# maniacs-ops/ringpop-go

Measured on AMD Instinct MI355X. Metric: simulated member-rounds/sec at 64k members, higher is better.
Workload: dtype u32; 1 GPU; config3_cascade: 65536 members, 655 killed at r=10; rounds 5-592 timed (steady state, kill, suspect wave; faulty wave from r>=35 in window); members=65536, live_member_rounds=38153303, parallelism=1 GPU

## Files before the change

### ringpop-go_amd/csrc/swimsim_engine.hip

```cpp
#include "swimsim_kernels.hip"
#include "swimsim_xchg.hip"
#include "swimsim_census.hip"
#include "swimsim_route.hip"

#include <hipcub/hipcub.hpp>
#include <rccl/rccl.h>

#include <algorithm>
#include <cmath>
#include <condition_variable>
#include <cstdarg>
#include <cstdio>
#include <cstring>
#include <memory>
#include <mutex>
#include <string>
#include <thread>
#include <vector>

#include "../../include/swimsim.h"

using namespace swimdev;

namespace {

const char *kStatus[4] = {"alive", "suspect", "faulty", "leave"};
constexpr uint32_t kWatchCap = 64;

struct Timed {
    int fam;
    hipEvent_t a, b;
};

enum Fam { F_TIMERS, F_SELECT, F_ISSUE, F_SORT, F_RECV, F_RESP, F_PINGREQ, F_JOBS, F_CS_WIDE, F_CS_NARROW, F_CSPREP,
           F_EVENTS, F_XCHG, F_RECVFIN, F_CSD_SCAN, F_CS_FALLBACK, F_JOBS_MERGE, F_NFAM };
const char *kFamName[F_NFAM] = {"timers", "select", "issue", "sort", "recv_merge", "resp_merge", "pingreq",
                                "rfs_jobs", "checksum_wide", "checksum_narrow", "checksum_prep", "events", "exchange",
                                "recv_finish", "checksum_delta_scan", "checksum_fallback", "rfs_merge"};

struct Transport {
    uint32_t G = 1, rank = 0;
    virtual ~Transport() {}
    virtual int sizes(const uint64_t *send, uint64_t *recv, int k) = 0;
    virtual int data(const uint8_t *sbuf, const uint64_t *soff, const uint64_t *sbytes, uint8_t *rbuf,
                     const uint64_t *roff, const uint64_t *rbytes, hipStream_t st) = 0;
    virtual int bcast(void *buf, size_t bytes, uint32_t root) = 0;
    virtual const char *name() const = 0;
    virtual bool stream_ordered() const { return false; }
    virtual int sizes_dev(const uint64_t *dsend, uint64_t *drecv, int k, hipStream_t st) { return SWIMSIM_EINVAL; }
};

struct LocalHub {
    uint32_t G;
    std::mutex m;
    std::condition_variable cv;
    uint32_t arrived = 0, gen = 0;
    bool aborted = false;
    std::vector<const void *> ptr;
    std::vector<const uint64_t *> off, len;
    std::vector<int> dev;
    explicit LocalHub(uint32_t g) : G(g), ptr(g), off(g), len(g), dev(g, 0) {}
    bool barrier() {
        std::unique_lock<std::mutex> lk(m);
        if (aborted) return false;
        const uint32_t my = gen;
        if (++arrived == G) {
            arrived = 0;
            gen++;
            cv.notify_all();
        } else {
            cv.wait(lk, [&] { return gen != my || aborted; });
        }
        return !aborted;
    }
    void abort() {
        std::lock_guard<std::mutex> lk(m);
        aborted = true;
        cv.notify_all();
    }
};

struct LocalPort : Transport {
    std::shared_ptr<LocalHub> hub;
    int device = 0;
    const char *name() const override { return "local"; }
    int sizes(const uint64_t *send, uint64_t *recv, int k) override {
        hub->ptr[rank] = send;
        if (!hub->barrier()) return SWIMSIM_EHIP;
        for (uint32_t s = 0; s < G; s++)
            for (int i = 0; i < k; i++) recv[s * k + i] = ((const uint64_t *)hub->ptr[s])[rank * k + i];
        return hub->barrier() ? 0 : SWIMSIM_EHIP;
    }
    int data(const uint8_t *sbuf, const uint64_t *soff, const uint64_t *sbytes, uint8_t *rbuf, const uint64_t *roff,
             const uint64_t *rbytes, hipStream_t st) override {
        hub->ptr[rank] = sbuf;
        hub->off[rank] = soff;
        hub->len[rank] = sbytes;
        hub->dev[rank] = device;
        if (!hub->barrier()) return SWIMSIM_EHIP;
        hipError_t e = hipSuccess;
        for (uint32_t s = 0; s < G && e == hipSuccess; s++) {
            if (!rbytes[s]) continue;
            const uint8_t *src = (const uint8_t *)hub->ptr[s] + hub->off[s][rank];
            e = hub->dev[s] == device ? hipMemcpyAsync(rbuf + roff[s], src, rbytes[s], hipMemcpyDeviceToDevice, st)
                                      : hipMemcpyPeerAsync(rbuf + roff[s], device, src, hub->dev[s], rbytes[s], st);
        }
        if (e == hipSuccess) e = hipStreamSynchronize(st);
        if (e != hipSuccess) { hub->abort(); return SWIMSIM_EHIP; }
        return hub->barrier() ? 0 : SWIMSIM_EHIP;
    }
    int bcast(void *buf, size_t bytes, uint32_t root) override {
        hub->ptr[rank] = buf;
        if (!hub->barrier()) return SWIMSIM_EHIP;
        if (rank != root) memcpy(buf, hub->ptr[root], bytes);
        return hub->barrier() ? 0 : SWIMSIM_EHIP;
    }
};

struct RcclPort : Transport {
    ncclComm_t comm = nullptr;
    hipStream_t st = nullptr;
    hipEvent_t order = nullptr;
    uint64_t *dsz = nullptr;
    size_t dsz_cap = 0;
    const char *name() const override { return "rccl"; }
    bool stream_ordered() const override { return true; }
    ~RcclPort() override {
        if (comm) ncclCommDestroy(comm);
        if (dsz) hipFree(dsz);
        if (order) hipEventDestroy(order);
    }
    int stage(size_t bytes) {
        if (bytes <= dsz_cap) return 0;
        if (dsz) hipFree(dsz);
        dsz_cap = std::max<size_t>(bytes, 4096);
        return hipMalloc(&dsz, dsz_cap) == hipSuccess ? 0 : SWIMSIM_ENOMEM;
    }
    int sizes(const uint64_t *send, uint64_t *recv, int k) override {
        const size_t n = (size_t)G * k;
        if (int rc = stage(2 * n * 8)) return rc;
        uint64_t *ds = dsz, *dr = dsz + n;
        if (hipMemcpyAsync(ds, send, n * 8, hipMemcpyHostToDevice, st) != hipSuccess) return SWIMSIM_EHIP;
        if (int rc = sizes_dev(ds, dr, k, st)) return rc;
        if (hipMemcpyAsync(recv, dr, n * 8, hipMemcpyDeviceToHost, st) != hipSuccess) return SWIMSIM_EHIP;
        return hipStreamSynchronize(st) == hipSuccess ? 0 : SWIMSIM_EHIP;
    }
    int sizes_dev(const uint64_t *dsend, uint64_t *drecv, int k, hipStream_t s) override {
        if (s != st) return SWIMSIM_EINVAL;
        ncclResult_t rc = ncclGroupStart();
        for (uint32_t p = 0; p < G && rc == ncclSuccess; p++) {
            rc = ncclSend(dsend + (size_t)p * k, k, ncclUint64, (int)p, comm, st);
            if (rc == ncclSuccess) rc = ncclRecv(drecv + (size_t)p * k, k, ncclUint64, (int)p, comm, st);
        }
        const ncclResult_t rc_end = ncclGroupEnd();
        return rc == ncclSuccess && rc_end == ncclSuccess ? 0 : SWIMSIM_EHIP;
    }
    int data(const uint8_t *sbuf, const uint64_t *soff, const uint64_t *sbytes, uint8_t *rbuf, const uint64_t *roff,
             const uint64_t *rbytes, hipStream_t s) override {
        if (s != st) {
            if (!order && hipEventCreateWithFlags(&order, hipEventDisableTiming) != hipSuccess) return SWIMSIM_EHIP;
            if (hipEventRecord(order, st) != hipSuccess || hipStreamWaitEvent(s, order, 0) != hipSuccess) return SWIMSIM_EHIP;
        }
        ncclResult_t rc = ncclGroupStart();
        for (uint32_t p = 0; p < G && rc == ncclSuccess; p++) {
            if (sbytes[p]) rc = ncclSend(sbuf + soff[p], sbytes[p], ncclUint8, (int)p, comm, s);
            if (rbytes[p] && rc == ncclSuccess) rc = ncclRecv(rbuf + roff[p], rbytes[p], ncclUint8, (int)p, comm, s);
        }
        const ncclResult_t rc_end = ncclGroupEnd();
        if (rc != ncclSuccess || rc_end != ncclSuccess) return SWIMSIM_EHIP;
        if (s != st && (hipEventRecord(order, s) != hipSuccess || hipStreamWaitEvent(st, order, 0) != hipSuccess))
            return SWIMSIM_EHIP;
        return 0;
    }
    int bcast(void *buf, size_t bytes, uint32_t root) override {
        if (int rc = stage(bytes)) return rc;
        if (hipMemcpyAsync(dsz, buf, bytes, hipMemcpyHostToDevice, st) != hipSuccess) return SWIMSIM_EHIP;
        if (ncclBroadcast(dsz, dsz, bytes, ncclUint8, (int)root, comm, st) != ncclSuccess) return SWIMSIM_EHIP;
        if (hipMemcpyAsync(buf, dsz, bytes, hipMemcpyDeviceToHost, st) != hipSuccess) return SWIMSIM_EHIP;
        return hipStreamSynchronize(st) == hipSuccess ? 0 : SWIMSIM_EHIP;
    }
};

struct HostPort : Transport {
    swimsim_host_transport t{};
    uint8_t *hs = nullptr, *hr = nullptr;
    size_t hs_cap = 0, hr_cap = 0;
    const char *name() const override { return "host"; }
    ~HostPort() override {
        if (hs) hipHostFree(hs);
        if (hr) hipHostFree(hr);
    }
    static int grow(uint8_t **p, size_t *cap, size_t bytes) {
        if (bytes <= *cap) return 0;
        if (*p) hipHostFree(*p);
        *cap = std::max<size_t>(bytes + bytes / 2, 1 << 16);
        return hipHostMalloc((void **)p, *cap, 0) == hipSuccess ? 0 : SWIMSIM_ENOMEM;
    }
    int sizes(const uint64_t *send, uint64_t *recv, int k) override {
        return t.alltoall_u64(t.ctx, send, recv, k) ? SWIMSIM_EHIP : 0;
    }
    int data(const uint8_t *sbuf, const uint64_t *soff, const uint64_t *sbytes, uint8_t *rbuf, const uint64_t *roff,
             const uint64_t *rbytes, hipStream_t st) override {
        size_t stot = 0, rtot = 0;
        for (uint32_t p = 0; p < G; p++) {
            stot = std::max<size_t>(stot, soff[p] + sbytes[p]);
            rtot = std::max<size_t>(rtot, roff[p] + rbytes[p]);
        }
        if (grow(&hs, &hs_cap, stot) || grow(&hr, &hr_cap, rtot)) return SWIMSIM_ENOMEM;
        if (stot && hipMemcpyAsync(hs, sbuf, stot, hipMemcpyDeviceToHost, st) != hipSuccess) return SWIMSIM_EHIP;
        if (hipStreamSynchronize(st) != hipSuccess) return SWIMSIM_EHIP;
        if (t.alltoallv(t.ctx, hs, soff, sbytes, hr, roff, rbytes)) return SWIMSIM_EHIP;
        if (rtot && hipMemcpyAsync(rbuf, hr, rtot, hipMemcpyHostToDevice, st) != hipSuccess) return SWIMSIM_EHIP;
        return hipStreamSynchronize(st) == hipSuccess ? 0 : SWIMSIM_EHIP;
    }
    int bcast(void *buf, size_t bytes, uint32_t root) override { return t.bcast(t.ctx, buf, bytes, root) ? SWIMSIM_EHIP : 0; }
};

struct CsrSet {
    bool ready = false, failed = false;
    uint32_t rows = 0;
    uint32_t *B = nullptr, *Lb = nullptr, *OB = nullptr, *SBw = nullptr, *fb = nullptr, *fbcnt = nullptr, *nrec = nullptr;
    uint4 *ent = nullptr, *P = nullptr;
    CsdRow *rinfo = nullptr;
    CsrPlan *plan = nullptr;
    CsrRec *rec = nullptr;
    uint4 *ucol = nullptr;
    uint32_t *fbsplit = nullptr;
    unsigned long long *acc = nullptr;
    void *cub_tmp = nullptr;
    size_t cub_bytes = 0;
    uint32_t *ucl = nullptr, *uhk = nullptr, *ucold = nullptr, *ucnt = nullptr;
};

}

struct swimsim {
    uint32_t N = 0, NP = 0, NL = 0, lo = 0, W = 19, K = 3, maxjobs = 5, pfactor = 15;
    int64_t t0 = 0;
    uint32_t period = 200;
    uint32_t to_susp = 25, to_faulty = 0, to_tomb = 0;
    uint64_t seed = 1;
    uint32_t ecap = 0, max_tl = 0;
    bool fast_cs = false;
    int device = 0;
    hipStream_t s = nullptr;
    hipStream_t side = nullptr;
    hipEvent_t ev_snap = nullptr, ev_side[2] = {nullptr, nullptr};
    hipEvent_t ev_rt = nullptr;
    hipStream_t side2 = nullptr;
    hipEvent_t ev_csr2 = nullptr;
    bool csr2_used = false;
    bool sync_spin = true;
    bool cs_async = true, side_pending = false;
    bool side_pend[2] = {false, false};
    uint32_t side_halves = 1, side_gen = 0;
    uint32_t cs_narrow_rows = CS_NARROW_ROWS;
    uint32_t snap_cap = 0;
    uint32_t *side_ids = nullptr, *side_cnt = nullptr;

    DS d{};
    std::vector<uint8_t> live;
    std::vector<int32_t> part;
    std::vector<int32_t> coff;
    int32_t coff_min = 0, coff_max = 0;
    std::vector<std::string> addrs;
    uint32_t round = 0;
    uint64_t host_ctr[SWIMSIM_NCOUNTERS] = {0};
    uint32_t G = 1, rank = 0;
    std::vector<uint32_t> shard_lo;
    std::unique_ptr<Transport> xp;
    uint4 *xitems = nullptr;
    uint32_t *xcnt = nullptr, xcap = 0;
    unsigned long long *xsz = nullptr, *xseg = nullptr, *xtcur = nullptr, *xdcur = nullptr;
    ulonglong2 *xsrcs = nullptr;
    uint8_t *sbuf = nullptr, *rbuf = nullptr;
    size_t sbuf_cap = 0, rbuf_cap = 0;
    uint2 *needlist = nullptr;
    uint32_t *needcnt = nullptr, needcap = 0;
    uint32_t *hsics = nullptr, *npairs = nullptr;
    unsigned long long *keys = nullptr, *keys_sorted = nullptr;
    uint32_t keycap = 0;
    uint64_t x_bytes = 0, x_calls = 0;
    uint64_t x_syncs = 0;
    uint64_t lazy_fallbacks = 0;
    uint64_t alloc_bytes = 0;
    int32_t *tgt = nullptr;
    uint8_t *failed = nullptr;
    MsgDesc *sdesc = nullptr, *rdesc = nullptr, *sdesc2 = nullptr, *rdesc2 = nullptr, *snapdesc = nullptr, *hdesc = nullptr;
    uint32_t *sI = nullptr, *sC = nullptr, *sI2 = nullptr, *sC2 = nullptr;
    uint32_t *sS = nullptr, *sS2 = nullptr;
    uint32_t *rcs = nullptr, *csreqcnt = nullptr;
    uint4 *csreq = nullptr;
    uint32_t *fpv = nullptr, *fpv_s = nullptr, *fph = nullptr, *fph_s = nullptr, *fplist = nullptr, *fpcnt = nullptr,
             *dup_of = nullptr;
    uint8_t *hflag = nullptr;
    uint32_t *H = nullptr, *nh = nullptr;
    uint32_t *keys_in = nullptr, *vals_out = nullptr;
    uint4 *pinfo = nullptr;
    uint32_t inbox_n = 0;
    uint32_t *ukeys = nullptr, *counts = nullptr, *offs = nullptr, *nruns = nullptr, *info = nullptr;
    void *cub_tmp = nullptr;
    size_t cub_bytes = 0;
    uint32_t *list = nullptr, *cnt = nullptr;
    uint4 *defer = nullptr;
    uint32_t *defer_cnt = nullptr;
    uint8_t *defer_eq = nullptr;
    unsigned long long *rep_tab = nullptr;
    unsigned long long *fp_tab = nullptr;
    uint32_t rep_mask = 0, rep_gen = 0;
    uint32_t *exh_list = nullptr, *exh_cnt = nullptr, *scratch = nullptr;
    uint8_t *need = nullptr, *fsflag = nullptr;
    uint4 *evbuf = nullptr;
    uint32_t *ev_applied = nullptr;
    uint32_t evcap = 0;
    uint4 *jl = nullptr;
    unsigned long long *digest_buf = nullptr;
    uint32_t *hinfo = nullptr;
    std::vector<void *> allocs;
    bool timing = false;
    uint32_t timing_mask = 0;
    std::vector<Timed> pending;
    std::vector<hipEvent_t> evpool;
    double fam_ms[F_NFAM] = {0};
    uint64_t fam_n[F_NFAM] = {0};
    uint64_t fam_bytes_base[CTR_STRIDE] = {0};
    std::vector<hipEvent_t> round_ev;
    std::vector<float> round_ms;
    std::vector<uint32_t> wslot_h;
    std::vector<uint8_t> wused;
    std::vector<uint32_t> wcs;
    std::vector<uint32_t> wcs_ev;
    std::vector<uint4 *> wev_h;
    std::vector<unsigned long long *> wevt_h;
    uint4 *wout = nullptr;
    uint32_t *winfo = nullptr;
    uint32_t *cn_slab = nullptr, *cn_part = nullptr, *cn_nlp = nullptr, *cn_ticket = nullptr, *cn_cols = nullptr,
             *cn_res = nullptr;
    size_t cn_cap = 0;
    hipEvent_t cn_ev[2] = {nullptr, nullptr};
    uint32_t *tr_cols = nullptr, *tr_buf = nullptr, *tr_part = nullptr, *tr_nlp = nullptr, *tr_state = nullptr;
    uint32_t tr_n = 0, tr_cap = 0;
    size_t tr_bytes[5] = {0, 0, 0, 0, 0};
    struct RouteTable {
        uint32_t R;
        uint32_t *hm;
        unsigned long long *pts;
    };
    std::vector<RouteTable> rt_tabs;
    uint8_t *rt_bytes = nullptr;
    uint64_t *rt_off = nullptr;
    uint32_t *rt_kh = nullptr, *rt_p0 = nullptr, *rt_rows = nullptr, *rt_cnt = nullptr;
    int32_t *rt_base = nullptr, *rt_own = nullptr;
    uint32_t *rt_srv = nullptr;
    int32_t *rt_nbase = nullptr;
    size_t rt_srv_cap = 0, rt_nbase_cap = 0;
    unsigned long long *rt_exc = nullptr, *rt_exc2 = nullptr, *rt_uniq = nullptr, *rt_cur = nullptr;
    void *rt_cub = nullptr;
    size_t rt_bytes_cap = 0, rt_keys_cap = 0, rt_rows_cap = 0, rt_own_cap = 0, rt_exc_cap = 0, rt_cub_bytes = 0;
    std::vector<uint64_t> rt_rel;
    hipEvent_t rt_ev[2] = {nullptr, nullptr};
    int csr_mode = 1;
    CsrSet csr, csr2;
    size_t csr_sbw_words = 0;
    uint32_t csr_ecap = 4096, csr_rcap = 1024, csr_KP = 0;
    uint64_t csr_launches = 0;
    uint32_t csr_side_min = 4097;
    int fault_inject = 0;
    int defer_test = 0;
    int cs_defer = 1;
    uint32_t rounds_left = 0;
    uint32_t round_deferred = 0;
    bool cs_carried = false;
    bool cs_defer_log = false;
    uint64_t cs_skipped_rounds = 0, cs_carried_rows = 0, cs_forced = 0, cs_units_base[3] = {0, 0, 0};
    bool colx_stale = false;
    std::string err;

    int fail(int code, const char *fmt, ...) {
        char buf[512];
        va_list ap;
        va_start(ap, fmt);
        vsnprintf(buf, sizeof buf, fmt, ap);
        va_end(ap);
        err = buf;
        return code;
    }
};

#define HIPCHK(h, x)                                                                             \
    do {                                                                                         \
        hipError_t e_ = (x);                                                                     \
        if (e_ != hipSuccess) return (h)->fail(SWIMSIM_EHIP, "%s: %s", #x, hipGetErrorString(e_)); \
    } while (0)

namespace {

template <typename T>
int dalloc(swimsim *h, T **p, size_t count, const char *what) {
    void *q = nullptr;
    size_t bytes = std::max<size_t>(count * sizeof(T), 16);
    hipError_t e = hipMalloc(&q, bytes);
    if (e != hipSuccess) return h->fail(SWIMSIM_ENOMEM, "hipMalloc(%s, %zu bytes): %s", what, bytes, hipGetErrorString(e));
    h->allocs.push_back(q);
    h->alloc_bytes += bytes;
    *p = (T *)q;
    return 0;
}

template <typename T>
void dfree(swimsim *h, T **p, size_t bytes) {
    if (!*p) return;
    auto it = std::find(h->allocs.begin(), h->allocs.end(), (void *)*p);
    if (it != h->allocs.end()) h->allocs.erase(it);
    hipFree(*p);
    h->alloc_bytes -= bytes;
    *p = nullptr;
}

hipEvent_t take_event(swimsim *h) {
    if (!h->evpool.empty()) {
        hipEvent_t e = h->evpool.back();
        h->evpool.pop_back();
        return e;
    }
    hipEvent_t e;
    hipEventCreate(&e);
    return e;
}

struct Scope {
    swimsim *h;
    int fam;
    hipStream_t st;
    hipEvent_t a{}, b{};
    bool on;
    Scope(swimsim *h_, int f, hipStream_t st_ = nullptr)
        : h(h_), fam(f), st(st_ ? st_ : h_->s), on(h_->timing && ((h_->timing_mask >> f) & 1u)) {
        if (on) {
            a = take_event(h);
            hipEventRecord(a, st);
        }
    }
    ~Scope() {
        if (on) {
            b = take_event(h);
            hipEventRecord(b, st);
            h->pending.push_back(Timed{fam, a, b});
        }
    }
};

void drain_timing(swimsim *h) {
    if (h->pending.empty()) return;
    hipStreamSynchronize(h->s);
    for (auto &t : h->pending) {
        float ms = 0;
        hipEventElapsedTime(&ms, t.a, t.b);
        h->fam_ms[t.fam] += ms;
        h->fam_n[t.fam]++;
        h->evpool.push_back(t.a);
        h->evpool.push_back(t.b);
    }
    h->pending.clear();
}

constexpr uint32_t SWIM_WAVE_BLOCK = 256;
constexpr uint32_t kWavesPerBlock = SWIM_WAVE_BLOCK / 64;
inline uint32_t blocks_for_waves(uint32_t waves) { return waves ? (waves + kWavesPerBlock - 1) / kWavesPerBlock : 1; }
inline uint32_t blocks_for_threads(uint32_t n) { return n ? (n + 255) / 256 : 1; }
inline uint32_t rep_slots(uint32_t nl) { uint32_t s = 1024; while (s < 2 * nl) s <<= 1; return s; }

constexpr uint32_t kMaxEcap = 1u << 24;

int build_tail_table(swimsim *h, uint32_t ecap) {
    if (ecap > kMaxEcap)
        return h->fail(SWIMSIM_ERANGE, "incarnation step %u beyond the checksum tables (at most 2^24 steps of the period)",
                       ecap - 1);
    std::vector<uint32_t> t((size_t)ecap * 4 * 8, 0u);
    uint32_t max_tl = 0, min_tl = 0xFFFFFFFFu;
    for (uint32_t e = 0; e < ecap; e++) {
        char digits[32];
        snprintf(digits, sizeof digits, "%lld", (long long)(h->t0 + (int64_t)e * h->period));
        for (uint32_t s = 0; s < 4; s++) {
            char buf[64];
            int n = snprintf(buf, sizeof buf, "%s%s;", kStatus[s], digits);
            if (n > 24) return h->fail(SWIMSIM_EINVAL, "incarnation %s too long for the checksum tail table", digits);
            uint8_t bytes[24] = {0};
            memcpy(bytes, buf, (size_t)n);
            uint32_t *dst = &t[((size_t)e * 4 + s) * 8];
            for (int w = 0; w < 6; w++)
                dst[w] = (uint32_t)bytes[4 * w] | ((uint32_t)bytes[4 * w + 1] << 8) | ((uint32_t)bytes[4 * w + 2] << 16) |
                         ((uint32_t)bytes[4 * w + 3] << 24);
            dst[6] = (uint32_t)n;
            max_tl = std::max(max_tl, (uint32_t)n);
            min_tl = std::min(min_tl, (uint32_t)n);
        }
    }
    std::vector<uint32_t> rt((size_t)ecap * 4 * 8, 0u);
    const uint32_t q = h->W / 4, r = h->W % 4;
    for (size_t i = 0; i < (size_t)ecap * 4; i++) {
        uint8_t bytes[32] = {0};
        const uint32_t n = t[i * 8 + 6];
        memcpy(bytes + r, &t[i * 8], n);
        for (int w = 0; w < 7; w++)
            rt[i * 8 + w] = (uint32_t)bytes[4 * w] | ((uint32_t)bytes[4 * w + 1] << 8) | ((uint32_t)bytes[4 * w + 2] << 16) |
                            ((uint32_t)bytes[4 * w + 3] << 24);
        const uint32_t L = h->W + n;
        const uint8_t *tb = (const uint8_t *)&t[i * 8];
        rt[i * 8 + 7] = (uint32_t)tb[n - 4] | ((uint32_t)tb[n - 3] << 8) | ((uint32_t)tb[n - 2] << 16) |
                        ((uint32_t)tb[n - 1] << 24);
        if (r + n > 27) return h->fail(SWIMSIM_EINVAL, "record tail too long for the checksum tail table");
        rt[i * 8 + 6] |= L << 24;
    }
    (void)q;
    std::vector<uint32_t> rt8((size_t)ecap * 8 * 8, 0u);
    for (size_t e = 0; e < ecap; e++)
        for (int s = 0; s < 4; s++) memcpy(&rt8[(e * 8 + s) * 8], &rt[(e * 4 + s) * 8], 32);
    uint32_t *dev = nullptr, *rdev = nullptr, *r8dev = nullptr;
    if (int rc = dalloc(h, &dev, t.size(), "tail table")) return rc;
    if (int rc = dalloc(h, &rdev, rt.size(), "record tail table")) return rc;
    if (int rc = dalloc(h, &r8dev, rt8.size(), "record tail table by member word")) return rc;
    HIPCHK(h, hipMemcpy(dev, t.data(), t.size() * 4, hipMemcpyHostToDevice));
    HIPCHK(h, hipMemcpy(rdev, rt.data(), rt.size() * 4, hipMemcpyHostToDevice));
    HIPCHK(h, hipMemcpy(r8dev, rt8.data(), rt8.size() * 4, hipMemcpyHostToDevice));
    h->d.tailw = dev;
    h->d.rtail = rdev;
    h->d.rtail8 = r8dev;
    {
        uint32_t d0 = t[6] - 6, nthr = 0;
        for (int k = 0; k < 8; k++) h->d.dig_thr[k] = 0xFFFFFFFFu;
        uint32_t prev = d0;
        for (uint32_t e = 1; e < ecap; e++) {
            const uint32_t de = t[((size_t)e * 4) * 8 + 6] - 6;
            if (de != prev) {
                if (de != prev + 1 || nthr == 8) return h->fail(SWIMSIM_EINVAL, "incarnation digit count changes too often");
                h->d.dig_thr[nthr++] = e;
                prev = de;
            }
        }
        h->d.dig_d0 = d0;
    }
    h->ecap = ecap;
    h->d.ecap = ecap;
    h->max_tl = max_tl;
    h->d.max_tail = max_tl;
    h->d.min_tail = min_tl;
    h->fast_cs = (h->W == 19 && h->W + max_tl <= 40);
    return 0;
}

hipError_t stream_sync(swimsim *h) {
    if (!h->sync_spin || !h->ev_rt) return hipStreamSynchronize(h->s);
    const hipError_t prior = hipPeekAtLastError();
    hipError_t e = hipEventRecord(h->ev_rt, h->s);
    if (e != hipSuccess) return e;
    while ((e = hipEventQuery(h->ev_rt)) == hipErrorNotReady) {
    }
    (void)hipGetLastError();
    return prior != hipSuccess ? prior : e;
}

int check_err(swimsim *h) {
    uint32_t e = 0;
    HIPCHK(h, hipMemcpyAsync(&e, h->d.err, 4, hipMemcpyDeviceToHost, h->s));
    HIPCHK(h, stream_sync(h));
    if (!e) return 0;
    hipMemsetAsync(h->d.err, 0, 4, h->s);
    if (e & E_POOL) return h->fail(SWIMSIM_ECAPACITY, "message pool overflow (raise message_pool_bytes)");
    if (e & E_DENSE) return h->fail(SWIMSIM_ECAPACITY, "dense snapshot pool overflow");
    if (e & E_ECAP) return h->fail(SWIMSIM_ECAPACITY, "incarnation beyond the checksum table");
    if (e & E_SHORT) return h->fail(SWIMSIM_EINVAL, "checksum string of <= 24 bytes is not supported");
    if (e & E_ITER) return h->fail(SWIMSIM_EINVAL, "iterator found no pingable member despite a positive count");
    return h->fail(SWIMSIM_EINVAL, "dissemination count mismatch (internal error %u)", e);
}

int read_counters(swimsim *h, uint64_t *out ) {
    std::vector<uint64_t> c((size_t)CTR_SHARDS * CTR_STRIDE);
    HIPCHK(h, hipMemcpyAsync(c.data(), h->d.ctr, c.size() * 8, hipMemcpyDeviceToHost, h->s));
    HIPCHK(h, stream_sync(h));
    for (int i = 0; i < CTR_STRIDE; i++) {
        uint64_t t = 0;
        for (int k = 0; k < CTR_SHARDS; k++) t += c[(size_t)k * CTR_STRIDE + i];
        out[i] = t;
    }
    return 0;
}

int sort_inbox(swimsim *h, uint32_t n, uint32_t *host_info) {
    Scope sc(h, F_SORT);
    h->inbox_n = n;
    int endbit = 1;
    while ((1u << endbit) <= h->N) endbit++;
    size_t bytes = h->cub_bytes;
    HIPCHK(h, hipcub::DeviceRadixSort::SortKeys(h->cub_tmp, bytes, h->keys, h->keys_sorted, (int)n, 0, 32 + endbit, h->s));
    hipLaunchKernelGGL(k_split_keys, dim3(blocks_for_threads(n)), dim3(256), 0, h->s, h->keys_sorted, n, h->keys_in,
                       h->vals_out);
    bytes = h->cub_bytes;
    HIPCHK(h, hipcub::DeviceRunLengthEncode::Encode(h->cub_tmp, bytes, h->keys_in, h->ukeys, h->counts, h->nruns,
                                                    (int)n, h->s));
    bytes = h->cub_bytes;
    HIPCHK(h, hipcub::DeviceScan::ExclusiveSum(h->cub_tmp, bytes, h->counts, h->offs, (int)n, h->s));
    HIPCHK(h, hipMemsetAsync(h->info, 0, 8, h->s));
    hipLaunchKernelGGL(k_runs_info, dim3(blocks_for_threads(n)), dim3(256), 0, h->s, h->ukeys, h->counts, h->nruns, h->N,
                       h->info);
    HIPCHK(h, hipMemcpyAsync(host_info, h->info, 16, hipMemcpyDeviceToHost, h->s));
    HIPCHK(h, stream_sync(h));
    return 0;
}

inline uint32_t owner_host(const swimsim *h, uint32_t o) {
    uint32_t r = 0;
    while (r + 1 < h->G && o >= h->shard_lo[r + 1]) r++;
    return r;
}

XArgs xargs(swimsim *h) {
    XArgs x{};
    x.sdesc = h->sdesc; x.sdesc2 = h->sdesc2; x.rdesc = h->rdesc; x.rdesc2 = h->rdesc2; x.snapdesc = h->snapdesc;
    x.hdesc = h->hdesc;
    x.sI = h->sI; x.sC = h->sC; x.sI2 = h->sI2; x.sC2 = h->sC2;
    x.hsics = h->hsics;
    x.need = h->need;
    x.keys = h->keys; x.npairs = h->npairs; x.keycap = h->keycap;
    x.needlist = h->needlist; x.needcnt = h->needcnt; x.needcap = h->needcap;
    x.sS = h->sS; x.sS2 = h->sS2; x.rcs = h->rcs;
    x.csreq = h->csreq; x.csreqcnt = h->csreqcnt; x.csreqcap = h->keycap;
    return x;
}

int xchg(swimsim *h) {
    Scope sc(h, F_XCHG);
    const uint32_t G = h->G;
    const XArgs x = xargs(h);
    HIPCHK(h, hipMemsetAsync(h->xsz, 0, 2 * G * 8, h->s));
    hipLaunchKernelGGL(k_x_size, dim3(blocks_for_threads(h->xcap)), dim3(256), 0, h->s, h->d, x, h->xitems, h->xcnt,
                       h->xcap, h->xsz);
    const bool dev_sizes = h->xp->stream_ordered();
    std::vector<uint64_t> sz(2 * G), sendsz(2 * G), recvsz(2 * G), devsend(2 * G);
    uint32_t nitems = 0;
    hipLaunchKernelGGL(k_x_sendsz, dim3(1), dim3(64), 0, h->s, h->xsz, G, h->xsz + 2 * G);
    if (dev_sizes) {
        if (int rc = h->xp->sizes_dev((const uint64_t *)(h->xsz + 2 * G), (uint64_t *)(h->xsz + 4 * G), 2, h->s))
            return h->fail(rc, "shard size exchange failed (%s)", h->xp->name());
        HIPCHK(h, hipMemcpyAsync(recvsz.data(), h->xsz + 4 * G, 2 * G * 8, hipMemcpyDeviceToHost, h->s));
    } else {
        HIPCHK(h, hipMemcpyAsync(devsend.data(), h->xsz + 2 * G, 2 * G * 8, hipMemcpyDeviceToHost, h->s));
    }
    HIPCHK(h, hipMemcpyAsync(sz.data(), h->xsz, 2 * G * 8, hipMemcpyDeviceToHost, h->s));
    HIPCHK(h, hipMemcpyAsync(&nitems, h->xcnt, 4, hipMemcpyDeviceToHost, h->s));
    HIPCHK(h, stream_sync(h));
    h->x_syncs++;
    if (nitems > h->xcap) return h->fail(SWIMSIM_ECAPACITY, "exchange item list overflow (%u items)", nitems);
    std::vector<uint64_t> soff(G), sbytes(G), tbl(G), cur(3 * G);
    uint64_t total = 0;
    for (uint32_t p = 0; p < G; p++) {
        tbl[p] = (sz[2 * p + 1] * 4 + 15) & ~15ull;
        sbytes[p] = sz[2 * p + 1] ? tbl[p] + sz[2 * p] : 0;
        soff[p] = total;
        total += (sbytes[p] + 15) & ~15ull;
        cur[p] = soff[p];
        cur[G + p] = 0;
        cur[2 * G + p] = tbl[p];
        sendsz[2 * p] = sbytes[p];
        sendsz[2 * p + 1] = sz[2 * p + 1];
    }
    if (!dev_sizes && devsend != sendsz)
        return h->fail(SWIMSIM_EHIP, "exchange: device send sizes (k_x_sendsz) differ from the host's");
    if (total > h->sbuf_cap) {
        if (h->sbuf) hipFree(h->sbuf);
        h->sbuf_cap = std::max<uint64_t>(total + total / 2, 1 << 20);
        HIPCHK(h, hipMalloc(&h->sbuf, h->sbuf_cap));
    }
    HIPCHK(h, hipMemcpyAsync(h->xseg, cur.data(), 3 * G * 8, hipMemcpyHostToDevice, h->s));
    if (nitems)
        hipLaunchKernelGGL(k_x_pack, dim3(blocks_for_waves(nitems)), dim3(SWIM_WAVE_BLOCK), 0, h->s, h->d, x, h->xitems, h->xcnt,
                           h->xcap, h->sbuf, h->xseg, h->xtcur, h->xdcur);
    if (!dev_sizes) {
        HIPCHK(h, stream_sync(h));
        if (int rc = h->xp->sizes(sendsz.data(), recvsz.data(), 2)) return h->fail(rc, "shard size exchange failed (%s)", h->xp->name());
        h->x_syncs += 2;
    }
    std::vector<uint64_t> roff(G), rbytes(G);
    std::vector<ulonglong2> srcs(G);
    uint64_t rtotal = 0, nparc = 0;
    for (uint32_t p = 0; p < G; p++) {
        rbytes[p] = recvsz[2 * p];
        roff[p] = rtotal;
        srcs[p] = make_ulonglong2(rtotal, nparc);
        rtotal += (rbytes[p] + 15) & ~15ull;
        nparc += recvsz[2 * p + 1];
    }
    if (rtotal > h->rbuf_cap) {
        if (h->rbuf) hipFree(h->rbuf);
        h->rbuf_cap = std::max<uint64_t>(rtotal + rtotal / 2, 1 << 20);
        HIPCHK(h, hipMalloc(&h->rbuf, h->rbuf_cap));
    }
    if (int rc = h->xp->data(h->sbuf, soff.data(), sbytes.data(), h->rbuf, roff.data(), rbytes.data(), h->s))
        return h->fail(rc, "shard data exchange failed (%s)", h->xp->name());
    if (nparc) {
        HIPCHK(h, hipMemcpyAsync(h->xsrcs, srcs.data(), G * sizeof(ulonglong2), hipMemcpyHostToDevice, h->s));
        hipLaunchKernelGGL(k_x_unpack, dim3(blocks_for_waves((uint32_t)nparc)), dim3(SWIM_WAVE_BLOCK), 0, h->s, h->d, x, h->rbuf,
                           h->xsrcs, G, (uint32_t)nparc);
    }
    HIPCHK(h, hipMemsetAsync(h->xcnt, 0, 4, h->s));
    h->x_bytes += total;
    h->x_calls++;
    return 0;
}

int shard_sum(swimsim *h, uint64_t v, uint64_t *out) {
    if (h->G == 1) { *out = v; return 0; }
    std::vector<uint64_t> send(h->G, v), recv(h->G);
    if (int rc = h->xp->sizes(send.data(), recv.data(), 1)) return h->fail(rc, "shard reduction failed");
    uint64_t t = 0;
    for (uint64_t x : recv) t += x;
    *out = t;
    return 0;
}

bool csr_wanted(swimsim *h, uint32_t n, CsKind kind) {
    if (h->csr_mode == 0 || h->csr.failed || n < CSD_MIN_ROWS || h->N < 1024) return false;
    return kind == CS_WIDE || h->csr_mode == 2;
}

bool csr_side_wanted(swimsim *h, uint32_t n) {
    return h->csr_mode != 0 && !h->csr2.failed && h->csr2.rows && n >= h->csr_side_min && n <= h->csr2.rows &&
           h->N >= 1024;
}

int csr_alloc(swimsim *h, CsrSet &c, uint32_t rows) {
    if (c.ready) return 0;
    if (c.failed) return 1;
    const bool side = &c == &h->csr2;
    h->csr_rcap = h->N <= 131072 ? 1024u : 512u;
    h->csr_sbw_words = ((size_t)h->N * (h->W + 32) + 256) / 4;
    h->csr_KP = (uint32_t)(h->csr_sbw_words * 4 / 20 + 2);
    c.rows = rows;
    const size_t nalloc0 = h->allocs.size();
    const uint64_t bytes0 = h->alloc_bytes;
    auto undo = [&](int rc) {
        for (size_t i = nalloc0; i < h->allocs.size(); i++) hipFree(h->allocs[i]);
        h->allocs.resize(nalloc0);
        h->alloc_bytes = bytes0;
        (void)hipGetLastError();
        c.failed = true;
        c.rows = 0;
        h->err.clear();
        return rc;
    };
    int rc = 0;
    if ((rc = dalloc(h, &c.B, (size_t)h->NP, "csr reference row")) ||
        (rc = dalloc(h, &c.Lb, (size_t)h->N + 1, "csr reference lengths")) ||
        (rc = dalloc(h, &c.OB, (size_t)h->N + 1, "csr reference offsets")) ||
        (rc = dalloc(h, &c.SBw, h->csr_sbw_words, "csr reference string")) ||
        (rc = dalloc(h, &c.P, (size_t)20 * h->csr_KP * 2, "csr premix table")) ||
        (rc = dalloc(h, &c.fb, (size_t)rows, "csr fallback list")) ||
        (rc = dalloc(h, &c.fbcnt, 8, "csr fallback count and reasons")) ||
        (rc = dalloc(h, &c.rinfo, (size_t)rows, "csr row info")) ||
        (rc = dalloc(h, &c.ent, ((size_t)rows * h->csr_ecap + CSR_EREG) * 2, "csr exception entries")) ||
        (rc = dalloc(h, &c.plan, (size_t)rows / CSR_ROWS + 1, "csr plans")) ||
        (rc = dalloc(h, &c.rec, (size_t)rows * h->csr_rcap, "csr records")) ||
        (rc = dalloc(h, &c.nrec, (size_t)rows, "csr record counts")) ||
        (rc = dalloc(h, &c.ucol, (size_t)h->N, "csr divergent column table")) ||
        (rc = (h->fault_inject & 1) ? h->fail(SWIMSIM_ENOMEM, "injected allocation failure") : 0) ||
        (rc = dalloc(h, &c.fbsplit, 4, "csr fallback split")) ||
        (rc = dalloc(h, &c.acc, 8, "csr path statistics")))
        return undo(rc);
    if (side && ((rc = dalloc(h, &c.ucl, (size_t)h->N, "csr side divergent columns")) ||
                 (rc = dalloc(h, &c.uhk, (size_t)h->N, "csr side divergent column slots")) ||
                 (rc = dalloc(h, &c.ucold, (size_t)h->N, "csr side cold columns")) ||
                 (rc = dalloc(h, &c.ucnt, 2, "csr side column counts"))))
        return undo(rc);
    size_t need = 0;
    hipcub::DeviceScan::ExclusiveSum(nullptr, need, c.Lb, c.OB, (int)h->N + 1, h->s);
    void *p = nullptr;
    if ((side || need > h->cub_bytes) && (rc = dalloc(h, (uint8_t **)&p, need, "cub temp (csr)"))) return undo(rc);
    if (hipMemsetAsync(c.acc, 0, 8 * sizeof(unsigned long long), h->s) != hipSuccess) return undo(SWIMSIM_EHIP);
    if (side) {
        c.cub_tmp = p;
        c.cub_bytes = need;
    } else if (p) {
        h->cub_tmp = p;
        h->cub_bytes = need;
    }
    c.ready = true;
    return 0;
}
int csr_alloc(swimsim *h) { return csr_alloc(h, h->csr, h->NL); }

__global__ void k_csr_fbsplit(uint32_t *fbcnt, uint32_t *split, unsigned long long *acc) {
    const uint32_t t = threadIdx.x;
    const uint32_t nf = fbcnt[0];
    if (t == 0) {
        split[0] = min(nf, 4096u);
        split[1] = nf > 4096u ? min(nf - 4096u, 8192u) : 0u;
        split[2] = nf > 12288u ? nf - 12288u : 0u;
    }
    if (t < 8 && nf) acc[t] += fbcnt[t];
}

int csr_hash(swimsim *h, CsrSet &c, const uint32_t *list, const uint32_t *cnt, uint32_t n, hipStream_t st, int chains = 4) {
    const bool side = &c == &h->csr2;
    if (n > (side ? c.rows : h->NL)) return 1;
    if (side ? !c.ready : csr_alloc(h, c, h->NL)) return 1;
    if (h->fault_inject & 2) {
        h->fault_inject &= ~2;
        return h->fail(SWIMSIM_EHIP, "csr_hash: injected HIP error");
    }
    DS d = h->d;
    if (side) { d.ucl = c.ucl; d.uhk = c.uhk; d.ucold = c.ucold; d.ucnt = c.ucnt; }
    void *cub = side ? c.cub_tmp : h->cub_tmp;
    size_t cub_bytes = side ? c.cub_bytes : h->cub_bytes;
    CsdArgs ca{};
    ca.B = c.B;
    ca.OB = c.OB;
    ca.SBw = c.SBw;
    ca.sbw_words = (uint32_t)h->csr_sbw_words;
    ca.ent = c.ent;
    ca.rinfo = c.rinfo;
    ca.ecap = h->csr_ecap;
    ca.ulist = d.ucl;
    ca.ucnt = d.ucnt;
    ca.ucol = c.ucol;
    ca.uhk = side ? nullptr : d.uhk;
    CsrArgs a{};
    a.P = c.P;
    a.KP = h->csr_KP;
    a.ent = c.ent;
    a.rinfo = c.rinfo;
    a.ecap = h->csr_ecap;
    a.plan = c.plan;
    a.rec = c.rec;
    a.nrec = c.nrec;
    a.rcap = h->csr_rcap;
    a.fb_list = c.fb;
    a.fb_cnt = c.fbcnt;
    a.exw = (h->fault_inject & 4) ? 8u : 0xFFFFFFFFu;
    a.stprio = (h->fault_inject & 16) ? 1u : 0u;
    a.jitter = (h->fault_inject & 64) ? (((uint32_t)h->fault_inject >> 8) & 15u) | ((uint32_t)h->fault_inject >> 12 << 8) : 0u;
    {
        Scope sc(h, F_CSD_SCAN, st);
        hipLaunchKernelGGL(k_csd_ref, dim3((h->N + 256) / 256), dim3(256), 0, st, d, list, n, c.B, c.Lb);
        size_t bytes = cub_bytes;
        HIPCHK(h, hipcub::DeviceScan::ExclusiveSum(cub, bytes, c.Lb, c.OB, (int)h->N + 1, st));
        HIPCHK(h, hipMemsetAsync(c.SBw, 0, h->csr_sbw_words * 4, st));
        hipLaunchKernelGGL(k_ucols, dim3(1), dim3(1024), 0, st, d);
        hipLaunchKernelGGL(k_csr_ucol, dim3((h->N + 255) / 256), dim3(256), 0, st, d.ucl, d.ucnt, c.B, c.OB, c.ucol);
        launch_csr(d, list, n, cnt, ca, a, st, 0);
        launch_csr(d, list, n, cnt, ca, a, st, 1);
        launch_csr(d, list, n, cnt, ca, a, st, 2);
        launch_csr(d, list, n, cnt, ca, a, st, 3);
        HIPCHK(h, hipMemsetAsync(c.fbcnt, 0, 32, st));
        hipLaunchKernelGGL(k_ctr_add, dim3(1), dim3(1), 0, st, d, (int)C_X_CSD_SCANNED, (unsigned long long)n);
    }
    {
        Scope sc(h, F_CS_WIDE, st);
        launch_csr(d, list, n, cnt, ca, a, st, chains);
    }
    h->csr_launches++;
    Scope sc(h, F_CS_FALLBACK, st);
    hipLaunchKernelGGL(k_csr_fbsplit, dim3(1), dim3(64), 0, st, c.fbcnt, c.fbsplit, c.acc);
    launch_checksum_kind(d, c.fb, c.fbsplit, std::min(n, 4096u), CS_NARROW, st);
    if (n > 4096u) launch_checksum_kind(d, c.fb + 4096, c.fbsplit + 1, std::min(n - 4096u, 8192u), CS_NARROW, st);
    if (n > 12288u) launch_checksum_kind(d, c.fb + 12288, c.fbsplit + 2, n - 12288u, CS_WIDE, st);
    return 0;
}
int csr_hash(swimsim *h, const uint32_t *list, const uint32_t *cnt, uint32_t n, int chains = 4) {
    return csr_hash(h, h->csr, list, cnt, n, h->s, chains);
}

int hash_rows(swimsim *h, const uint32_t *list, const uint32_t *cnt, uint32_t maxn, uint32_t nrows,
              hipStream_t st = nullptr, bool ordered = false) {
    if (std::min(maxn, nrows) == 0) return 0;
    if (!st && !ordered && nrows != ~0u && nrows >= 64 && nrows <= h->NL && (list == h->list || list == h->fplist)) {
        Scope sc(h, F_CSPREP);
        uint32_t *out = list == h->list ? h->fplist : h->list;
        const uint32_t maxid = h->NL + h->d.dense_cap;
        size_t bytes = h->cub_bytes;
        if (hipcub::DeviceRadixSort::SortKeys(h->cub_tmp, bytes, list, out, (int)nrows, 0, 32 - __builtin_clz(maxid),
                                              h->s) == hipSuccess)
            list = out;
    }
    const uint32_t n = std::min(maxn, nrows);
    const CsKind kind = cs_kind(n, h->cs_narrow_rows);
    if (!st && nrows != ~0u && csr_wanted(h, n, kind)) {
        const int rc = csr_hash(h, list, cnt, n);
        if (rc <= 0) return rc;
    }
    if (st && nrows != ~0u && csr_side_wanted(h, n)) {
        if (h->csr2_used) HIPCHK(h, hipStreamWaitEvent(st, h->ev_csr2, 0));
        const int rc = csr_hash(h, h->csr2, list, cnt, n, st);
        HIPCHK(h, hipEventRecord(h->ev_csr2, st));
        h->csr2_used = true;
        if (rc <= 0) return rc;
    }
    Scope sc(h, kind == CS_WIDE ? F_CS_WIDE : F_CS_NARROW, st);
    launch_checksum_kind(h->d, list, cnt, n, kind, st ? st : h->s);
    return 0;
}

void hot_flush(swimsim *h, uint32_t ol0, uint32_t n) {
    if (!h->d.hidx || n == 0) return;
    hipLaunchKernelGGL(k_hot_flush, dim3(blocks_for_waves(n)), dim3(SWIM_WAVE_BLOCK), 0, h->s, h->d, ol0, n);
}

void hot_reset(swimsim *h, bool flush) {
    if (!h->d.hidx) return;
    if (flush) hot_flush(h, 0, h->NL);
    hipMemsetAsync(h->d.hidx, 0xFF, (size_t)h->N * 4, h->s);
    hipMemsetAsync(h->d.hotnew, 0, (size_t)h->d.NBIT * 4, h->s);
    hipMemsetAsync(h->d.hot_cnt, 0, 8, h->s);
    hipLaunchKernelGGL(k_nhe_reset, dim3(blocks_for_threads(h->NL)), dim3(256), 0, h->s, h->d);
}

void hot_update(swimsim *h) {
    if (!h->d.hidx) return;
    hipLaunchKernelGGL(k_hot_extend, dim3(1), dim3(1024), 0, h->s, h->d);
    hipLaunchKernelGGL(k_hot_fill, dim3(blocks_for_waves(h->NL)), dim3(SWIM_WAVE_BLOCK), 0, h->s, h->d);
}

int retire_half(swimsim *h, uint32_t g) {
    if (!h->side_pend[g]) return 0;
    HIPCHK(h, hipStreamWaitEvent(h->s, h->ev_side[g], 0));
    const uint32_t lo = h->d.dense_cap + g * h->snap_cap;
    hipLaunchKernelGGL(k_side_retire, dim3(blocks_for_threads(h->NL)), dim3(256), 0, h->s, h->d, lo, lo + h->snap_cap);
    h->side_pend[g] = false;
    h->side_pending = h->side_pend[0] || h->side_pend[1];
    return 0;
}

int sync_side(swimsim *h) {
    if (!h->side_pending) return 0;
    for (uint32_t g = 0; g < 2; g++)
        if (int rc = retire_half(h, (h->side_gen + g) % 2)) return rc;
    return 0;
}

constexpr uint32_t CS_DEFER_CHANGED_NUM = 3, CS_DEFER_CHANGED_DEN = 4, CS_DEFER_MAX_DEFERRED_DIV = 64;

int checksum_dirty(swimsim *h, int mode, bool async = false) {
    const uint32_t g = h->side_gen;
    if (async && h->cs_async && h->side_halves == 2) {
        if (int rc = retire_half(h, g)) return rc;
    } else if (int rc = sync_side(h)) {
        return rc;
    }
    HIPCHK(h, hipMemsetAsync(h->cnt, 0, 8, h->s));
    {
        Scope sc(h, F_CSPREP);
        hipLaunchKernelGGL(k_list, dim3(blocks_for_threads(h->NL)), dim3(256), 0, h->s, h->d, mode, h->tgt, h->failed,
                           h->list, h->cnt);
    }
    if (mode != 0) return hash_rows(h, h->list, h->cnt, h->NL, ~0u);
    uint32_t *hn = h->hinfo + 8;
    HIPCHK(h, hipMemcpyAsync(hn, h->cnt, 8, hipMemcpyDeviceToHost, h->s));
    HIPCHK(h, stream_sync(h));
    const uint32_t n = *hn;
    if (async && h->cs_defer && h->rounds_left && n) {
        const uint32_t changed = hn[1];
        const bool wide = n > (h->cs_async ? h->snap_cap : 0u);
        const bool moving = (uint64_t)changed * CS_DEFER_CHANGED_DEN >= (uint64_t)n * CS_DEFER_CHANGED_NUM;
        const bool calm = h->round_deferred <= h->NL / CS_DEFER_MAX_DEFERRED_DIV;
        const bool skip = h->cs_defer == 2 || (wide && moving && calm);
        if (h->cs_defer_log)
            fprintf(stderr, "cs_defer round %u: dirty %u changed %u deferred %u: %s\n", h->round, n, changed,
                    h->round_deferred, skip ? "carried" : wide && moving ? "hashed (valve)" : "hashed");
        if (skip) {
            hipLaunchKernelGGL(k_carry, dim3(blocks_for_threads(h->NL)), dim3(256), 0, h->s, h->d);
            h->cs_carried = true;
            h->cs_skipped_rounds++;
            h->cs_carried_rows += n;
            return 0;
        }
        if (wide && moving) h->cs_forced++;
    }
    h->cs_carried = false;
    auto go_side = [&](const uint32_t *rows, uint32_t n2, const uint32_t *vals, const uint32_t *dups) -> int {
        uint32_t *ids = h->side_ids + (size_t)g * h->snap_cap, *icnt = h->side_cnt + g;
        {
            Scope sc(h, F_CSPREP);
            hipLaunchKernelGGL(k_snap_rows, dim3(blocks_for_waves(std::max(n2, 1u))), dim3(SWIM_WAVE_BLOCK), 0, h->s, h->d, rows, n2,
                               ids, icnt, h->d.dense_cap + g * h->snap_cap);
            hipLaunchKernelGGL(k_snap_dups, dim3(blocks_for_threads(n)), dim3(256), 0, h->s, h->d, vals, n, dups);
            hipLaunchKernelGGL(k_ctr_add, dim3(1), dim3(1), 0, h->s, h->d, (int)C_X_CS_DUP, (unsigned long long)(n - n2));
        }
        HIPCHK(h, hipEventRecord(h->ev_snap, h->s));
        hipStream_t ss = g == 0 || !h->side2 ? h->side : h->side2;
        HIPCHK(h, hipStreamWaitEvent(ss, h->ev_snap, 0));
        if (int rc = hash_rows(h, ids, icnt, n2, n2, ss)) return rc;
        HIPCHK(h, hipEventRecord(h->ev_side[g], ss));
        h->side_pend[g] = true;
        h->side_pending = true;
        h->side_gen = (g + 1) % h->side_halves;
        return 0;
    };
    const bool side_ok = async && h->cs_async;
    if (n < 2) {
        if (n == 1 && side_ok && h->snap_cap >= 1) return go_side(h->list, 1, h->list, nullptr);
        return hash_rows(h, h->list, h->cnt, n, n);
    }
    {
        Scope sc(h, F_CSPREP);
        const unsigned long long keymask = (h->fault_inject & 8) ? 7ull : ~0ull;
        const uint32_t fmask = 2u * rep_slots(h->NL) - 1u;
        HIPCHK(h, hipMemsetAsync(h->fp_tab, 0xFF, (size_t)(fmask + 1) * 2 * 8, h->s));
        for (int pass = 0; pass < 2; pass++)
            hipLaunchKernelGGL(k_fp_table, dim3(blocks_for_threads(n)), dim3(256), 0, h->s, h->d, h->list, n, h->fp_tab,
                               fmask, keymask, pass);
        hipLaunchKernelGGL(k_ucols, dim3(1), dim3(1024), 0, h->s, h->d);
        hipLaunchKernelGGL(k_fp_verify_tab, dim3(blocks_for_waves(n)), dim3(SWIM_WAVE_BLOCK), 0, h->s, h->d, h->list, n,
                           h->fp_tab, fmask, keymask, h->hflag, h->dup_of);
        hipLaunchKernelGGL(k_list_flagged_ordered, dim3(1), dim3(1024), 0, h->s, h->NL, h->hflag, h->fplist, h->fpcnt);
        HIPCHK(h, hipMemcpyAsync(hn + 1, h->fpcnt, 4, hipMemcpyDeviceToHost, h->s));
    }
    HIPCHK(h, stream_sync(h));
    if (side_ok && hn[1] <= h->snap_cap) return go_side(h->fplist, hn[1], h->list, h->dup_of);
    if (int rc = hash_rows(h, h->fplist, h->fpcnt, n, hn[1], nullptr, true)) return rc;
    Scope sc(h, F_CSPREP);
    hipLaunchKernelGGL(k_fp_copy, dim3(blocks_for_threads(n)), dim3(256), 0, h->s, h->d, h->list, n, h->dup_of);
    return 0;
}

int bound_lazy_snapshots(swimsim *h, int mode) {
    if (h->NL <= h->d.dense_cap / 2) return 0;
    HIPCHK(h, hipMemsetAsync(h->cnt, 0, 4, h->s));
    hipLaunchKernelGGL(k_list, dim3(blocks_for_threads(h->NL)), dim3(256), 0, h->s, h->d, mode, h->tgt, h->failed,
                       h->list, h->cnt);
    uint32_t *hc = h->hinfo + 12;
    HIPCHK(h, hipMemcpyAsync(hc, h->cnt, 4, hipMemcpyDeviceToHost, h->s));
    HIPCHK(h, stream_sync(h));
    if (*hc <= h->d.dense_cap / 2) return 0;
    if (int rc = sync_side(h)) return rc;
    if (int rc = hash_rows(h, h->list, h->cnt, h->NL, *hc)) return rc;
    h->lazy_fallbacks++;
    return 0;
}

int resolve_deferred(swimsim *h, int phase, MsgDesc *rdesc, uint32_t maxn) {
    const bool remote = h->G > 1 && phase != 2;
    uint32_t *sS = phase == 0 ? h->sS : phase == 1 ? h->sS2 : nullptr;
    const uint32_t *sI = phase == 1 ? h->sI2 : h->sI;
    if (remote || phase == 2)
        if (int rc = sync_side(h)) return rc;
    uint32_t maxlist = 2 * maxn;
    {
        Scope sc(h, F_CSPREP);
        HIPCHK(h, hipMemsetAsync(h->cnt, 0, 8, h->s));
        hipLaunchKernelGGL(k_ucols, dim3(1), dim3(1024), 0, h->s, h->d);
        if (h->rep_tab) {
            h->rep_gen = h->rep_gen % 255u + 1u;
            hipLaunchKernelGGL(k_cs_reps, dim3(blocks_for_threads(h->NL)), dim3(256), 0, h->s, h->d, h->defer_cnt, h->rep_tab,
                               h->rep_mask, h->rep_gen);
        }
        hipLaunchKernelGGL(k_defer_eq, dim3(blocks_for_waves(maxn)), dim3(SWIM_WAVE_BLOCK), 0, h->s, h->d, h->defer, h->defer_cnt,
                           phase, h->defer_eq, h->rep_tab, h->rep_mask, h->rep_gen, sS);
        if (sS)
            hipLaunchKernelGGL(k_lazy_mat, dim3(blocks_for_waves(maxn)), dim3(SWIM_WAVE_BLOCK), 0, h->s, h->d, h->defer,
                               h->defer_eq, (const uint4 *)nullptr, h->defer_cnt, 0xFFFFFFFFu, phase, sS, sI);
        hipLaunchKernelGGL(k_defer_ids, dim3(blocks_for_threads(maxn)), dim3(256), 0, h->s, h->d, h->defer,
                           h->defer_cnt, h->defer_eq, h->list, h->cnt, phase, sS);
    }
    if (remote) {
        HIPCHK(h, hipMemsetAsync(h->csreqcnt, 0, 4, h->s));
        hipLaunchKernelGGL(k_x_csreq, dim3(blocks_for_threads(maxn)), dim3(256), 0, h->s, h->d, h->defer, h->defer_cnt,
                           phase, h->xitems, h->xcnt, h->xcap);
        if (int rc = xchg(h)) return rc;
        hipLaunchKernelGGL(k_lazy_mat, dim3(blocks_for_waves(h->keycap)), dim3(SWIM_WAVE_BLOCK), 0, h->s, h->d,
                           (const uint4 *)nullptr, (const uint8_t *)nullptr, h->csreq, h->csreqcnt, h->keycap, phase, sS, sI);
        hipLaunchKernelGGL(k_csreq_ids, dim3(blocks_for_threads(h->keycap)), dim3(256), 0, h->s, h->d, h->csreq,
                           h->csreqcnt, h->list, h->cnt, sS);
        maxlist += h->keycap;
    }
    {
        uint32_t *hc = h->hinfo + 10;
        HIPCHK(h, hipMemcpyAsync(hc, h->cnt, 4, hipMemcpyDeviceToHost, h->s));
        HIPCHK(h, hipMemcpyAsync(hc + 1, h->cnt + 1, 4, hipMemcpyDeviceToHost, h->s));
        HIPCHK(h, hipMemcpyAsync(h->hinfo + 14, h->defer_cnt, 4, hipMemcpyDeviceToHost, h->s));
        HIPCHK(h, stream_sync(h));
        if (phase != 2) h->round_deferred += h->hinfo[14];
        if (int rc = hash_rows(h, h->list, h->cnt, maxlist, *hc)) return rc;
        if (hc[1])
            if (int rc = sync_side(h)) return rc;
    }
    if (remote) {
        hipLaunchKernelGGL(k_x_csresp, dim3(blocks_for_threads(h->keycap)), dim3(256), 0, h->s, h->d, h->csreq,
                           h->csreqcnt, h->xitems, h->xcnt, h->xcap, sS);
        if (int rc = xchg(h)) return rc;
    }
    Scope sc(h, phase == 1 ? F_PINGREQ : F_RECVFIN);
    hipLaunchKernelGGL(k_recv_finish, dim3(blocks_for_threads(maxn)), dim3(256), 0, h->s, h->d, h->defer,
                       h->defer_cnt, rdesc, phase, h->fsflag, h->rcs, h->defer_eq, sS);
    return 0;
}

int run_waves(swimsim *h, int phase, uint32_t nruns_valid, uint32_t maxcount) {
    RecvArgs a{};
    a.ukeys = h->ukeys; a.counts = h->counts; a.offs = h->offs; a.vals = h->vals_out;
    a.nruns_max = nruns_valid;
    a.phase = phase;
    a.sdesc = phase == 0 ? h->sdesc : h->sdesc2;
    a.sI = phase == 0 ? h->sI : h->sI2;
    a.sC = phase == 0 ? h->sC : h->sC2;
    a.sS = phase == 0 ? h->sS : h->sS2;
    a.rdesc = phase == 0 ? h->rdesc : h->rdesc2;
    a.defer = h->defer;
    a.defer_cnt = h->defer_cnt;
    a.fsflag = h->fsflag;
    a.r = h->round;
    a.pinfo = h->pinfo;
    hipMemsetAsync(h->defer_cnt, 0, 4, h->s);
    {
        Scope sc(h, F_SORT);
        hipLaunchKernelGGL(k_pair_info, dim3(blocks_for_threads(std::max(h->inbox_n, h->NL))), dim3(256), 0, h->s, h->d,
                           h->vals_out, h->inbox_n, phase, a.sdesc, a.sI, a.sC, a.sS, h->pinfo);
    }
    {
        Scope sc(h, F_RECV);
        hipLaunchKernelGGL(k_recv, dim3(blocks_for_waves(nruns_valid)), dim3(SWIM_WAVE_BLOCK), 0, h->s, h->d, a);
    }
    const uint32_t maxdefer = std::min<uint64_t>((uint64_t)nruns_valid * maxcount, h->d.dense_cap);
    if (int rc = resolve_deferred(h, phase, a.rdesc, maxdefer)) return rc;
    if (phase == 0) {
        Scope sc(h, F_RECVFIN);
        hipLaunchKernelGGL(k_build_jobs, dim3(blocks_for_threads(nruns_valid)), dim3(256), 0, h->s, h->d, h->ukeys,
                           h->counts, h->offs, h->vals_out, nruns_valid, h->fsflag);
    }
    return 0;
}

void clock_offset_range(swimsim *h) {
    h->coff_min = h->coff_max = 0;
    for (int32_t k : h->coff) {
        h->coff_min = std::min(h->coff_min, k);
        h->coff_max = std::max(h->coff_max, k);
    }
}

inline uint32_t census_cols_chunks(const swimsim *h) {
    return std::max(1u, (h->NL + CENSUS_COLS_CHUNK_ROWS - 1) / CENSUS_COLS_CHUNK_ROWS);
}
inline uint32_t census_chunks(const swimsim *h) { return std::max(1u, (h->NL + CENSUS_CHUNK_ROWS - 1) / CENSUS_CHUNK_ROWS); }

int flush_events(swimsim *h, std::vector<uint4> &evs) {
    if (evs.empty()) return 0;
    Scope sc(h, F_EVENTS);
    if (evs.size() > h->evcap) return h->fail(SWIMSIM_EINVAL, "too many events in one round (%zu)", evs.size());
    HIPCHK(h, hipMemcpyAsync(h->evbuf, evs.data(), evs.size() * sizeof(uint4), hipMemcpyHostToDevice, h->s));
    hipLaunchKernelGGL(k_events, dim3(1), dim3(64), 0, h->s, h->d, h->evbuf, (uint32_t)evs.size(), h->round, h->ev_applied);
    evs.clear();
    return 0;
}

int upload_topology(swimsim *h) {
    HIPCHK(h, hipMemcpyAsync(h->d.live, h->live.data(), h->N, hipMemcpyHostToDevice, h->s));
    HIPCHK(h, hipMemcpyAsync(h->d.part, h->part.data(), h->N * 4, hipMemcpyHostToDevice, h->s));
    return 0;
}

bool host_reach(swimsim *h, uint32_t a, uint32_t b) { return h->live[a] && h->live[b] && h->part[a] == h->part[b]; }

int ensure_clean_checksum(swimsim *h, uint32_t ol) {
    hipLaunchKernelGGL(k_list_one, dim3(1), dim3(64), 0, h->s, h->list, h->cnt, ol, h->d);
    return hash_rows(h, h->list, h->cnt, 1, 1);
}

inline bool own(const swimsim *h, uint32_t o) { return o >= h->lo && o < h->lo + h->NL; }

int push_item(swimsim *h, uint4 it) {
    hipLaunchKernelGGL(k_x_item, dim3(1), dim3(64), 0, h->s, h->d, it, h->xitems, h->xcnt, h->xcap);
    return 0;
}

int ping_with(swimsim *h, uint32_t o, uint32_t t, int slot) {
    const uint32_t root = owner_host(h, o), ot = owner_host(h, t);
    if (h->rank == root) {
        if (int rc = ensure_clean_checksum(h, o - h->lo)) return rc;
        hipLaunchKernelGGL(k_sender_info, dim3(1), dim3(64), 0, h->s, h->d, o - h->lo, h->hsics);
    }
    const MsgDesc *md = h->hdesc + slot;
    const uint32_t *sics = h->hsics;
    if (h->G > 1) {
        if (h->rank == root) {
            HIPCHK(h, hipMemcpyAsync(h->hdesc + 7, h->hdesc + slot, sizeof(MsgDesc), hipMemcpyDeviceToDevice, h->s));
            push_item(h, make_uint4(ot, P_PING, t, o));
        }
        if (int rc = xchg(h)) return rc;
        md = h->hdesc + 5;
        sics = h->hsics + 2;
    }
    if (h->rank == ot) {
        hipMemsetAsync(h->defer_cnt, 0, 4, h->s);
        hipLaunchKernelGGL(k_ping_with, dim3(1), dim3(64), 0, h->s, h->d, t - h->lo, o, md, sics, h->hdesc + 8,
                           h->defer, h->defer_cnt, h->round);
        if (int rc = resolve_deferred(h, 2, h->hdesc + 9, 1)) return rc;
    }
    return 0;
}

int do_heal(swimsim *h, uint32_t o, std::vector<int32_t> *ret) {
    if (int rc = sync_side(h)) return rc;
    const uint32_t root = owner_host(h, o);
    const bool me = h->rank == root;
    const uint32_t ol = o - h->lo;
    std::vector<int32_t> targets;
    if (me) {
        std::vector<uint32_t> row(h->NP);
        HIPCHK(h, hipMemcpyAsync(row.data(), h->d.mw + (size_t)ol * h->NP, h->NP * 4, hipMemcpyDeviceToHost, h->s));
        HIPCHK(h, stream_sync(h));
        for (uint32_t m = 0; m < h->N; m++)
            if ((row[m] & 7u) >= ST_FAULTY) targets.push_back((int32_t)m);
        for (uint32_t i = 0; i < targets.size(); i++) {
            const U4 v = philox10(h->round, o, 3u, i >> 2, h->seed);
            const uint32_t j = mulhi_n(pick(v, i), i + 1);
            std::swap(targets[i], targets[j]);
        }
    }
    auto del = [](std::vector<int32_t> &t, int32_t v) {
        for (size_t i = 0; i < t.size(); i++) {
            if (t[i] != v) continue;
            t[i] = t.back();
            t.pop_back();
            i--;
        }
    };
    int failures = 0;
    for (;;) {
        int32_t cmd = (me && !targets.empty() && failures < 10) ? targets[0] : -1;
        if (h->G > 1)
            if (int rc = h->xp->bcast(&cmd, sizeof cmd, root)) return h->fail(rc, "heal broadcast failed");
        if (cmd < 0) break;
        const uint32_t target = (uint32_t)cmd;
        if (me) {
            del(targets, cmd);
            h->host_ctr[SWIMSIM_C_HEAL_ATTEMPTS]++;
        }
        if (!host_reach(h, o, target)) {
            if (me) {
                failures++;
                h->host_ctr[SWIMSIM_C_HEAL_FAILURES]++;
            }
            continue;
        }
        const uint32_t ot = owner_host(h, target);
        HIPCHK(h, hipMemsetAsync(h->d.dense_cur, 0, 4, h->s));
        if (h->G == 1) {
            hipLaunchKernelGGL(k_snapshot_row, dim3(1), dim3(64), 0, h->s, h->d, target - h->lo, h->hdesc + 1);
        } else {
            if (h->rank == ot) {
                hipLaunchKernelGGL(k_snapshot_row, dim3(1), dim3(64), 0, h->s, h->d, target - h->lo, h->hdesc + 6);
                push_item(h, make_uint4(root, P_HEALROW, target, 0));
            }
            if (int rc = xchg(h)) return rc;
        }
        uint32_t lens[2] = {0, 0};
        MsgDesc hd[4];
        if (me) {
            hipLaunchKernelGGL(k_snapshot_row, dim3(1), dim3(64), 0, h->s, h->d, ol, h->hdesc + 0);
            hipLaunchKernelGGL(k_heal_diff, dim3(1), dim3(64), 0, h->s, h->d, h->hdesc + 0, h->hdesc + 1, h->hdesc + 2,
                               h->hdesc + 3);
            HIPCHK(h, hipMemcpyAsync(hd, h->hdesc, sizeof hd, hipMemcpyDeviceToHost, h->s));
            HIPCHK(h, stream_sync(h));
            if (hd[0].kind != 1 || hd[1].kind != 1) return h->fail(SWIMSIM_ECAPACITY, "dense snapshot pool overflow in heal");
            lens[0] = hd[2].len;
            lens[1] = hd[3].len;
        }
        if (h->G > 1)
            if (int rc = h->xp->bcast(lens, sizeof lens, root)) return h->fail(rc, "heal broadcast failed");
        if (lens[0] || lens[1]) {
            if (me && lens[0]) hipLaunchKernelGGL(k_apply_msg, dim3(1), dim3(64), 0, h->s, h->d, ol, h->hdesc + 2, h->round);
            if (lens[1])
                if (int rc = ping_with(h, o, target, 3)) return rc;
        } else {
            if (me) {
                hipLaunchKernelGGL(k_apply_msg, dim3(1), dim3(64), 0, h->s, h->d, ol, h->hdesc + 1, h->round);
                hipLaunchKernelGGL(k_snapshot_row, dim3(1), dim3(64), 0, h->s, h->d, ol, h->hdesc + 4);
            }
            if (int rc = ping_with(h, o, target, 4)) return rc;
        }
        if (me) {
            std::vector<uint32_t> mb(h->NP);
            HIPCHK(h, hipMemcpyAsync(mb.data(), h->d.dense + (size_t)hd[1].off_lo * h->NP, h->NP * 4,
                                     hipMemcpyDeviceToHost, h->s));
            HIPCHK(h, stream_sync(h));
            for (uint32_t m = 0; m < h->N; m++) {
                const uint32_t st = mb[m] & 7u;
                if (st != ST_UNKNOWN && is_pingable(st == ST_TOMB ? ST_FAULTY : st)) del(targets, (int32_t)m);
            }
            if (ret) ret->push_back(cmd);
        }
    }
    return 0;
}

int step_one(swimsim *h, const swimsim_event *ev, size_t nev, uint32_t rounds_left) {
    const uint32_t r = h->round;
    const bool sharded = h->G > 1;
    h->rounds_left = rounds_left;
    h->round_deferred = 0;
    {
        hipEvent_t e = take_event(h);
        HIPCHK(h, hipEventRecord(e, h->s));
        h->round_ev.push_back(e);
    }
    HIPCHK(h, hipMemsetAsync(h->d.pool_cur, 0, POOL_SHARDS * POOL_CUR_STRIDE * 8, h->s));
    std::vector<uint4> batch;
    bool topo_dirty = false;
    for (size_t i = 0; i < nev; i++) {
        const swimsim_event &e = ev[i];
        if (e.round != r) continue;
        const uint32_t a = (uint32_t)e.a;
        if (a >= h->N) return h->fail(SWIMSIM_EINVAL, "event member %d out of range", e.a);
        switch (e.kind) {
        case SWIMSIM_EV_KILL: h->live[a] = 0; topo_dirty = true; break;
        case SWIMSIM_EV_REVIVE:
            h->live[a] = 1; topo_dirty = true;
            if (own(h, a)) batch.push_back(make_uint4(2, a, a, 0));
            break;
        case SWIMSIM_EV_REINCARNATE: if (h->live[a] && own(h, a)) batch.push_back(make_uint4(2, a, a, 0)); break;
        case SWIMSIM_EV_LEAVE: if (h->live[a] && own(h, a)) batch.push_back(make_uint4(3, a, a, 0)); break;
        case SWIMSIM_EV_PARTITION: h->part[a] = e.b; topo_dirty = true; break;
        case SWIMSIM_EV_REAP: if (h->live[a] && own(h, a)) batch.push_back(make_uint4(4, a, a, 0)); break;
        case SWIMSIM_EV_CLOCK:
            h->coff[a] = e.b;
            clock_offset_range(h);
            batch.push_back(make_uint4(5, a, a, (uint32_t)e.b));
            break;
        case SWIMSIM_EV_HEAL:
            if (!h->live[a]) break;
            if (int rc = flush_events(h, batch)) return rc;
            if (int rc = upload_topology(h)) return rc;
            topo_dirty = false;
            if (int rc = do_heal(h, a, nullptr)) return rc;
            break;
        default: return h->fail(SWIMSIM_EINVAL, "unknown event kind %u", e.kind);
        }
    }
    if (int rc = flush_events(h, batch)) return rc;
    if (topo_dirty)
        if (int rc = upload_topology(h)) return rc;
    {
        Scope sc(h, F_TIMERS);
        hipLaunchKernelGGL(k_timers, dim3(blocks_for_waves(h->NL)), dim3(SWIM_WAVE_BLOCK), 0, h->s, h->d, r);
    }
    {
        Scope sc(h, F_SELECT);
        hipMemsetAsync(h->exh_cnt, 0, 4, h->s);
        hipLaunchKernelGGL(k_select, dim3(blocks_for_threads(h->NL)), dim3(256), 0, h->s, h->d, h->tgt, h->exh_list,
                           h->exh_cnt);
        hipLaunchKernelGGL(k_select_exhaust, dim3(64), dim3(64), 0, h->s, h->d, h->exh_list, h->exh_cnt, h->scratch);
    }
    uint32_t *hi = h->hinfo;
    uint32_t ninbox = h->NL;
    if (int rc = bound_lazy_snapshots(h, 1)) return rc;
    HIPCHK(h, hipMemsetAsync(h->d.dense_cur, 0, 4, h->s));
    hot_update(h);
    {
        {
            Scope sc(h, F_ISSUE);
            hipLaunchKernelGGL(k_issue, dim3(blocks_for_waves(h->NL)), dim3(SWIM_WAVE_BLOCK), 0, h->s, h->d, 0, h->tgt, h->failed,
                               h->sdesc, h->sI, h->sC, h->sS);
        }
        Scope sc(h, F_SORT);
        HIPCHK(h, hipMemsetAsync(h->info + 2, 0, 4, h->s));
        hipLaunchKernelGGL(k_pairs_direct, dim3(blocks_for_threads(h->NL)), dim3(256), 0, h->s, h->d, h->tgt, h->keys,
                           h->failed, h->info, h->xitems, h->xcnt, h->xcap);
    }
    if (sharded) {
        HIPCHK(h, hipMemcpyAsync(h->npairs, &h->NL, 4, hipMemcpyHostToDevice, h->s));
        if (int rc = xchg(h)) return rc;
        HIPCHK(h, hipMemcpyAsync(&hi[5], h->npairs, 4, hipMemcpyDeviceToHost, h->s));
    }
    if (sharded) {
        HIPCHK(h, stream_sync(h));
        ninbox = std::min(hi[5], h->keycap);
    }
    if (int rc = sort_inbox(h, ninbox, hi)) return rc;
    const uint32_t nfailed = hi[2];
    if (int rc = run_waves(h, 0, hi[0], hi[1])) return rc;
    if (sharded) {
        hipLaunchKernelGGL(k_x_resp, dim3(blocks_for_threads(ninbox)), dim3(256), 0, h->s, h->d, h->keys, ninbox, 0,
                           h->xitems, h->xcnt, h->xcap);
        if (int rc = xchg(h)) return rc;
    }
    {
        Scope sc(h, F_RESP);
        hipLaunchKernelGGL(k_resp, dim3(blocks_for_waves(h->NL)), dim3(SWIM_WAVE_BLOCK), 0, h->s, h->d, h->tgt, h->failed, h->sdesc,
                           h->rdesc, r);
    }
    uint64_t anyfailed = nfailed;
    if (int rc = shard_sum(h, nfailed, &anyfailed)) return rc;
    if (anyfailed) {
        {
            Scope sc(h, F_PINGREQ);
            hipLaunchKernelGGL(k_helpers, dim3(blocks_for_threads(h->NL)), dim3(256), 0, h->s, h->d, h->tgt, h->failed,
                               h->H, h->nh, r);
        }
        if (int rc = bound_lazy_snapshots(h, 2)) return rc;
        HIPCHK(h, hipMemsetAsync(h->d.dense_cur, 0, 4, h->s));
        {
            {
                Scope sc(h, F_ISSUE);
                hipLaunchKernelGGL(k_issue, dim3(blocks_for_waves(h->NL)), dim3(SWIM_WAVE_BLOCK), 0, h->s, h->d, 1, h->tgt, h->failed,
                                   h->sdesc2, h->sI2, h->sC2, h->sS2);
            }
            Scope sc(h, F_PINGREQ);
            hipLaunchKernelGGL(k_pairs_helpers, dim3(blocks_for_threads(h->NL * h->K)), dim3(256), 0, h->s, h->d,
                               h->failed, h->H, h->nh, h->keys, h->xitems, h->xcnt, h->xcap);
        }
        uint32_t ninbox2 = h->NL * h->K;
        if (sharded) {
            HIPCHK(h, hipMemcpyAsync(h->npairs, &ninbox2, 4, hipMemcpyHostToDevice, h->s));
            if (int rc = xchg(h)) return rc;
            HIPCHK(h, hipMemcpyAsync(&hi[5], h->npairs, 4, hipMemcpyDeviceToHost, h->s));
            HIPCHK(h, stream_sync(h));
            ninbox2 = std::min(hi[5], h->keycap);
        }
        if (int rc = sort_inbox(h, ninbox2, hi)) return rc;
        if (int rc = run_waves(h, 1, hi[0], hi[1])) return rc;
        if (sharded) {
            hipLaunchKernelGGL(k_x_resp, dim3(blocks_for_threads(ninbox2)), dim3(256), 0, h->s, h->d, h->keys, ninbox2, 1,
                               h->xitems, h->xcnt, h->xcap);
            if (int rc = xchg(h)) return rc;
        }
        {
            Scope sc(h, F_PINGREQ);
            hipLaunchKernelGGL(k_resolve, dim3(blocks_for_waves(h->NL)), dim3(SWIM_WAVE_BLOCK), 0, h->s, h->d, h->tgt, h->failed,
                               h->H, h->nh, h->sdesc2, h->rdesc2, r);
        }
    }
    {
        Scope sc(h, F_JOBS);
        HIPCHK(h, hipMemsetAsync(h->d.dense_cur, 0, 4, h->s));
        hipLaunchKernelGGL(k_jobs_mark, dim3(blocks_for_threads(h->NL)), dim3(256), 0, h->s, h->d, h->need);
    }
    if (sharded) {
        HIPCHK(h, hipMemsetAsync(h->needcnt, 0, 4, h->s));
        hipLaunchKernelGGL(k_x_need, dim3(blocks_for_threads(h->N)), dim3(256), 0, h->s, h->d, h->need, h->xitems,
                           h->xcnt, h->xcap);
        if (int rc = xchg(h)) return rc;
    }
    {
        Scope sc(h, F_JOBS);
        hipLaunchKernelGGL(k_jobs_snap, dim3(blocks_for_waves(h->NL)), dim3(SWIM_WAVE_BLOCK), 0, h->s, h->d, h->need, h->snapdesc);
    }
    if (sharded) {
        hipLaunchKernelGGL(k_x_snap, dim3(blocks_for_threads(h->needcap)), dim3(256), 0, h->s, h->d, h->needlist,
                           h->needcnt, h->xitems, h->xcnt, h->xcap);
        if (int rc = xchg(h)) return rc;
    }
    {
        Scope sc(h, F_JOBS_MERGE);
        hipLaunchKernelGGL(k_jobs_merge, dim3(blocks_for_waves(h->NL)), dim3(SWIM_WAVE_BLOCK), 0, h->s, h->d, h->snapdesc, r);
    }
    {
        Scope sc(h, F_JOBS);
        hipLaunchKernelGGL(k_jobs_reset, dim3(blocks_for_threads(std::max(h->NL, h->N))), dim3(256), 0, h->s, h->d,
                           h->need);
    }
    if (int rc = checksum_dirty(h, 0, true)) return rc;
    if (h->tr_n)
        hipLaunchKernelGGL(k_census_cols, dim3(census_cols_chunks(h)), dim3(64), 0, h->s, h->d, h->tr_cols, h->tr_n, 0u,
                           h->tr_part, h->tr_nlp, h->tr_state + 2, h->tr_buf, 6u, h->tr_state, h->tr_cap,
                           2u + 6u * h->tr_n, r);
    h->round++;
    h->host_ctr[SWIMSIM_C_ROUNDS]++;
    HIPCHK(h, hipGetLastError());
    return 0;
}

int ensure_ecap(swimsim *h, uint32_t upto) {
    if (upto < h->ecap) return 0;
    if (upto >= kMaxEcap)
        return h->fail(SWIMSIM_ERANGE, "incarnation step %u beyond the checksum tables (at most 2^24 steps of the period)", upto);
    uint32_t c = h->ecap;
    while (c <= upto) c = c >= kMaxEcap / 2 ? kMaxEcap : c * 2;
    HIPCHK(h, stream_sync(h));
    return build_tail_table(h, c);
}

int to_e(swimsim *h, int64_t inc_ms, uint32_t *e) {
    const int64_t dlt = inc_ms - h->t0;
    if (dlt < 0 || dlt % h->period) return h->fail(SWIMSIM_ERANGE, "incarnation %lld is not t0 + e*period", (long long)inc_ms);
    const int64_t q = dlt / h->period;
    if (q >= (int64_t)kMaxEcap) return h->fail(SWIMSIM_ERANGE, "incarnation %lld too far from t0 (at most 2^24 periods)", (long long)inc_ms);
    *e = (uint32_t)q;
    return 0;
}

inline int64_t from_e(const swimsim *h, uint32_t e) { return h->t0 + (int64_t)e * h->period; }

constexpr int64_t kMaxClockOffset = 32767;

int check_clock_offset(swimsim *h, uint32_t o, int64_t k, uint32_t round) {
    if (k > kMaxClockOffset || k < -kMaxClockOffset)
        return h->fail(SWIMSIM_ERANGE, "clock offset of observer %u: %lld periods (at most %lld either way)", o, (long long)k,
                       (long long)kMaxClockOffset);
    if ((int64_t)round + k < 0)
        return h->fail(SWIMSIM_ERANGE, "clock offset of observer %u: %lld periods at round %u puts its clock before t0", o,
                       (long long)k, round);
    return 0;
}

int clock_offset_periods(swimsim *h, uint32_t o, int64_t offset_ms, int64_t *k) {
    if (offset_ms % (int64_t)h->period)
        return h->fail(SWIMSIM_ERANGE, "clock offset of observer %u: %lld ms is not a multiple of the period (%u ms)", o,
                       (long long)offset_ms, h->period);
    *k = offset_ms / (int64_t)h->period;
    return 0;
}

std::vector<uint32_t> canonical_split(uint32_t N, uint32_t G) {
    std::vector<uint32_t> lo(G + 1);
    for (uint32_t r = 0; r <= G; r++) lo[r] = (uint32_t)((uint64_t)N * r / G);
    return lo;
}

int set_shards(swimsim *h, uint32_t G, uint32_t rank, const std::vector<uint32_t> &lo) {
    if (lo[rank] != h->lo || lo[rank + 1] != h->lo + h->NL)
        return h->fail(SWIMSIM_EINVAL, "observer range [%u, %u) is not shard %u of %u ([%u, %u))", h->lo, h->lo + h->NL,
                       rank, G, lo[rank], lo[rank + 1]);
    int rc = 0;
    uint32_t *sl = nullptr;
    h->xcap = (uint32_t)((size_t)h->N * h->K + h->N + 64);
    h->needcap = h->NL * (G - 1) + 64;
    if ((rc = dalloc(h, &sl, G + 1, "shard table")) || (rc = dalloc(h, &h->xitems, h->xcap, "exchange items")) ||
        (rc = dalloc(h, &h->xcnt, 1, "exchange count")) || (rc = dalloc(h, &h->xsz, 6 * G, "exchange sizes")) ||
        (rc = dalloc(h, &h->xseg, 3 * G, "exchange cursors")) || (rc = dalloc(h, &h->xsrcs, G, "exchange sources")) ||
        (rc = dalloc(h, &h->needlist, h->needcap, "need list")) || (rc = dalloc(h, &h->needcnt, 1, "need count")))
        return rc;
    h->xtcur = h->xseg + G;
    h->xdcur = h->xseg + 2 * G;
    HIPCHK(h, hipMemcpy(sl, lo.data(), (G + 1) * 4, hipMemcpyHostToDevice));
    HIPCHK(h, hipMemset(h->xcnt, 0, 4));
    HIPCHK(h, hipMemset(h->needcnt, 0, 4));
    h->G = G;
    h->rank = rank;
    h->shard_lo = lo;
    h->d.G = G;
    h->d.rank = rank;
    h->d.shard_lo = sl;
    return 0;
}

}

extern "C" {

int swimsim_abi_version(void) { return SWIMSIM_ABI_VERSION; }

static thread_local std::string create_err;

const char *swimsim_last_error(swimsim_t *h) {
    if (h) return h->err.c_str();
    return create_err.empty() ? "null handle" : create_err.c_str();
}

int swimsim_create(const swimsim_config *cfg, swimsim_t **out) {
    if (!cfg || !out) return SWIMSIM_EINVAL;
    *out = nullptr;
    swimsim *h = new swimsim();
    create_err.clear();
    auto bail = [&](int rc) {
        create_err = h->err;
        swimsim_destroy(h);
        return rc;
    };
    h->N = cfg->num_members;
    if (h->N < 1 || h->N >= (1u << 24)) return bail(SWIMSIM_EINVAL);
    h->NP = (h->N + 63) & ~63u;
    h->lo = cfg->observer_begin;
    const uint32_t hi_o = cfg->observer_end ? cfg->observer_end : h->N;
    if (h->lo >= hi_o || hi_o > h->N) return bail(SWIMSIM_EINVAL);
    h->NL = hi_o - h->lo;
    h->t0 = cfg->t0_ms ? cfg->t0_ms : 1500000000000ll;
    h->period = cfg->protocol_period_ms ? cfg->protocol_period_ms : 200;
    const uint32_t ts = cfg->suspect_timeout_ms ? cfg->suspect_timeout_ms : 5000;
    const uint32_t tf = cfg->faulty_timeout_ms ? cfg->faulty_timeout_ms : 24u * 3600u * 1000u;
    const uint32_t tt = cfg->tombstone_timeout_ms ? cfg->tombstone_timeout_ms : 60000;
    if (ts % h->period || tf % h->period || tt % h->period) {
        h->err = "state timeouts must be multiples of the protocol period";
        return bail(SWIMSIM_EINVAL);
    }
    h->to_susp = ts / h->period;
    h->to_faulty = tf / h->period;
    h->to_tomb = tt / h->period;
    h->K = cfg->ping_request_size ? cfg->ping_request_size : 3;
    if (h->K > 8) {
        h->err = "ping_request_size " + std::to_string(h->K) + " is above the limit of 8";
        return bail(SWIMSIM_EINVAL);
    }
    h->maxjobs = cfg->max_reverse_full_sync_jobs ? cfg->max_reverse_full_sync_jobs : 5;
    h->pfactor = cfg->p_factor ? cfg->p_factor : 15;
    {
        const uint64_t maxp = (uint64_t)h->pfactor * (uint64_t)digits10((int32_t)std::max<uint32_t>(h->N - 1, 1u));
        if (maxp > 255) {
            h->err = "p_factor " + std::to_string(h->pfactor) + " gives maxP " + std::to_string(maxp) + " at " +
                     std::to_string(h->N) + " members: the 8-bit piggyback counter holds maxP up to 255";
            return bail(SWIMSIM_EINVAL);
        }
    }
    h->seed = cfg->seed;
    h->device = (int)cfg->device;
    h->addrs.resize(h->N);
    if (cfg->addresses) {
        for (uint32_t m = 0; m < h->N; m++) {
            const char *a = cfg->addresses + (size_t)m * cfg->addr_stride;
            h->addrs[m] = std::string(a, strnlen(a, cfg->addr_stride));
        }
        h->W = (uint32_t)h->addrs[0].size();
        for (uint32_t m = 0; m < h->N; m++) {
            if (h->addrs[m].size() != h->W || (m && !(h->addrs[m - 1] < h->addrs[m]))) {
                h->err = "addresses must be fixed-width and strictly ascending";
                return bail(SWIMSIM_EINVAL);
            }
        }
    } else {
        char buf[32];
        for (uint32_t m = 0; m < h->N; m++) {
            snprintf(buf, sizeof buf, "10.%03u.%03u.%03u:7000", (m >> 16) & 255, (m >> 8) & 255, m & 255);
            h->addrs[m] = buf;
        }
        h->W = 19;
    }
    if (h->W < 13 || h->W > 20) {
        h->err = "address width must be 13..20 bytes";
        return bail(SWIMSIM_EINVAL);
    }
#ifdef SWIMSIM_DEV_W19
    if (h->W != 19) {
        h->err = "this library was built with DEV=1 (checksum kernels for 19-byte addresses only)";
        return bail(SWIMSIM_EINVAL);
    }
#endif
    if (hipSetDevice(h->device) != hipSuccess) {
        h->err = "hipSetDevice failed (no usable MI355X device)";
        return bail(SWIMSIM_EHIP);
    }
    if (hipStreamCreateWithFlags(&h->s, hipStreamNonBlocking) != hipSuccess ||
        hipStreamCreateWithFlags(&h->side, hipStreamNonBlocking) != hipSuccess ||
        hipStreamCreateWithFlags(&h->side2, hipStreamNonBlocking) != hipSuccess ||
        hipEventCreateWithFlags(&h->ev_csr2, hipEventDisableTiming) != hipSuccess ||
        hipEventCreateWithFlags(&h->ev_snap, hipEventDisableTiming) != hipSuccess ||
        hipEventCreateWithFlags(&h->ev_side[0], hipEventDisableTiming) != hipSuccess ||
        hipEventCreateWithFlags(&h->ev_side[1], hipEventDisableTiming) != hipSuccess ||
        hipEventCreateWithFlags(&h->ev_rt, hipEventDisableTiming) != hipSuccess) {
        h->err = "hipStreamCreate / hipEventCreate failed";
        return bail(SWIMSIM_EHIP);
    }
    const swimsim_tuning *tun = cfg->tuning;
    if (tun && tun->cs_async >= 0) h->cs_async = tun->cs_async != 0;
    if (tun && tun->cs_narrow_rows >= 0) h->cs_narrow_rows = (uint32_t)tun->cs_narrow_rows;
    if (tun && tun->cs_ref >= 0) h->csr_mode = tun->cs_ref;
    if (tun && tun->fault_inject > 0) h->fault_inject = tun->fault_inject;
    if (tun && tun->defer_test > 0) h->defer_test = tun->defer_test;
    if (tun && tun->cs_defer >= 0) h->cs_defer = tun->cs_defer;
    if (const char *v = getenv("SWIMSIM_CS_DEFER")) h->cs_defer = atoi(v);
    if (const char *v = getenv("SWIMSIM_CS_DEFER_LOG")) h->cs_defer_log = atoi(v) != 0;
    if (h->cs_defer < 0 || h->cs_defer > 2) {
        h->err = "swimsim_tuning.cs_defer is -1, 0, 1 or 2";
        return bail(SWIMSIM_EINVAL);
    }
    if (h->fault_inject & 32) h->csr_ecap = 24;
    if (h->fault_inject & 256) h->csr_side_min = 1024;
    if (const char *v = getenv("SWIMSIM_SYNC_SPIN")) h->sync_spin = atoi(v) != 0;
    if (const char *v = getenv("SWIMSIM_SIDE2"))
        if (atoi(v) == 0 && h->side2) { hipStreamDestroy(h->side2); h->side2 = nullptr; }
    DS &d = h->d;
    d.N = h->N; d.NP = h->NP; d.NL = h->NL; d.lo = h->lo;
    d.NB = h->NP / 64;
    d.NBW = (d.NB + 63) / 64;
    d.NBIT = ((h->NP / 32) + 3) & ~3u;
    d.W = h->W; d.pfactor = h->pfactor; d.K = h->K; d.maxjobs = h->maxjobs;
    d.to_susp = h->to_susp; d.to_faulty = h->to_faulty; d.to_tomb = h->to_tomb;
    d.seed = h->seed;
    const size_t rows = (size_t)h->NL * h->NP;
    int rc = 0;
    if ((rc = dalloc(h, &d.mw, rows, "member words")) || (rc = dalloc(h, &d.dent, rows, "dissemination entries")) ||
        (rc = dalloc(h, &d.tst, rows, "timer states")) ||
        (rc = dalloc(h, &d.tmr, rows, "timers")) ||
        (rc = dalloc(h, &d.ping, h->NL, "ping")) || (rc = dalloc(h, &d.maxp, h->NL, "maxp")) ||
        (rc = dalloc(h, &d.dcnt, h->NL, "dcnt")) || (rc = dalloc(h, &d.dirty, h->NL, "dirty")) ||
        (rc = dalloc(h, &d.cs, h->NL, "cs")) || (rc = dalloc(h, &d.it_idx, h->NL, "it_idx")) ||
        (rc = dalloc(h, &d.it_ep, h->NL, "it_ep")) || (rc = dalloc(h, &d.tmin, h->NL, "tmin")) ||
        (rc = dalloc(h, &d.njobs, h->NL, "njobs")) || (rc = dalloc(h, &d.jobs, (size_t)h->NL * h->maxjobs, "jobs")) ||
        (rc = dalloc(h, &d.dbit, (size_t)h->NL * d.NBIT, "dbit")) || (rc = dalloc(h, &d.tblk, (size_t)h->NL * d.NB, "tblk")) ||
        (rc = dalloc(h, &d.live, h->N, "live")) || (rc = dalloc(h, &d.part, h->N, "part")) ||
        (rc = dalloc(h, &d.coff, h->N, "clock offsets")) ||
        (rc = dalloc(h, &d.ctr, (size_t)CTR_SHARDS * CTR_STRIDE, "counters")) || (rc = dalloc(h, &d.err, 4, "err")) ||
        (rc = dalloc(h, &d.clen, h->NL, "clen")) || (rc = dalloc(h, &d.clast, h->NL, "clast")) ||
        (rc = dalloc(h, &d.cpslot, h->NL, "cpslot")) || (rc = dalloc(h, &d.nhe, h->NL, "cold entry counts")) ||
        (rc = dalloc(h, &d.colx, d.NBIT, "divergent columns")) || (rc = dalloc(h, &d.ucl, h->N, "divergent column list")) ||
        (rc = dalloc(h, &d.uhk, h->N, "divergent column hot slots")) || (rc = dalloc(h, &d.ucold, h->N, "cold divergent columns")) ||
        (rc = dalloc(h, &d.ucnt, 2, "divergent column counts")))
        return bail(rc);
    hipMemset(d.nhe, 0, (size_t)h->NL * 4);
    hipMemset(d.coff, 0, (size_t)h->N * 4);
    h->coff.assign(h->N, 0);
    hipMemset(d.colx, 0xFF, (size_t)d.NBIT * 4);
    hipMemset(d.cpslot, 0xFF, (size_t)h->NL * 4);
    {
        uint32_t hp = std::min<uint32_t>(2048u, h->NP);
        if (tun && tun->hot_slots >= 0) hp = std::min<uint32_t>((uint32_t)tun->hot_slots, h->NP);
        hp = std::min<uint32_t>((hp + 63) & ~63u, RT_MAXSLOTS);
        d.hidx = nullptr; d.hlist = nullptr; d.hmw = nullptr; d.hde = nullptr; d.hotnew = nullptr; d.hot_cnt = nullptr;
        d.HP = 0;
        if (hp) {
            if ((rc = dalloc(h, &d.hidx, h->N, "hot index")) || (rc = dalloc(h, &d.hlist, hp, "hot list")) ||
                (rc = dalloc(h, &d.hmw, (size_t)h->NL * hp, "hot member words")) ||
                (rc = dalloc(h, &d.hde, (size_t)h->NL * hp, "hot dissemination cells")) ||
                (rc = dalloc(h, &d.hotnew, d.NBIT, "hot candidates")) || (rc = dalloc(h, &d.hot_cnt, 2, "hot count")))
                return bail(rc);
            d.HP = hp;
            hot_reset(h, false);
        }
    }
    {
        std::vector<uint32_t> aw((size_t)h->N * 6, 0u);
        for (uint32_t m = 0; m < h->N; m++) {
            uint8_t b[24] = {0};
            memcpy(b, h->addrs[m].data(), h->W);
            for (int w = 0; w < 6; w++)
                aw[(size_t)m * 6 + w] = (uint32_t)b[4 * w] | ((uint32_t)b[4 * w + 1] << 8) | ((uint32_t)b[4 * w + 2] << 16) |
                                        ((uint32_t)b[4 * w + 3] << 24);
        }
        uint32_t *dev = nullptr;
        if ((rc = dalloc(h, &dev, aw.size(), "address words"))) return bail(rc);
        if (hipMemcpy(dev, aw.data(), aw.size() * 4, hipMemcpyHostToDevice) != hipSuccess) return bail(SWIMSIM_EHIP);
        d.addrw = dev;
    }
    if ((rc = build_tail_table(h, cfg->max_rounds ? cfg->max_rounds : 65536))) return bail(rc);
    size_t free_rows = 0, total_rows = 0;
    hipMemGetInfo(&free_rows, &total_rows);
    const uint64_t pool_bound = std::max<uint64_t>(8ull << 30, (uint64_t)(free_rows / 100) * 45) / 16;
    const uint64_t want_records = cfg->message_pool_bytes
                                      ? cfg->message_pool_bytes / 16
                                      : std::min<uint64_t>(std::max<uint64_t>(4ull * h->NL * h->N, 1ull << 20), pool_bound);
    if (want_records < (uint64_t)POOL_SHARDS * h->N) {
        h->err = "message_pool_bytes below 64 sub-pools x N records x 16 bytes";
        return bail(SWIMSIM_EINVAL);
    }
    d.pool_cap = want_records;
    if ((rc = dalloc(h, &d.pool, want_records, "message pool")) || (rc = dalloc(h, &d.pool_cur, POOL_SHARDS * POOL_CUR_STRIDE, "pool cursors")))
        return bail(rc);
    {
        size_t freeb = 0, totalb = 0;
        hipMemGetInfo(&freeb, &totalb);
        const uint64_t by_mem = (uint64_t)(freeb / 3) / (4ull * h->NP);
        d.dense_cap = (uint32_t)std::max<uint64_t>(64, std::min<uint64_t>(2ull * h->NL + 64, by_mem));
        if (tun && tun->dense_slots >= 0)
            d.dense_cap = std::max<uint32_t>(64, std::min<uint32_t>(d.dense_cap, (uint32_t)tun->dense_slots));
        const uint64_t snap_mem = (uint64_t)(freeb / 8) / (4ull * h->NP);
        uint64_t async_rows = CS_ASYNC_ROWS;
        if (tun && tun->cs_async_rows >= 0) async_rows = (uint64_t)tun->cs_async_rows;
        h->snap_cap = h->cs_async ? (uint32_t)std::min<uint64_t>(std::min<uint64_t>(async_rows, h->NL), snap_mem) : 0u;
        h->side_halves = h->snap_cap && snap_mem >= 2ull * h->snap_cap && !(h->fault_inject & 1024) ? 2u : 1u;
    }
    const size_t nslots = (size_t)d.dense_cap + (size_t)h->side_halves * h->snap_cap;
    if ((rc = dalloc(h, &d.dense, nslots * h->NP, "dense snapshots")) ||
        (rc = dalloc(h, &d.dense_meta, nslots, "dense meta")) || (rc = dalloc(h, &d.dense_cur, 1, "dense cursor")) ||
        (rc = dalloc(h, &d.dense_len, nslots, "dense len")) || (rc = dalloc(h, &d.dense_last, nslots, "dense last")) ||
        (rc = dalloc(h, &d.dense_cs, nslots, "dense cs")) ||
        (rc = dalloc(h, &h->side_ids, (size_t)h->side_halves * std::max<uint32_t>(h->snap_cap, 1), "side ids")) ||
        (rc = dalloc(h, &h->side_cnt, 2, "side count")))
        return bail(rc);
    const size_t NLK = (size_t)h->NL * h->K, NK = (size_t)h->N * h->K;
    h->keycap = (uint32_t)(NK + 64);
    const size_t KC = h->keycap;
    if ((rc = dalloc(h, &h->tgt, h->NL, "tgt")) || (rc = dalloc(h, &h->failed, h->NL, "failed")) ||
        (rc = dalloc(h, &h->sdesc, h->N, "sdesc")) || (rc = dalloc(h, &h->rdesc, h->N, "rdesc")) ||
        (rc = dalloc(h, &h->sdesc2, h->N, "sdesc2")) || (rc = dalloc(h, &h->rdesc2, NK, "rdesc2")) ||
        (rc = dalloc(h, &h->snapdesc, h->N, "snapdesc")) || (rc = dalloc(h, &h->hdesc, 10, "hdesc")) ||
        (rc = dalloc(h, &h->sI, h->N, "sI")) || (rc = dalloc(h, &h->sC, h->N, "sC")) ||
        (rc = dalloc(h, &h->sI2, h->N, "sI2")) || (rc = dalloc(h, &h->sC2, h->N, "sC2")) ||
        (rc = dalloc(h, &h->sS, h->N, "sS")) || (rc = dalloc(h, &h->sS2, h->N, "sS2")) ||
        (rc = dalloc(h, &h->rcs, h->N, "rcs")) || (rc = dalloc(h, &h->csreq, KC, "csreq")) ||
        (rc = dalloc(h, &h->csreqcnt, 1, "csreqcnt")) ||
        (rc = dalloc(h, &h->fpv, h->NL, "fpv")) || (rc = dalloc(h, &h->fpv_s, h->NL, "fpv_s")) ||
        (rc = dalloc(h, &h->fph, h->NL, "fph")) || (rc = dalloc(h, &h->fph_s, h->NL, "fph_s")) ||
        (rc = dalloc(h, &h->fplist, h->NL, "fplist")) || (rc = dalloc(h, &h->fpcnt, 1, "fpcnt")) ||
        (rc = dalloc(h, &h->dup_of, h->NL, "dup_of")) || (rc = dalloc(h, &h->hflag, h->NL, "hflag")) || (rc = dalloc(h, &h->d.fp, h->NL, "fp")) ||
        (rc = dalloc(h, &h->H, NLK, "H")) || (rc = dalloc(h, &h->nh, h->NL, "nh")) ||
        (rc = dalloc(h, &h->keys, KC, "keys")) || (rc = dalloc(h, &h->keys_sorted, KC, "keys_sorted")) ||
        (rc = dalloc(h, &h->keys_in, KC, "receivers")) || (rc = dalloc(h, &h->vals_out, KC, "vals_out")) ||
        (rc = dalloc(h, &h->pinfo, (size_t)KC * 2, "inbox pair snapshots")) ||
        (rc = dalloc(h, &h->ukeys, KC, "ukeys")) || (rc = dalloc(h, &h->counts, KC, "counts")) ||
        (rc = dalloc(h, &h->offs, KC, "offs")) || (rc = dalloc(h, &h->nruns, 1, "nruns")) ||
        (rc = dalloc(h, &h->info, 8, "info")) || (rc = dalloc(h, &h->list, 3 * KC + 2 * (size_t)h->NL + 64, "list")) ||
        (rc = dalloc(h, &h->cnt, 2, "cnt")) || (rc = dalloc(h, &h->defer, KC + 2 * (size_t)h->NL + 64, "defer")) ||
        (rc = dalloc(h, &h->defer_eq, KC + 2 * (size_t)h->NL + 64, "defer eq")) ||
        (rc = dalloc(h, &h->rep_tab, (size_t)rep_slots(h->NL), "checksum representatives")) ||
        (rc = dalloc(h, &h->fp_tab, (size_t)rep_slots(h->NL) * 4, "dedup groups")) ||
        (rc = dalloc(h, &h->d.ulog, (size_t)h->NL * ULOG_STRIDE, "receive-phase undo log")) ||
        (rc = dalloc(h, &h->d.ulog_cnt, (size_t)h->NL, "receive-phase undo log counts")) ||
        (rc = dalloc(h, &h->d.ilen, (size_t)h->NL, "issue-time checksum lengths")) ||
        (rc = dalloc(h, &h->d.ilast, (size_t)h->NL, "issue-time last members")) ||
        (rc = dalloc(h, &h->defer_cnt, 1, "defer_cnt")) || (rc = dalloc(h, &h->exh_list, h->NL, "exh_list")) ||
        (rc = dalloc(h, &h->exh_cnt, 1, "exh_cnt")) || (rc = dalloc(h, &h->scratch, (size_t)64 * (h->NP / 32), "scratch")) ||
        (rc = dalloc(h, &h->need, h->N, "need")) || (rc = dalloc(h, &h->digest_buf, 4, "digest")) ||
        (rc = dalloc(h, &h->fsflag, KC, "fsflag")) || (rc = dalloc(h, &h->hsics, 4, "hsics")) ||
        (rc = dalloc(h, &h->npairs, 1, "npairs")))
        return bail(rc);
    h->rep_mask = (h->defer_test & 16) ? 0u : rep_slots(h->NL) - 1u;
    h->d.ulog_stride = ULOG_STRIDE;
    h->d.ulog_cap = (h->defer_test & 8) ? 2u : ULOG_CAP;
    h->d.defer_test = (uint32_t)h->defer_test;
    hipMemset(h->rep_tab, 0, (size_t)rep_slots(h->NL) * 8);
    h->evcap = 4 * h->N + 64;
    if ((rc = dalloc(h, &h->evbuf, h->evcap, "events")) || (rc = dalloc(h, &h->ev_applied, h->evcap, "ev_applied")))
        return bail(rc);
    {
        size_t b1 = 0, b2 = 0, b3 = 0, b4 = 0, b5 = 0;
        hipcub::DeviceRadixSort::SortKeys(nullptr, b1, h->keys, h->keys_sorted, (int)KC, 0, 64);
        hipcub::DeviceRunLengthEncode::Encode(nullptr, b2, h->keys_in, h->ukeys, h->counts, h->nruns, (int)KC);
        hipcub::DeviceScan::ExclusiveSum(nullptr, b3, h->counts, h->offs, (int)KC);
        hipcub::DeviceRadixSort::SortPairs(nullptr, b4, h->keys, h->keys_sorted, h->fpv, h->fpv_s, (int)h->NL, 0, 64);
        hipcub::DeviceScan::InclusiveScan(nullptr, b5, h->fph, h->fph_s, hipcub::Max(), (int)h->NL);
        size_t b6 = 0;
        hipcub::DeviceRadixSort::SortKeys(nullptr, b6, h->fplist, h->list, (int)h->NL, 0, 32);
        h->cub_bytes = std::max(std::max(std::max(b1, b6), std::max(b2, b3)), std::max(b4, b5));
        if ((rc = dalloc(h, (uint8_t **)&h->cub_tmp, h->cub_bytes, "cub temp"))) return bail(rc);
    }
    {
        uint32_t *sl = nullptr;
        if ((rc = dalloc(h, &sl, 2, "shard table"))) return bail(rc);
        const uint32_t t2[2] = {0, h->N};
        if (hipMemcpy(sl, t2, 8, hipMemcpyHostToDevice) != hipSuccess) return bail(SWIMSIM_EHIP);
        h->shard_lo = {0, h->N};
        d.G = 1; d.rank = 0; d.shard_lo = sl;
    }
    if (hipHostMalloc((void **)&h->hinfo, 128, 0) != hipSuccess) return bail(SWIMSIM_ENOMEM);
    hipMemset(d.ctr, 0, (size_t)CTR_SHARDS * CTR_STRIDE * 8);
    hipMemset(d.err, 0, 4);
    hipMemset(h->need, 0, h->N);
    hipMemset(h->fsflag, 0, KC);
    hipMemset(h->sS, 0xFF, h->N * 4);
    hipMemset(h->hflag, 0, h->NL);
    hipMemset(h->sS2, 0xFF, h->N * 4);
    hipMemset(d.njobs, 0, h->NL * 4);
    h->live.assign(h->N, 1);
    h->part.assign(h->N, 0);
    if (upload_topology(h) || hipStreamSynchronize(h->s) != hipSuccess) return bail(SWIMSIM_EHIP);
    if (h->csr_mode != 0 && h->N >= 1024 && h->NL > h->cs_narrow_rows && h->NL >= CSD_MIN_ROWS) (void)csr_alloc(h);
    if (h->csr_mode != 0 && h->N >= 1024 && h->cs_async && h->snap_cap >= h->csr_side_min && !(h->fault_inject & 128)) {
        const uint32_t rcap = h->N <= 131072 ? 1024u : 512u;
        const uint64_t kp = ((uint64_t)h->N * (h->W + 32) + 256) / 20 + 2;
        const uint64_t need = (uint64_t)h->snap_cap * ((uint64_t)h->csr_ecap * 32 + rcap * sizeof(CsrRec) + 64) +
                              kp * 20 * 32 + (uint64_t)h->N * 64 + (64ull << 20);
        size_t fr = 0, tot = 0;
        if (hipMemGetInfo(&fr, &tot) == hipSuccess && fr > need && fr - need >= tot / 100 * 12)
            (void)csr_alloc(h, h->csr2, h->snap_cap);
    }
    if (hipGetLastError() != hipSuccess) return bail(SWIMSIM_EHIP);
    *out = h;
    return SWIMSIM_OK;
}

int swimsim_destroy(swimsim_t *h) {
    if (!h) return SWIMSIM_OK;
    if (h->side) hipStreamSynchronize(h->side);
    if (h->side2) hipStreamSynchronize(h->side2);
    if (h->s) hipStreamSynchronize(h->s);
    for (auto &t : h->pending) { hipEventDestroy(t.a); hipEventDestroy(t.b); }
    for (auto e : h->round_ev) hipEventDestroy(e);
    for (auto e : h->evpool) hipEventDestroy(e);
    for (void *p : h->allocs) hipFree(p);
    if (h->sbuf) hipFree(h->sbuf);
    if (h->rbuf) hipFree(h->rbuf);
    h->xp.reset();
    if (h->hinfo) hipHostFree(h->hinfo);
    if (h->ev_snap) hipEventDestroy(h->ev_snap);
    if (h->ev_rt) hipEventDestroy(h->ev_rt);
    for (hipEvent_t e : h->ev_side)
        if (e) hipEventDestroy(e);
    if (h->side) hipStreamDestroy(h->side);
    if (h->side2) hipStreamDestroy(h->side2);
    if (h->ev_csr2) hipEventDestroy(h->ev_csr2);
    for (hipEvent_t e : h->cn_ev)
        if (e) hipEventDestroy(e);
    for (hipEvent_t e : h->rt_ev)
        if (e) hipEventDestroy(e);
    if (h->s) hipStreamDestroy(h->s);
    delete h;
    return SWIMSIM_OK;
}

static int init_rows(swimsim_t *h, int mode) {
    hot_reset(h, false);
    hipLaunchKernelGGL(k_init_rows, dim3(blocks_for_waves(h->NL)), dim3(SWIM_WAVE_BLOCK), 0, h->s, h->d, mode, 0u);
    HIPCHK(h, hipMemsetAsync(h->d.colx, mode == 0 ? 0 : 0xFF, (size_t)h->d.NBIT * 4, h->s));
    h->colx_stale = mode != 0;
    if (int rc = checksum_dirty(h, 0)) return rc;
    return check_err(h);
}

int swimsim_init_converged(swimsim_t *h) { return h ? init_rows(h, 0) : SWIMSIM_EINVAL; }
int swimsim_init_self_only(swimsim_t *h) { return h ? init_rows(h, 1) : SWIMSIM_EINVAL; }


int swimsim_set_member(swimsim_t *h, uint32_t o, uint32_t m, int32_t status, int64_t inc_ms) {
    if (!h || !own(h, o) || m >= h->N) return SWIMSIM_EINVAL;
    if (!(status >= 0 && status <= 4) && status != SWIMSIM_UNKNOWN) return SWIMSIM_EINVAL;
    uint32_t e = 0;
    if (status != SWIMSIM_UNKNOWN) {
        if (int rc = to_e(h, inc_ms, &e)) return rc;
        if (int rc = ensure_ecap(h, e)) return rc;
    }
    const uint32_t w = (e << 3) | (uint32_t)status;
    HIPCHK(h, hipMemsetAsync(h->d.colx, 0xFF, (size_t)h->d.NBIT * 4, h->s));
    h->colx_stale = true;
    hot_reset(h, true);
    HIPCHK(h, hipMemcpyAsync(h->d.mw + (size_t)(o - h->lo) * h->NP + m, &w, 4, hipMemcpyHostToDevice, h->s));
    hipLaunchKernelGGL(k_recount, dim3(1), dim3(64), 0, h->s, h->d, o - h->lo);
    HIPCHK(h, stream_sync(h));
    return SWIMSIM_OK;
}

int swimsim_set_row(swimsim_t *h, uint32_t o, const uint8_t *status, const int64_t *inc_ms) {
    if (!h || !own(h, o) || !status || !inc_ms) return SWIMSIM_EINVAL;
    std::vector<uint32_t> row(h->NP, (uint32_t)SWIMSIM_UNKNOWN);
    uint32_t emax = 0;
    for (uint32_t m = 0; m < h->N; m++) {
        const int32_t s = status[m];
        if (s == SWIMSIM_UNKNOWN) continue;
        if (s > 4) return h->fail(SWIMSIM_EINVAL, "member %u: status %d", m, s);
        uint32_t e;
        if (int rc = to_e(h, inc_ms[m], &e)) return rc;
        row[m] = (e << 3) | (uint32_t)s;
        emax = std::max(emax, e);
    }
    if (int rc = ensure_ecap(h, emax)) return rc;
    HIPCHK(h, hipMemsetAsync(h->d.colx, 0xFF, (size_t)h->d.NBIT * 4, h->s));
    h->colx_stale = true;
    hot_reset(h, true);
    HIPCHK(h, hipMemcpyAsync(h->d.mw + (size_t)(o - h->lo) * h->NP, row.data(), (size_t)h->N * 4,
                             hipMemcpyHostToDevice, h->s));
    hipLaunchKernelGGL(k_recount, dim3(1), dim3(64), 0, h->s, h->d, o - h->lo);
    HIPCHK(h, stream_sync(h));
    return SWIMSIM_OK;
}

int swimsim_make_change(swimsim_t *h, uint32_t o, uint32_t m, int64_t inc_ms, int32_t status) {
    if (!h || !own(h, o) || m >= h->N || status < 0 || status > 4) return SWIMSIM_EINVAL;
    uint32_t e;
    if (int rc = to_e(h, inc_ms, &e)) return rc;
    if (int rc = ensure_ecap(h, e)) return rc;
    std::vector<uint4> b{make_uint4(1, o, m, e | ((uint32_t)status << 29))};
    if (int rc = flush_events(h, b)) return rc;
    uint32_t applied = 0;
    HIPCHK(h, hipMemcpyAsync(&applied, h->ev_applied, 4, hipMemcpyDeviceToHost, h->s));
    HIPCHK(h, stream_sync(h));
    return (int)applied;
}

int swimsim_clear_changes(swimsim_t *h, uint32_t o) {
    if (!h || !own(h, o)) return SWIMSIM_EINVAL;
    hipLaunchKernelGGL(k_clear_changes, dim3(1), dim3(256), 0, h->s, h->d, o - h->lo);
    HIPCHK(h, stream_sync(h));
    return SWIMSIM_OK;
}

int swimsim_add_join_list(swimsim_t *h, uint32_t o, const int32_t *member, const int32_t *status, const int64_t *inc_ms,
                          const int32_t *source, const int64_t *source_inc_ms, size_t n, uint32_t *applied) {
    if (!h || !own(h, o) || (n && (!member || !status || !inc_ms))) return SWIMSIM_EINVAL;
    if (n > h->N) return h->fail(SWIMSIM_EINVAL, "join list of %zu changes for %u members", n, h->N);
    std::vector<uint4> rec(n);
    std::vector<uint8_t> seen(h->N, 0);
    uint32_t emax = 0;
    for (size_t i = 0; i < n; i++) {
        const int32_t m = member[i], st = status[i];
        if (m < 0 || (uint32_t)m >= h->N) return h->fail(SWIMSIM_EINVAL, "join list change %zu: member %d", i, m);
        if (st < 0 || st > 4) return h->fail(SWIMSIM_EINVAL, "join list change %zu: status %d", i, st);
        if (seen[m]++) return h->fail(SWIMSIM_EINVAL, "join list names member %d twice (MembershipAsChanges lists each once)", m);
        uint32_t e = 0, se = 0, src = SRC_NONE;
        if (int rc = to_e(h, inc_ms[i], &e)) return rc;
        if (source && source[i] >= 0) {
            if ((uint32_t)source[i] >= h->N) return h->fail(SWIMSIM_EINVAL, "join list change %zu: source %d", i, source[i]);
            src = (uint32_t)source[i];
            if (source_inc_ms)
                if (int rc = to_e(h, source_inc_ms[i], &se)) return rc;
        }
        emax = std::max(emax, e);
        rec[i] = make_uint4((uint32_t)m | ((uint32_t)st << 24), e, src, se);
    }
    if (int rc = ensure_ecap(h, std::max(emax, h->round + (uint32_t)h->coff_max) + 1)) return rc;
    if (!h->jl)
        if (int rc = dalloc(h, &h->jl, h->N, "join list")) return rc;
    uint32_t napp = 0;
    if (n) {
        HIPCHK(h, hipMemcpyAsync(h->jl, rec.data(), n * sizeof(uint4), hipMemcpyHostToDevice, h->s));
        hipLaunchKernelGGL(k_add_join_list, dim3(1), dim3(64), 0, h->s, h->d, o - h->lo, h->jl, (uint32_t)n, h->round,
                           h->ev_applied);
        HIPCHK(h, hipMemcpyAsync(&napp, h->ev_applied, 4, hipMemcpyDeviceToHost, h->s));
    }
    HIPCHK(h, stream_sync(h));
    if (applied) *applied = napp;
    return check_err(h);
}

int swimsim_set_live(swimsim_t *h, uint32_t m, int32_t live) {
    if (!h || m >= h->N) return SWIMSIM_EINVAL;
    h->live[m] = live ? 1 : 0;
    return upload_topology(h);
}

int swimsim_set_partition(swimsim_t *h, uint32_t m, int32_t label) {
    if (!h || m >= h->N) return SWIMSIM_EINVAL;
    h->part[m] = label;
    return upload_topology(h);
}

int swimsim_set_round(swimsim_t *h, uint32_t r) {
    if (!h) return SWIMSIM_EINVAL;
    if ((int64_t)r + h->coff_min < 0)
        return h->fail(SWIMSIM_ERANGE, "round %u puts a clock before t0 (an offset of %d periods is in force)", r, h->coff_min);
    h->round = r;
    return ensure_ecap(h, r + (uint32_t)h->coff_max + 1);
}

int swimsim_set_clock_offset(swimsim_t *h, uint32_t o, int64_t offset_ms) {
    if (!h || o >= h->N) return SWIMSIM_EINVAL;
    int64_t k = 0;
    if (int rc = clock_offset_periods(h, o, offset_ms, &k)) return rc;
    if (int rc = check_clock_offset(h, o, k, h->round)) return rc;
    if (int rc = ensure_ecap(h, h->round + (uint32_t)std::max<int64_t>(k, h->coff_max) + 1)) return rc;
    h->coff[o] = (int32_t)k;
    clock_offset_range(h);
    HIPCHK(h, hipMemcpyAsync(h->d.coff + o, &h->coff[o], 4, hipMemcpyHostToDevice, h->s));
    HIPCHK(h, stream_sync(h));
    return SWIMSIM_OK;
}

int swimsim_set_clock_offsets(swimsim_t *h, const int64_t *offset_ms) {
    if (!h || !offset_ms) return SWIMSIM_EINVAL;
    std::vector<int32_t> ks(h->N);
    int64_t kmax = 0;
    for (uint32_t o = 0; o < h->N; o++) {
        int64_t k = 0;
        if (int rc = clock_offset_periods(h, o, offset_ms[o], &k)) return rc;
        if (int rc = check_clock_offset(h, o, k, h->round)) return rc;
        ks[o] = (int32_t)k;
        kmax = std::max(kmax, k);
    }
    if (int rc = ensure_ecap(h, h->round + (uint32_t)kmax + 1)) return rc;
    h->coff.swap(ks);
    clock_offset_range(h);
    HIPCHK(h, hipMemcpyAsync(h->d.coff, h->coff.data(), (size_t)h->N * 4, hipMemcpyHostToDevice, h->s));
    HIPCHK(h, stream_sync(h));
    return SWIMSIM_OK;
}

int swimsim_clock_offsets(swimsim_t *h, int64_t *out) {
    if (!h || !out) return SWIMSIM_EINVAL;
    for (uint32_t o = 0; o < h->N; o++) out[o] = (int64_t)h->coff[o] * (int64_t)h->period;
    return SWIMSIM_OK;
}

static int agree_ecap(swimsim *h) {
    if (h->G == 1 || dynamic_cast<LocalPort *>(h->xp.get())) return 0;
    std::vector<uint64_t> send(h->G, h->ecap), recv(h->G);
    if (int rc = h->xp->sizes(send.data(), recv.data(), 1)) return h->fail(rc, "shard table exchange failed (%s)", h->xp->name());
    const uint64_t want = *std::max_element(recv.begin(), recv.end());
    if (want > kMaxEcap) return h->fail(SWIMSIM_ERANGE, "a shard reports a checksum table of %llu steps", (unsigned long long)want);
    return ensure_ecap(h, (uint32_t)want - 1);
}

int swimsim_step(swimsim_t *h, uint32_t nrounds, const swimsim_event *events, size_t nevents) {
    if (!h) return SWIMSIM_EINVAL;
    if (h->G == 1 && h->NL != h->N) return h->fail(SWIMSIM_EINVAL, "a partial observer range needs a shard transport");
    int32_t ev_kmax = 0;
    for (size_t i = 0; i < nevents; i++) {
        const swimsim_event &e = events[i];
        if (e.kind != SWIMSIM_EV_CLOCK || e.round < h->round || e.round - h->round >= nrounds) continue;
        if (e.a < 0 || (uint32_t)e.a >= h->N) return h->fail(SWIMSIM_EINVAL, "event member %d out of range", e.a);
        if (int rc = check_clock_offset(h, (uint32_t)e.a, e.b, e.round)) return rc;
        ev_kmax = std::max(ev_kmax, e.b);
    }
    if (nrounds)
        if (int rc = agree_ecap(h)) return rc;
    if (h->colx_stale && nrounds) {
        if (h->side_pending) return h->fail(SWIMSIM_EINVAL, "internal: divergent-column rebuild with side checksums pending");
        hipLaunchKernelGGL(k_colx_rebuild, dim3(blocks_for_threads(h->NP)), dim3(256), 0, h->s, h->d);
        h->colx_stale = false;
    }
    for (uint32_t i = 0; i < nrounds; i++) {
        if (int rc = ensure_ecap(h, h->round + (uint32_t)std::max(h->coff_max, ev_kmax) + 1)) return rc;
        if (int rc = step_one(h, events, nevents, nrounds - 1 - i)) return rc;
    }
    h->rounds_left = 0;
    if (h->cs_carried)
        if (int rc = checksum_dirty(h, 0)) return rc;
    if (int rc = sync_side(h)) return rc;
    if (!h->round_ev.empty()) {
        hipEvent_t e = take_event(h);
        HIPCHK(h, hipEventRecord(e, h->s));
        h->round_ev.push_back(e);
    }
    if (int rc = check_err(h)) return rc;
    for (size_t i = 0; i + 1 < h->round_ev.size(); i++) {
        float ms = 0;
        hipEventElapsedTime(&ms, h->round_ev[i], h->round_ev[i + 1]);
        if (h->round_ms.size() < (1u << 20)) h->round_ms.push_back(ms);
    }
    for (hipEvent_t e : h->round_ev) h->evpool.push_back(e);
    h->round_ev.clear();
    drain_timing(h);
    return SWIMSIM_OK;
}

int swimsim_heal(swimsim_t *h, uint32_t o, int32_t *targets, size_t cap, size_t *ntargets) {
    if (!h || !own(h, o)) return SWIMSIM_EINVAL;
    if (h->G > 1) return h->fail(SWIMSIM_EINVAL, "sharded clusters heal through SWIMSIM_EV_HEAL events (collective)");
    std::vector<int32_t> ret;
    HIPCHK(h, hipMemsetAsync(h->d.pool_cur, 0, POOL_SHARDS * POOL_CUR_STRIDE * 8, h->s));
    if (int rc = do_heal(h, o, &ret)) return rc;
    if (int rc = check_err(h)) return rc;
    if (targets)
        for (size_t i = 0; i < ret.size() && i < cap; i++) targets[i] = ret[i];
    if (ntargets) *ntargets = ret.size();
    return SWIMSIM_OK;
}

uint32_t swimsim_round(swimsim_t *h) { return h ? h->round : 0; }
// ... 906 lines not shown
```

### ringpop-go_amd/csrc/swimsim_kernels.hip

```cpp
#include "swimsim_kernels.h"

namespace swimdev {

#define SWIM_DPP(old, src, ctrl, rm) ((uint32_t)__builtin_amdgcn_update_dpp((int)(old), (int)(src), (ctrl), (rm), 0xf, false))
template <typename Op>
__device__ __forceinline__ uint32_t dpp_scan(uint32_t x, uint32_t id, Op op) {
    x = op(x, SWIM_DPP(id, x, 0x111, 0xf));
    x = op(x, SWIM_DPP(id, x, 0x112, 0xf));
    x = op(x, SWIM_DPP(id, x, 0x114, 0xf));
    x = op(x, SWIM_DPP(id, x, 0x118, 0xf));
    x = op(x, SWIM_DPP(id, x, 0x142, 0xa));
    x = op(x, SWIM_DPP(id, x, 0x143, 0xc));
    return x;
}
__device__ __forceinline__ uint32_t dpp_scan_add(uint32_t x) { return dpp_scan(x, 0u, [](uint32_t a, uint32_t b) { return a + b; }); }
__device__ __forceinline__ uint32_t dpp_scan_umin(uint32_t x) {
    return dpp_scan(x, 0xFFFFFFFFu, [](uint32_t a, uint32_t b) { return min(a, b); });
}
__device__ __forceinline__ int32_t dpp_scan_imax(int32_t x) {
    return (int32_t)dpp_scan((uint32_t)x, 0x80000000u, [](uint32_t a, uint32_t b) { return (uint32_t)max((int32_t)a, (int32_t)b); });
}
__device__ __forceinline__ int32_t dpp_scan_imin(int32_t x) {
    return (int32_t)dpp_scan((uint32_t)x, 0x7FFFFFFFu, [](uint32_t a, uint32_t b) { return (uint32_t)min((int32_t)a, (int32_t)b); });
}
// ... 747 lines not shown
                     ((v[u].w & 7u) != ST_UNKNOWN);
        }
    }
    known = wsum(known);
    if (lane_id() == 0) {
        d.dense_meta[slot] = make_uint4(o, d.mw[(size_t)ol * d.NP + o] >> 3, (uint32_t)known, 0);
        d.dense_len[slot] = d.clen[ol];
        d.dense_last[slot] = d.clast[ol];
    }
    out.kind = 1; out.off_lo = slot; out.len = (uint32_t)known;
    return true;
}

__global__ void k_init_rows(DS d, int mode, uint32_t e0) {
    const uint32_t ol = wave_gid();
    if (ol >= d.NL) return;
    const uint32_t o = d.lo + ol;
    unsigned long long fp = 0;
    for (uint32_t m = lane_id(); m < d.NP; m += 64) {
        const size_t idx = (size_t)ol * d.NP + m;
        uint32_t w = ST_UNKNOWN;
        if (m < d.N && (mode == 0 || m == o)) w = (e0 << 3) | ST_ALIVE;
        if (m < d.N) fp += fpmix(m, w);
        d.mw[idx] = w;
        d.dent[idx] = make_uint2(DE_NONE, 0);
        d.tst[idx] = 0;
        d.tmr[idx] = make_uint2(NO_DEADLINE, 0);
    }
    for (uint32_t b = lane_id(); b < d.NB; b += 64) d.tblk[(size_t)ol * d.NB + b] = NO_DEADLINE;
    for (uint32_t b = lane_id(); b < d.NBIT; b += 64) d.dbit[(size_t)ol * d.NBIT + b] = 0;
#pragma unroll
    for (int off = 32; off > 0; off >>= 1) fp += __shfl_xor(fp, off, 64);
    if (lane_id() == 0) {
        d.fp[ol] = fp;
        const int32_t p = mode == 0 ? (int32_t)d.N - 1 : 0;
        const uint32_t rl = (uint32_t)reclen(d, ST_ALIVE, e0);
        d.clen[ol] = mode == 0 ? rl * d.N : rl;
        d.clast[ol] = mode == 0 ? (int32_t)d.N - 1 : (int32_t)o;
        d.ping[ol] = p;
        d.maxp[ol] = mode == 0 ? (int32_t)d.pfactor * digits10(p) : (int32_t)d.pfactor;
        d.dcnt[ol] = 0;
        d.nhe[ol] = 0;
        d.dirty[ol] = 1;
        d.cs[ol] = 0;
        d.it_idx[ol] = -1;
        d.it_ep[ol] = 0;
        d.tmin[ol] = NO_DEADLINE;
        d.njobs[ol] = 0;
    }
}

__global__ void k_recount(DS d, uint32_t ol) {
    const uint32_t o = d.lo + ol;
    int p = 0, c = 0, len = 0, last = -1;
    unsigned long long fp = 0;
    for (uint32_t m = lane_id(); m < d.N; m += 64) {
        const size_t idx = (size_t)ol * d.NP + m;
        const uint32_t w = d.mw[idx];
        fp += fpmix(m, w);
        if (m != o && is_pingable(w & 7u)) p++;
        if (de_p(d.dent[idx].x) != DP_NONE) c++;
        len += reclen(d, w & 7u, w >> 3);
        if ((w & 7u) < 4u) last = (int)m;
    }
    p = wsum(p);
    c = wsum(c);
    len = wsum(len);
    last = wmax(last);
#pragma unroll
    for (int off = 32; off > 0; off >>= 1) fp += __shfl_xor(fp, off, 64);
    if (lane_id() == 0) {
        d.ping[ol] = p; d.dcnt[ol] = c; d.dirty[ol] = 1; d.clen[ol] = (uint32_t)len; d.clast[ol] = last; d.fp[ol] = fp;
        d.nhe[ol] = c;
    }
}

__global__ void k_clear_changes(DS d, uint32_t ol) {
    for (uint32_t m = threadIdx.x; m < d.NP; m += blockDim.x) d.dent[(size_t)ol * d.NP + m].x = DE_NONE;
    if (d.hidx)
        for (uint32_t k = threadIdx.x; k < d.HP; k += blockDim.x) d.hde[(size_t)ol * d.HP + k].x = DE_NONE;
    for (uint32_t b = threadIdx.x; b < d.NBIT; b += blockDim.x) d.dbit[(size_t)ol * d.NBIT + b] = 0;
    if (threadIdx.x == 0) {
        d.dcnt[ol] = 0;
        d.nhe[ol] = 0;
    }
}

__global__ void k_nhe_reset(DS d) {
    const uint32_t ol = blockIdx.x * blockDim.x + threadIdx.x;
    if (ol < d.NL) d.nhe[ol] = d.dcnt[ol];
}

__global__ void __launch_bounds__(1024) k_hot_extend(DS d) {
    __shared__ uint32_t n;
    if (threadIdx.x == 0) {
        n = d.hot_cnt[0];
        d.hot_cnt[1] = n;
    }
    __syncthreads();
    for (uint32_t w = threadIdx.x; w < d.NBIT; w += blockDim.x) {
        uint32_t bits = d.hotnew[w];
        if (!bits) continue;
        d.hotnew[w] = 0;
        while (bits) {
            const uint32_t m = w * 32 + (uint32_t)(__ffs(bits) - 1);
            bits &= bits - 1;
            if (m >= d.N || d.hidx[m] != SRC_NONE) continue;
            const uint32_t k = atomicAdd(&n, 1u);
            if (k < d.HP) {
                d.hidx[m] = k;
                d.hlist[k] = m;
            }
        }
    }
    __syncthreads();
    if (threadIdx.x == 0) d.hot_cnt[0] = min(n, d.HP);
}

__global__ void k_hot_fill(DS d) {
    const uint32_t ol = wave_gid();
    if (ol >= d.NL) return;
    const uint32_t k0 = d.hot_cnt[1], k1 = d.hot_cnt[0];
    const size_t rb = (size_t)ol * d.NP, hb = (size_t)ol * d.HP;
    int nowhot = 0;
    for (uint32_t k = k0 + lane_id(); k < k1; k += 64 * MB) {
        uint32_t m[MB], w[MB];
        uint2 cell[MB];
#pragma unroll
        for (int u = 0; u < MB; u++) m[u] = k + 64u * u < k1 ? d.hlist[k + 64u * u] : 0u;
#pragma unroll
        for (int u = 0; u < MB; u++) {
            cell[u] = d.dent[rb + m[u]];
            w[u] = d.mw[rb + m[u]];
        }
#pragma unroll
        for (int u = 0; u < MB; u++) {
            if (k + 64u * u >= k1) continue;
            d.hmw[hb + k + 64u * u] = w[u];
            d.hde[hb + k + 64u * u] = cell[u];
            nowhot += de_p(cell[u].x) != DP_NONE;
        }
    }
    if (k1 > k0) {
        nowhot = wsum(nowhot);
        if (lane_id() == 0 && nowhot) d.nhe[ol] -= nowhot;
    }
}

__global__ void k_hot_flush(DS d, uint32_t ol0, uint32_t nrows) {
    const uint32_t i = wave_gid();
    if (i >= nrows) return;
    const uint32_t ol = ol0 + i, k1 = d.hot_cnt[0];
    const size_t rb = (size_t)ol * d.NP, hb = (size_t)ol * d.HP;
    for (uint32_t k = lane_id(); k < k1; k += 64) d.dent[rb + d.hlist[k]] = d.hde[hb + k];
}

__global__ void k_add_join_list(DS d, uint32_t ol, const uint4 *__restrict__ rec, uint32_t n, uint32_t r,
                                uint32_t *applied_out) {
    const uint32_t o = d.lo + ol;
    const uint32_t now = wave_clock(d, o, r);
    const uint32_t *rowp = d.mw + (size_t)ol * d.NP;
    MAcc acc;
    acc_begin(d, ol, acc);
    for (uint32_t base = 0; base < n; base += 64 * MB) {
        uint4 c[MB];
        uint32_t cur[MB];
#pragma unroll
        for (int u = 0; u < MB; u++) {
            const uint32_t i = base + u * 64 + lane_id();
            c[u] = i < n ? rec[i] : make_uint4(0xFFFFFFFFu, 0, 0, 0);
        }
#pragma unroll
        for (int u = 0; u < MB; u++) cur[u] = c[u].x != 0xFFFFFFFFu ? rowp[c[u].x & 0xFFFFFFu] : 0u;
#pragma unroll
        for (int u = 0; u < MB; u++) {
            if (c[u].x == 0xFFFFFFFFu) continue;
            const uint32_t m = c[u].x & 0xFFFFFFu;
            const int before = acc.napp;
            merge_change_w(d, ol, o, m, cur[u], c[u].x >> 24, c[u].y, c[u].z, c[u].w, now, now, acc);
            if (acc.napp != before && m != o) {
                const size_t idx = (size_t)ol * d.NP + m;
                d.dent[idx].x = DE_NONE;
                const uint32_t hk = hot_slot(d, m);
                if (hk != SRC_NONE) d.hde[(size_t)ol * d.HP + hk].x = DE_NONE;
                else acc.dnh--;
                atomicAnd(&d.dbit[(size_t)ol * d.NBIT + (m >> 5)], ~(1u << (m & 31)));
                acc.ddc--;
            }
        }
    }
    const int napp = wsum(acc.napp);
    __threadfence_block();
    wave_finalize(d, ol, acc, 2);
    if (lane_id() == 0) *applied_out = (uint32_t)napp;
}

__device__ int thread_make_change(const DS &d, uint32_t ol, uint32_t o, uint32_t m, uint32_t e, uint32_t st, uint32_t now) {
    MAcc acc;
    acc_begin(d, ol, acc);
    const uint32_t self_e = d.mw[(size_t)ol * d.NP + o] >> 3;
    merge_change(d, ol, o, m, st, e, o, self_e, now, now, acc);
    fold_row(d, ol, acc.dping, acc.ddc, acc.napp, acc.nref, 0, acc.dlen, acc.maxlast, acc.inval, acc.dfp, true, acc.dnh);
    return acc.napp;
}

__global__ void k_events(DS d, const uint4 *ev, uint32_t nev, uint32_t r, uint32_t *applied_out) {
    if (threadIdx.x != 0 || blockIdx.x != 0) return;
    for (uint32_t i = 0; i < nev; i++) {
        const uint4 e = ev[i];
        const uint32_t kind = e.x, o = e.y;
        if (kind == 5) {
            d.coff[o] = (int32_t)e.w;
            if (applied_out) applied_out[i] = 0;
            continue;
        }
        if (o < d.lo || o >= d.lo + d.NL) continue;
        const uint32_t ol = o - d.lo;
        const uint32_t now = clock_of(d, o, r);
        int applied = 0;
        switch (kind) {
        case 1:
            applied = thread_make_change(d, ol, o, e.z, e.w & 0x1FFFFFFFu, e.w >> 29, now);
            break;
        case 2:
            applied = thread_make_change(d, ol, o, o, now, ST_ALIVE, now);
            break;
        case 3:
            applied = thread_make_change(d, ol, o, o, d.mw[(size_t)ol * d.NP + o] >> 3, ST_LEAVE, now);
            break;
        case 4:
            for (uint32_t m = 0; m < d.N; m++) {
                const uint32_t w = d.mw[(size_t)ol * d.NP + m];
                if ((w & 7u) == ST_FAULTY) applied += thread_make_change(d, ol, o, m, w >> 3, ST_TOMB, now);
            }
            break;
        }
        if (applied_out) applied_out[i] = (uint32_t)applied;
    }
}

__global__ void k_timers(DS d, uint32_t round) {
    const uint32_t ol = wave_gid();
    if (ol >= d.NL) return;
    const uint32_t o = d.lo + ol;
    const uint32_t r = wave_clock(d, o, round);
    if (!d.live[o] || d.tmin[ol] > r) return;
    const uint32_t self_e = d.mw[(size_t)ol * d.NP + o] >> 3;
    MAcc acc;
    const unsigned long long tbase = d.useq ? d.useq[ol] : 0ull;
    uint32_t newmin = NO_DEADLINE;
    int fired = 0;
    for (uint32_t b0 = 0; b0 < d.NB; b0 += 64) {
        const uint32_t bl = b0 + lane_id();
        const uint32_t bm = bl < d.NB ? d.tblk[(size_t)ol * d.NB + bl] : NO_DEADLINE;
        unsigned long long due = __ballot(bm <= r);
        if (bm > r) newmin = min(newmin, bm);
        while (due) {
            const uint32_t bb = __ffsll((long long)due) - 1;
            due &= due - 1;
            const uint32_t b = b0 + bb;
            const uint32_t m = (b << 6) + lane_id();
            const size_t idx = (size_t)ol * d.NP + m;
            const uint8_t ts = d.tst[idx];
            const uint32_t state = ts & 7u;
            uint2 a = d.tmr[idx];
            if (state && !(ts & 0x80) && a.x <= r) {
                d.tst[idx] = ts | 0x80;
                fired++;
                acc.tag = tbase + ((0xFFFFull - min(r - a.x, 0xFFFFu)) << 24) + m;
                if (state == ST_SUSPECT) merge_change(d, ol, o, m, ST_FAULTY, a.y, o, self_e, r, a.x, acc);
                else if (state == ST_FAULTY) merge_change(d, ol, o, m, ST_TOMB, a.y, o, self_e, r, a.x, acc);
                else {
                    const uint32_t w = d.mw[idx];
                    if ((w & 7u) != ST_UNKNOWN && m != o) {
                        if (is_pingable(w & 7u)) acc.dping--;
                        d.mw[idx] = (w & ~7u) | ST_UNKNOWN;
                        colmark(d, m);
                        const uint32_t hk = hot_slot(d, m);
                        if (hk != SRC_NONE) d.hmw[(size_t)ol * d.HP + hk] = (w & ~7u) | ST_UNKNOWN;
                        track_len(d, ol, m, w, (w & ~7u) | ST_UNKNOWN, acc);
                        acc.dfp += fpmix(m, (w & ~7u) | ST_UNKNOWN) - fpmix(m, w);
                        acc.evict++;
                    }
                }
                a = d.tmr[idx];
            }
            const uint8_t ts2 = d.tst[idx];
            const uint32_t v = ((ts2 & 7u) && !(ts2 & 0x80)) ? a.x : NO_DEADLINE;
            const uint32_t bmin = wmin(v);
            if (lane_id() == 0) d.tblk[(size_t)ol * d.NB + b] = bmin;
            newmin = min(newmin, bmin);
        }
    }
    newmin = wmin(newmin);
    if (lane_id() == 0) d.tmin[ol] = newmin;
    fired = wsum(fired);
    if (lane_id() == 0 && fired) ctr_add(d, C_TIMERS_FIRED, (unsigned long long)fired);
    const int napp_t = wsum(acc.napp);
    if (lane_id() == 0 && napp_t && d.useq) d.useq[ol] = tbase + (1ull << 40);
    __threadfence_block();
    wave_finalize(d, ol, acc, 0, false);
}

__global__ void k_select(DS d, int32_t *tgt, uint32_t *exh_list, uint32_t *exh_cnt) {
    const uint32_t ol = blockIdx.x * blockDim.x + threadIdx.x;
    if (ol >= d.NL) return;
    const uint32_t o = d.lo + ol;
    int32_t target = -1;
    if (d.live[o]) {
        if (d.ping[ol] <= 0) {
            exh_list[atomicAdd(exh_cnt, 1u)] = ol;
        } else {
            int32_t idx = d.it_idx[ol];
            uint32_t ep = d.it_ep[ol];
            Feistel f;
            f.init(d.seed, o, ep, d.N);
            const uint32_t *row = d.mw + (size_t)ol * d.NP;
            for (uint32_t guard = 0; guard < 4 * d.N + 8; guard++) {
                idx++;
                if (idx >= (int32_t)d.N) { idx = 0; ep++; f.init(d.seed, o, ep, d.N); }
                const uint32_t m = f.perm((uint32_t)idx, d.N);
                const uint32_t st = row[m] & 7u;
                if (st == ST_UNKNOWN) continue;
                if (m != o && is_pingable(st)) { target = (int32_t)m; break; }
            }
            if (target < 0) atomicOr(d.err, E_ITER);
            d.it_idx[ol] = idx;
            d.it_ep[ol] = ep;
        }
    }
    tgt[ol] = target;
}

__global__ void k_select_exhaust(DS d, const uint32_t *exh_list, const uint32_t *exh_cnt, uint32_t *scratch) {
    const uint32_t cnt = *exh_cnt;
    uint32_t *vis = scratch + (size_t)blockIdx.x * (d.NP / 32);
    for (uint32_t q = blockIdx.x; q < cnt; q += gridDim.x) {
        const uint32_t ol = exh_list[q], o = d.lo + ol;
        for (uint32_t i = threadIdx.x; i < d.NP / 32; i += blockDim.x) vis[i] = 0;
        __syncthreads();
        if (threadIdx.x == 0) {
            const uint32_t *row = d.mw + (size_t)ol * d.NP;
            uint32_t known = 0;
            for (uint32_t m = 0; m < d.N; m++) known += (row[m] & 7u) != ST_UNKNOWN;
            int32_t idx = d.it_idx[ol];
            uint32_t ep = d.it_ep[ol], nvis = 0;
            Feistel f;
            f.init(d.seed, o, ep, d.N);
            uint64_t guard = 0;
            while (nvis < known && guard++ < 8ull * d.N + 8) {
                idx++;
                if (idx >= (int32_t)d.N) { idx = 0; ep++; f.init(d.seed, o, ep, d.N); }
                const uint32_t m = f.perm((uint32_t)idx, d.N);
                if ((row[m] & 7u) == ST_UNKNOWN) continue;
                if (!(vis[m >> 5] & (1u << (m & 31)))) { vis[m >> 5] |= 1u << (m & 31); nvis++; }
            }
            d.it_idx[ol] = idx;
            d.it_ep[ol] = ep;
        }
        __syncthreads();
    }
}

__global__ void k_list(DS d, int mode, const int32_t *tgt, const uint8_t *failed, uint32_t *list, uint32_t *cnt) {
    const uint32_t ol = blockIdx.x * blockDim.x + threadIdx.x;
    if (ol >= d.NL) return;
    const uint32_t dv = d.dirty[ol];
    bool take = dv != 0;
    if (mode == 1) take = take && tgt[ol] >= 0;
    if (mode == 2) take = take && failed[ol];
    if (take) list[atomicAdd(cnt, 1u)] = ol;
    if (take && mode == 0) d.cpslot[ol] = SRC_NONE;
    if (mode == 0) {
        const unsigned long long fresh = __ballot(dv == 1u);
        if (fresh && lane_id() == 0) atomicAdd(cnt + 1, (uint32_t)__popcll(fresh));
    }
}

__global__ void k_carry(DS d) {
    const uint32_t ol = blockIdx.x * blockDim.x + threadIdx.x;
    if (ol < d.NL && d.dirty[ol]) d.dirty[ol] = DIRTY_CARRIED;
}

__global__ void k_list_one(uint32_t *list, uint32_t *cnt, uint32_t ol, const DS d) {
    if (threadIdx.x == 0) { *cnt = d.dirty[ol] ? 1u : 0u; list[0] = ol; }
}

__global__ void k_issue(DS d, int mode, const int32_t *tgt, const uint8_t *failed, MsgDesc *sdesc, uint32_t *sI,
                        uint32_t *sC, uint32_t *sS) {
    const uint32_t ol = wave_gid();
    if (ol >= d.NL) return;
    const uint32_t o = d.lo + ol;
    if ((mode == 0 && tgt[ol] < 0) || (mode == 1 && !failed[ol])) {
        if (sS && lane_id() == 0) sS[o] = SRC_NONE;
        return;
    }
    const uint32_t dirty = d.dirty[ol], cpslot = d.cpslot[ol], cs = d.cs[ol], selfw = d.mw[(size_t)ol * d.NP + o];
    const uint32_t clen = d.clen[ol];
    const int32_t clast = d.clast[ol];
    MsgDesc md;
    wave_issue(d, ol, md);
    uint32_t slot = SRC_NONE;
    if (sS && dirty && !d.ulog) {
        MsgDesc sn;
        if (wave_snapshot(d, ol, o, sn)) slot = sn.off_lo;
        if (lane_id() == 0) ctr_add(d, C_X_ISSUE_SNAPS, 1ull);
    } else if (sS && dirty) {
        slot = SRC_PEND;
        if (lane_id() == 0) { d.ilen[ol] = clen; d.ilast[ol] = clast; }
    } else if (sS) {
        slot = cpslot;
    }
    if (lane_id() == 0) {
        sdesc[o] = md;
        sI[o] = selfw >> 3;
        sC[o] = slot == SRC_NONE ? cs : 0u;
        if (sS) sS[o] = slot;
        if (mode == 0) {
            ctr_add(d, C_PINGS, 1ull);
            ctr_add(d, C_MSG_CHANGES, (unsigned long long)md.len);
        }
        ctr_add(d, C_X_ISSUED, (unsigned long long)md.len);
    }
}

__device__ __forceinline__ void x_push(uint4 *items, uint32_t *cnt, uint32_t cap, uint32_t *err, uint4 it) {
    const uint32_t i = atomicAdd(cnt, 1u);
    if (i < cap) items[i] = it;
    else atomicOr(err, E_XCAP);
}

__global__ void k_pairs_direct(DS d, const int32_t *tgt, unsigned long long *keys, uint8_t *failed, uint32_t *info,
                               uint4 *xitems, uint32_t *xcnt, uint32_t xcap) {
    const uint32_t ol = blockIdx.x * blockDim.x + threadIdx.x;
    if (ol >= d.NL) return;
    const uint32_t o = d.lo + ol;
    const int32_t t = tgt[ol];
    unsigned long long key = (unsigned long long)d.N << 32;
    uint8_t f = 0;
    if (t >= 0) {
        if (!reach(d, o, (uint32_t)t)) {
            f = 1;
            atomicAdd(&info[2], 1u);
        } else if (d.G > 1 && owner_of(d, (uint32_t)t) != d.rank) {
            x_push(xitems, xcnt, xcap, d.err, make_uint4(owner_of(d, (uint32_t)t), 1u , o, (uint32_t)t));
        } else {
            key = ((unsigned long long)(uint32_t)t << 32) | o;
        }
    }
    keys[ol] = key;
    failed[ol] = f;
}

__global__ void k_helpers(DS d, const int32_t *tgt, const uint8_t *failed, uint32_t *H, uint32_t *nh, uint32_t r) {
    const uint32_t ol = blockIdx.x * blockDim.x + threadIdx.x;
    if (ol >= d.NL) return;
    nh[ol] = 0;
    if (!failed[ol]) return;
    const uint32_t o = d.lo + ol, t = (uint32_t)tgt[ol], K = d.K;
    const uint32_t *row = d.mw + (size_t)ol * d.NP;
    ctr_add(d, C_PINGREQS, 1ull);
    const int32_t eligible = d.ping[ol] - (is_pingable(row[t] & 7u) ? 1 : 0);
    const uint32_t need = (uint32_t)max(0, min((int32_t)K, eligible));
    uint32_t got = 0, h[8];
    U4 blk = U4{0, 0, 0, 0};
    for (uint32_t i = 0; i < 64 && got < need; i++) {
        if ((i & 3) == 0) blk = philox10(r, o, 2u, i >> 2, d.seed);
        const uint32_t c = mulhi_n(pick(blk, i), d.N);
        if (c == o || c == t || !is_pingable(row[c] & 7u)) continue;
        bool dup = false;
        for (uint32_t q = 0; q < got; q++) dup |= h[q] == c;
        if (!dup) h[got++] = c;
    }
    if (got < need) {
        const uint32_t start = mulhi_n(philox10(r, o, 2u, 16u, d.seed).x, d.N);
        for (uint32_t q = 0; q < d.N && got < need; q++) {
            uint32_t c = start + q;
            if (c >= d.N) c -= d.N;
            if (c == o || c == t || !is_pingable(row[c] & 7u)) continue;
            bool dup = false;
            for (uint32_t z = 0; z < got; z++) dup |= h[z] == c;
            if (!dup) h[got++] = c;
        }
    }
    for (uint32_t q = 0; q < got; q++) H[(size_t)ol * K + q] = h[q];
    nh[ol] = got;
}

__global__ void k_pairs_helpers(DS d, const uint8_t *failed, const uint32_t *H, const uint32_t *nh,
                                unsigned long long *keys, uint4 *xitems, uint32_t *xcnt, uint32_t xcap) {
    const uint32_t i = blockIdx.x * blockDim.x + threadIdx.x;
    const uint32_t K = d.K;
    if (i >= d.NL * K) return;
    const uint32_t ol = i / K, q = i % K, o = d.lo + ol;
    unsigned long long key = (unsigned long long)d.N << 32;
    if (failed[ol] && q < nh[ol]) {
        const uint32_t h = H[i];
        if (reach(d, o, h)) {
            if (d.G > 1 && owner_of(d, h) != d.rank)
                x_push(xitems, xcnt, xcap, d.err, make_uint4(owner_of(d, h), 2u , o * K + q, h));
            else
                key = ((unsigned long long)h << 32) | (o * K + q);
        }
    }
    keys[i] = key;
}

__global__ void k_split_keys(const unsigned long long *keys, uint32_t n, uint32_t *recv, uint32_t *vals) {
    const uint32_t i = blockIdx.x * blockDim.x + threadIdx.x;
    if (i >= n) return;
    const unsigned long long k = keys[i];
    recv[i] = (uint32_t)(k >> 32);
    vals[i] = (uint32_t)k;
}

__global__ void k_runs_info(const uint32_t *ukeys, const uint32_t *counts, const uint32_t *nruns, uint32_t N,
                            uint32_t *info) {
    const uint32_t i = blockIdx.x * blockDim.x + threadIdx.x;
    if (i >= *nruns) return;
    if (ukeys[i] == N) return;
    atomicMax(&info[1], counts[i]);
    atomicAdd(&info[0], 1u);
}

struct RecvArgs {
    const uint32_t *ukeys, *counts, *offs, *vals;
    const uint4 *pinfo;
    uint32_t nruns_max;
    int phase;
    const MsgDesc *sdesc;
    const uint32_t *sI, *sC;
    uint32_t *sS;
    MsgDesc *rdesc;
    uint4 *defer;
    uint32_t *defer_cnt;
    uint8_t *fsflag;
    uint32_t r;
};

__global__ void k_pair_info(const DS d, const uint32_t *vals, uint32_t n, int phase, const MsgDesc *sdesc, const uint32_t *sI,
                            const uint32_t *sC, const uint32_t *sS, uint4 *pinfo) {
    const uint32_t i = blockIdx.x * blockDim.x + threadIdx.x;
    if (d.ulog_cnt && i < d.NL) d.ulog_cnt[i] = 0u;
    if (i >= n) return;
    const uint32_t v = vals[i], sender = phase == 0 ? v : v / d.K;
    if (sender >= d.N) return;
    const MsgDesc md = sdesc[sender];
    pinfo[2 * (size_t)i] = make_uint4(md.off_lo, md.off_hi, md.len, md.kind);
    pinfo[2 * (size_t)i + 1] = make_uint4(sI[sender], sC[sender], sS ? sS[sender] : SRC_NONE, v);
}

__device__ __forceinline__ void recv_one_pre(const DS &d, const RecvArgs &a, uint32_t j, const uint4 pi0, const uint4 pi1,
                                             uint32_t pair, uint32_t nslots, uint32_t now, RowPre &p, LazyCtx &lz) {
    const uint32_t ol = j - d.lo;
    const uint32_t v = pi1.w, sender = a.phase == 0 ? v : v / d.K, resp_idx = v;
    MsgDesc md;
    md.off_lo = pi0.x; md.off_hi = pi0.y; md.len = pi0.z; md.kind = pi0.w;
    const uint64_t bound = (uint64_t)(uint32_t)p.dcnt + md.len;
    const bool early = md.kind == 0 && bound > 0 && bound <= min(4096ull, d.pool_cap / POOL_SHARDS / 16);
    unsigned long long roff = 0;
    if (early && lane_id() == 0) roff = pool_alloc_lane0(d, (uint32_t)bound);
    wave_merge_msg_pre(d, ol, j, md, now, now, 0, p, -1, nullptr, true, &lz);
    MsgDesc resp;
    resp.kind = 0; resp.len = 0; resp.off_lo = resp.off_hi = 0;
    uint32_t kept = 0;
    const uint32_t cnt = (uint32_t)p.dcnt;
    if (cnt) {
        const unsigned long long off = early ? bcast64(roff) : pool_alloc(d, cnt);
        if (off != ~0ull) {
            int del = 0, delnh = 0;
            kept = wave_issue_body<true>(d, ol, sender, pi1.x, resp, cnt, p.maxp, d.hidx && p.nhe == 0, nslots, off, del,
                                         delnh);
            if (del) { p.dcnt -= del; if (lane_id() == 0) d.dcnt[ol] = p.dcnt; }
            if (delnh) { p.nhe -= delnh; if (lane_id() == 0) d.nhe[ol] = p.nhe; }
            __threadfence_block();
        }
    }
    if (lane_id() == 0) {
        ctr_add(d, C_X_RISSUED, (unsigned long long)kept);
        ctr_add(d, C_X_RCALLS, 1ull);
    }
    if (kept == 0) {
        const uint32_t scs = pi1.y;
        const uint32_t sslot = a.sS ? pi1.z : SRC_NONE;
        const bool rdirty = p.dirty != 0;
        const uint32_t rpend = rdirty ? SRC_NONE : p.cpslot;
        if (rdirty || rpend != SRC_NONE || sslot != SRC_NONE) {
            if (wave_snapshot(d, ol, j, resp) && lane_id() == 0) {
                if (rpend != SRC_NONE) d.dense_meta[resp.off_lo].w = rpend + 1u;
                else if (!rdirty) d.dense_cs[resp.off_lo] = p.cs;
                a.defer[atomicAdd(a.defer_cnt, 1u)] =
                    make_uint4(resp_idx | (rdirty ? 0x80000000u : 0u), resp.off_lo, sslot != SRC_NONE ? sslot : scs,
                               pair | (sslot != SRC_NONE ? 0x80000000u : 0u));
            }
            resp.kind = 2;
        } else if (p.cs != scs) {
            wave_snapshot(d, ol, j, resp);
            if (lane_id() == 0) {
                if (a.phase == 0) a.fsflag[pair] = 1;
                ctr_add(d, a.phase == 0 ? C_FULL_SYNCS : C_FULL_SYNCS_PINGREQ, 1ull);
            }
        }
    }
    if (lane_id() == 0) {
        a.rdesc[resp_idx] = resp;
        if (resp.kind != 2) ctr_add(d, C_MSG_CHANGES, (unsigned long long)resp.len);
        if (a.phase == 1) {
            ctr_add(d, C_HELPER_CALLS, 1ull);
            ctr_add(d, C_MSG_CHANGES, (unsigned long long)md.len);
        }
    }
}

constexpr int RECV_MIN_WAVES = 4;
__global__ void __launch_bounds__(256, RECV_MIN_WAVES) k_recv(DS d, RecvArgs a) {
    const uint32_t u = wave_gid();
    if (u >= a.nruns_max) return;
    const uint32_t key = a.ukeys[u];
    if (key >= d.N) return;
    const uint32_t n = a.counts[u], off = a.offs[u];
    RowPre p = row_pre(d, key - d.lo);
    const uint32_t now = wave_clock(d, key, a.r);
    const uint32_t nslots = d.hidx ? d.hot_cnt[0] : 0u;
    LazyCtx lz;
    lz.sS = a.sS; lz.sI = a.sI;
    lz.pend = a.sS && d.ulog && uni(a.sS[key]) == SRC_PEND;
    for (uint32_t w = 0; w < n; w++) {
        const uint32_t pair = off + w;
        recv_one_pre(d, a, key, a.pinfo[2 * (size_t)pair], a.pinfo[2 * (size_t)pair + 1], pair, nslots, now, p, lz);
    }
    if (d.ulog_cnt && lane_id() == 0) d.ulog_cnt[key - d.lo] = min(p.ulog, d.ulog_cap + 1u);
}

__global__ void k_colx_rebuild(DS d) {
    const uint32_t m = blockIdx.x * blockDim.x + threadIdx.x;
    bool diff = false;
    if (m < d.N) {
        const uint32_t w0 = d.mw[m];
        for (uint32_t ol = 1; ol < d.NL && !diff; ol++) diff = d.mw[(size_t)ol * d.NP + m] != w0;
    }
    const unsigned long long bits = __ballot(diff);
    const uint32_t w = (m & ~63u) >> 5;
    if (lane_id() == 0) {
        if (w < d.NBIT) d.colx[w] = (uint32_t)bits;
        if (w + 1 < d.NBIT) d.colx[w + 1] = (uint32_t)(bits >> 32);
    }
}

__global__ void __launch_bounds__(1024) k_ucols(DS d) {
    __shared__ uint32_t part[1024];
    __shared__ uint32_t ncold;
    const uint32_t t = threadIdx.x, per = (d.NBIT + 1023) / 1024, w0 = t * per;
    if (t == 0) ncold = 0;
    auto bitsof = [&](uint32_t w) -> uint32_t {
        const uint32_t x = d.colx[w], lo = w * 32;
        return lo + 32 <= d.N ? x : lo >= d.N ? 0u : x & ((1u << (d.N - lo)) - 1u);
    };
    uint32_t c = 0;
    for (uint32_t w = w0; w < min(w0 + per, d.NBIT); w++) c += (uint32_t)__popc(bitsof(w));
    part[t] = c;
    __syncthreads();
    for (uint32_t off = 1; off < 1024; off <<= 1) {
        const uint32_t v = t >= off ? part[t - off] : 0u;
        __syncthreads();
        part[t] += v;
        __syncthreads();
    }
    uint32_t at = part[t] - c;
    for (uint32_t w = w0; w < min(w0 + per, d.NBIT); w++) {
        uint32_t bits = bitsof(w);
        while (bits) {
            const uint32_t m = w * 32 + (uint32_t)__builtin_ctz(bits);
            bits &= bits - 1;
            const uint32_t k = hot_slot(d, m);
            d.ucl[at] = m;
            d.uhk[at] = k;
            if (k == SRC_NONE) d.ucold[atomicAdd(&ncold, 1u)] = m;
            at++;
        }
    }
    __syncthreads();
    if (t == 0) {
        d.ucnt[0] = part[1023];
        d.ucnt[1] = ncold;
    }
}

__device__ bool wave_rows_differ(const DS &d, const uint32_t *a, const uint32_t *b, const uint32_t *ha, const uint32_t *hb) {
    const uint32_t lane = lane_id();
    bool diff = false;
    const uint32_t nu = d.ucnt[0];
    if (nu <= d.N / 4) {
        if (ha && hb) {
            const uint32_t nh = d.hot_cnt[0], nc = d.ucnt[1];
            for (uint32_t k0 = 0; k0 < nh && !__any(diff); k0 += 64 * MB) {
                uint32_t x[MB], y[MB];
#pragma unroll
                for (int u = 0; u < MB; u++) {
                    const uint32_t k = k0 + u * 64 + lane;
                    x[u] = k < nh ? ha[k] : 0u;
                    y[u] = k < nh ? hb[k] : 0u;
                }
#pragma unroll
                for (int u = 0; u < MB; u++) diff |= x[u] != y[u];
            }
            for (uint32_t c0 = 0; c0 < nc && !__any(diff); c0 += 64 * MB) {
                uint32_t x[MB], y[MB];
#pragma unroll
                for (int u = 0; u < MB; u++) {
                    const uint32_t c = c0 + u * 64 + lane;
                    const uint32_t m = c < nc ? d.ucold[c] : 0u;
                    x[u] = c < nc ? a[m] : 0u;
                    y[u] = c < nc ? b[m] : 0u;
                }
#pragma unroll
                for (int u = 0; u < MB; u++) diff |= x[u] != y[u];
            }
        } else {
            for (uint32_t c0 = 0; c0 < nu && !__any(diff); c0 += 64 * MB) {
                uint32_t x[MB], y[MB];
#pragma unroll
                for (int u = 0; u < MB; u++) {
                    const uint32_t c = c0 + u * 64 + lane;
                    const uint32_t m = c < nu ? d.ucl[c] : 0u;
                    x[u] = c < nu ? a[m] : 0u;
                    y[u] = c < nu ? b[m] : 0u;
                }
#pragma unroll
                for (int u = 0; u < MB; u++) diff |= x[u] != y[u];
            }
        }
    } else {
        const uint4 *a4 = (const uint4 *)a, *b4 = (const uint4 *)b;
        for (uint32_t base = 0; base < d.NP / 4 && !__any(diff); base += 64 * MB) {
            uint4 x[MB], y[MB];
#pragma unroll
            for (int u = 0; u < MB; u++) {
                const uint32_t k = base + u * 64 + lane;
                x[u] = k < d.NP / 4 ? a4[k] : make_uint4(0, 0, 0, 0);
                y[u] = k < d.NP / 4 ? b4[k] : make_uint4(0, 0, 0, 0);
            }
#pragma unroll
            for (int u = 0; u < MB; u++) diff |= x[u].x != y[u].x || x[u].y != y[u].y || x[u].z != y[u].z || x[u].w != y[u].w;
        }
    }
    return __any(diff);
}

__device__ bool wave_rows_differ_undo(const DS &d, const uint32_t *a, const uint32_t *b, const uint2 *log, uint32_t nlog,
                                      bool &done, bool full = false) {
    const uint32_t lane = lane_id();
    const bool bycol = d.ucnt[0] <= d.N / 4;
    const uint32_t nu = bycol ? d.ucnt[0] : d.N;
    done = bycol || full;
    if (!done) return true;
    bool diff = false;
    for (uint32_t c0 = 0; c0 < nu && !__any(diff); c0 += 64 * MB) {
        uint32_t m[MB], x[MB], y[MB];
#pragma unroll
        for (int u = 0; u < MB; u++) {
            const uint32_t c = c0 + u * 64 + lane;
            m[u] = c >= nu ? 0xFFFFFFFEu : bycol ? d.ucl[c] : c;
            x[u] = c < nu ? a[m[u]] : 0u;
            y[u] = c < nu ? b[m[u]] : 0u;
        }
        for (int k0 = nlog ? (int)((nlog - 1u) & ~63u) : -1; k0 >= 0; k0 -= 64) {
            const uint2 L = (uint32_t)k0 + lane < nlog ? log[(uint32_t)k0 + lane] : make_uint2(0xFFFFFFFFu, 0u);
            for (int k = (int)min(64u, nlog - (uint32_t)k0) - 1; k >= 0; k--) {
                const uint32_t lm = (uint32_t)__builtin_amdgcn_readlane((int)L.x, k);
                const uint32_t lw = (uint32_t)__builtin_amdgcn_readlane((int)L.y, k);
#pragma unroll
                for (int u = 0; u < MB; u++) y[u] = m[u] == lm ? lw : y[u];
            }
        }
#pragma unroll
        for (int u = 0; u < MB; u++) diff |= x[u] != y[u];
    }
    return __any(diff);
}

__device__ __forceinline__ uint32_t rep_hash(uint32_t cs, uint32_t mask) { return fmix32(cs ^ 0x9E3779B9u) & mask; }
__global__ void k_cs_reps(DS d, const uint32_t *defer_cnt, unsigned long long *tab, uint32_t mask, uint32_t gen) {
    const uint32_t ol = blockIdx.x * blockDim.x + threadIdx.x;
    if (*defer_cnt == 0 || ol >= d.NL) return;
    if (d.dirty[ol] || d.cpslot[ol] != SRC_NONE) return;
    const uint32_t cs = d.cs[ol];
    tab[rep_hash(cs, mask)] = ((unsigned long long)gen << 56) | ((unsigned long long)ol << 32) | cs;
}
__device__ __forceinline__ uint32_t rep_find(const DS &d, const unsigned long long *tab, uint32_t mask, uint32_t gen,
                                             uint32_t cs) {
    const unsigned long long cur = tab[rep_hash(cs, mask)];
    if ((uint32_t)(cur >> 56) != gen || (uint32_t)cur != cs) return SRC_NONE;
    const uint32_t r = (uint32_t)(cur >> 32) & 0xFFFFFFu;
    return r < d.NL && !d.dirty[r] && d.cpslot[r] == SRC_NONE && d.cs[r] == cs ? r : SRC_NONE;
}

__device__ __forceinline__ uint32_t lazy_slot(uint32_t z, const uint32_t *sS, uint32_t sender) {
    return z == SRC_PEND && sS ? sS[sender] : z;
}

__global__ void k_defer_eq(DS d, const uint4 *defer, const uint32_t *defer_cnt, int phase, uint8_t *eq,
                           const unsigned long long *tab, uint32_t mask, uint32_t gen, const uint32_t *sS) {
    const uint32_t i = wave_gid();
    if (i >= *defer_cnt) return;
    const uint4 e = defer[i];
    const uint32_t ri = e.x & 0x7FFFFFFFu, sender = phase == 1 ? ri / d.K : ri;
    const uint32_t *srow = nullptr;
    bool viarep = false, pendlive = false;
    const uint32_t dt = d.defer_test;
    if (phase != 2) {
        if (e.w & 0x80000000u) {
            const uint32_t z = lazy_slot(e.z, sS, sender);
            if (z == SRC_PEND) pendlive = true;
            else if (!(z & 0x80000000u) && z != SRC_CLAIM) srow = d.dense + (size_t)z * d.NP;
        } else if (!(dt & 1u) && sender >= d.lo && sender < d.lo + d.NL && !d.dirty[sender - d.lo]) {
            srow = d.mw + (size_t)(sender - d.lo) * d.NP;
        } else if (tab && !(dt & 2u)) {
            const uint32_t r = rep_find(d, tab, mask, gen, e.z);
            if (r != SRC_NONE) {
                srow = d.mw + (size_t)r * d.NP;
                viarep = true;
            }
        }
    }
    bool same = false, viaundo = false, over = false;
    if (srow) {
        same = !wave_rows_differ(d, d.dense + (size_t)e.y * d.NP, srow, nullptr, nullptr);
    } else if (pendlive) {
        const uint32_t sl = sender - d.lo;
        bool done = false;
        same = !wave_rows_differ_undo(d, d.dense + (size_t)e.y * d.NP, d.mw + (size_t)sl * d.NP,
                                      d.ulog + (size_t)sl * d.ulog_stride, min(d.ulog_cnt[sl], d.ulog_cap), done, true);
    } else if (phase != 2 && !(e.w & 0x80000000u) && d.ulog && !(dt & 4u) && sender >= d.lo && sender < d.lo + d.NL) {
        const uint32_t sl = sender - d.lo, nlog = d.ulog_cnt[sl];
        over = nlog > d.ulog_cap;
        if (!over) {
            bool done = false;
            const bool differ = wave_rows_differ_undo(d, d.dense + (size_t)e.y * d.NP, d.mw + (size_t)sl * d.NP,
                                                      d.ulog + (size_t)sl * d.ulog_stride, nlog, done);
            viaundo = done;
            same = done && !differ;
        }
    }
    if (lane_id() == 0) {
        eq[i] = same ? 1 : 0;
        ctr_add(d, C_X_DEFER, 1ull);
        if (same) ctr_add(d, viarep ? C_X_DEFER_REP : viaundo ? C_X_DEFER_UNDO : C_X_DEFER_EQ, 1ull);
        else if (viarep || viaundo) ctr_add(d, viarep ? C_X_DEFER_REP_DIFF : C_X_DEFER_UNDO_DIFF, 1ull);
        if (!srow && !viaundo && !pendlive) ctr_add(d, C_X_DEFER_NOROW, 1ull);
        if (over) ctr_add(d, C_X_DEFER_UNDO_OVER, 1ull);
        if (!(e.w & 0x80000000u)) ctr_add(d, C_X_DEFER_CLEAN, 1ull);
    }
}

__global__ void k_lazy_mat(DS d, const uint4 *defer, const uint8_t *eq, const uint4 *req, const uint32_t *cnt, uint32_t cap,
                           int phase, uint32_t *sS, const uint32_t *sI) {
    const uint32_t i = wave_gid();
    if (i >= *cnt || i >= cap) return;
    uint32_t sender;
    if (req) {
        if (req[i].y != SRC_PEND) return;
        sender = req[i].x;
    } else {
        const uint4 e = defer[i];
        if (eq[i] || !(e.w & 0x80000000u) || e.z != SRC_PEND) return;
        const uint32_t ri = e.x & 0x7FFFFFFFu;
        sender = phase == 1 ? ri / d.K : ri;
    }
    if (sender < d.lo || sender >= d.lo + d.NL) return;
    uint32_t won = 0;
    if (lane_id() == 0) won = atomicCAS(&sS[sender], SRC_PEND, SRC_CLAIM) == SRC_PEND;
    if (!__builtin_amdgcn_readlane((int)won, 0)) return;
    const uint32_t sl = sender - d.lo;
    const uint32_t slot = wave_rebuild_issue_row(d, sl, sender, sI[sender], min(d.ulog_cnt[sl], d.ulog_cap));
    if (lane_id() == 0) {
        if (slot != SRC_NONE) sS[sender] = slot;
        ctr_add(d, C_X_LAZY_MAT, 1ull);
    }
}

__global__ void k_recv_finish(DS d, const uint4 *defer, const uint32_t *defer_cnt, MsgDesc *rdesc, int phase,
                              uint8_t *fsflag, const uint32_t *rcs, const uint8_t *eq, const uint32_t *sS) {
    const uint32_t i = blockIdx.x * blockDim.x + threadIdx.x;
    if (i >= *defer_cnt) return;
    const uint4 e = defer[i];
    const uint32_t slot = e.y, pair = e.w & 0x7FFFFFFFu;
    const uint32_t ri = e.x & 0x7FFFFFFFu, sender = phase == 1 ? ri / d.K : ri;
    MsgDesc resp;
    resp.kind = 0; resp.len = 0; resp.off_lo = resp.off_hi = 0;
    bool differ = false;
    if (!eq[i]) {
        const uint32_t z = (e.w & 0x80000000u) ? lazy_slot(e.z, sS, sender) : 0u;
        const uint32_t scs = !(e.w & 0x80000000u) ? e.z : (z & 0x80000000u) ? rcs[sender] :
                             z < SRC_CLAIM ? d.dense_cs[z] : 0u;
        const uint32_t alias = d.dense_meta[slot].w;
        if (alias) d.dense_cs[slot] = d.dense_cs[alias - 1u];
        differ = d.dense_cs[slot] != scs;
    }
    if (differ) {
        resp.kind = 1; resp.off_lo = slot; resp.len = d.dense_meta[slot].z;
        ctr_add(d, phase == 1 ? C_FULL_SYNCS_PINGREQ : C_FULL_SYNCS, 1ull);
        ctr_add(d, C_X_DEFER_FS, 1ull);
        if (phase == 2) {
            const uint32_t ol = d.dense_meta[slot].x - d.lo;
            if (d.njobs[ol] < d.maxjobs) d.jobs[(size_t)ol * d.maxjobs + d.njobs[ol]++] = pair;
            else ctr_add(d, C_RFS_OMITTED, 1ull);
        } else if (phase == 0) {
            fsflag[pair] = 1;
        }
    }
    rdesc[ri] = resp;
    if (phase != 2) ctr_add(d, C_MSG_CHANGES, (unsigned long long)resp.len);
}

__global__ void k_defer_ids(DS d, const uint4 *defer, const uint32_t *defer_cnt, const uint8_t *eq, uint32_t *list,
                            uint32_t *cnt, int phase, const uint32_t *sS) {
    const uint32_t i = blockIdx.x * blockDim.x + threadIdx.x;
    if (i >= *defer_cnt || eq[i]) return;
    atomicAdd(cnt + 1, 1u);
    const uint4 e = defer[i];
    if (e.x & 0x80000000u) list[atomicAdd(cnt, 1u)] = d.NL + e.y;
    const uint32_t ri = e.x & 0x7FFFFFFFu, sender = phase == 1 ? ri / d.K : ri;
    const uint32_t z = lazy_slot(e.z, sS, sender);
    if ((e.w & 0x80000000u) && !(z & 0x80000000u) && z < d.dense_cap)
        list[atomicAdd(cnt, 1u)] = d.NL + z;
}

__global__ void k_build_jobs(DS d, const uint32_t *ukeys, const uint32_t *counts, const uint32_t *offs,
                             const uint32_t *vals, uint32_t nruns, uint8_t *fsflag) {
    const uint32_t u = blockIdx.x * blockDim.x + threadIdx.x;
    if (u >= nruns || ukeys[u] >= d.N) return;
    const uint32_t ol = ukeys[u] - d.lo;
    for (uint32_t w = 0; w < counts[u]; w++) {
        const uint32_t p = offs[u] + w;
        if (!fsflag[p]) continue;
        fsflag[p] = 0;
        if (d.njobs[ol] < d.maxjobs) d.jobs[(size_t)ol * d.maxjobs + d.njobs[ol]++] = vals[p];
        else ctr_add(d, C_RFS_OMITTED, 1ull);
    }
}

__global__ void k_resp(DS d, const int32_t *tgt, const uint8_t *failed, const MsgDesc *sdesc, const MsgDesc *rdesc,
                       uint32_t r) {
    const uint32_t ol = wave_gid();
    if (ol >= d.NL) return;
    if (tgt[ol] < 0 || failed[ol]) return;
    const uint32_t o = d.lo + ol;
    RowPre p = row_pre(d, ol);
    const uint32_t now = wave_clock(d, o, r);
    const MsgDesc sd = sdesc[o], rd = rdesc[o];
    uint4 rec0[MB];
    merge_first(d, rd, rec0);
    wave_bump_pre(d, ol, sd, p);
    wave_merge_msg_pre(d, ol, o, rd, now, now, 1, p, C_X_DENSE_RESP, rec0);
    if (lane_id() == 0) {
        ctr_add(d, C_PINGS_OK, 1ull);
        if (sd.kind == 0) ctr_add(d, C_X_BUMPED, (unsigned long long)sd.len);
    }
}

__global__ void k_resolve(DS d, const int32_t *tgt, const uint8_t *failed, const uint32_t *H, const uint32_t *nh,
                          const MsgDesc *sdesc2, const MsgDesc *rdesc2, uint32_t r) {
    const uint32_t ol = wave_gid();
    if (ol >= d.NL || !failed[ol]) return;
    const uint32_t o = d.lo + ol, K = d.K;
    const uint32_t now = wave_clock(d, o, r);
    uint32_t errs = 0;
    for (uint32_t q = 0; q < nh[ol]; q++) {
        const uint32_t h = H[(size_t)ol * K + q];
        if (!reach(d, o, h)) {
            errs++;
            wave_bump(d, ol, sdesc2[o]);
        } else {
            wave_merge_msg(d, ol, o, rdesc2[(size_t)o * K + q], now, now, 2, C_X_DENSE_RESP);
        }
    }
    if (lane_id() == 0) {
        if (errs) ctr_add(d, C_HELPER_ERRORS, (unsigned long long)errs);
        if (errs == K) {
            ctr_add(d, C_INCONCLUSIVE, 1ull);
        } else {
            ctr_add(d, C_SUSPECT_DECL, 1ull);
            const uint32_t t = (uint32_t)tgt[ol];
            const uint32_t te = d.mw[(size_t)ol * d.NP + t] >> 3;
            thread_make_change(d, ol, o, t, te, ST_SUSPECT, now);
        }
    }
}

__global__ void k_jobs_mark(DS d, uint8_t *need) {
    const uint32_t ol = blockIdx.x * blockDim.x + threadIdx.x;
    if (ol >= d.NL) return;
    for (uint32_t q = 0; q < d.njobs[ol]; q++) need[d.jobs[(size_t)ol * d.maxjobs + q]] = 1;
}

__global__ void k_jobs_snap(DS d, const uint8_t *need, MsgDesc *snapdesc) {
    const uint32_t ol = wave_gid();
    if (ol >= d.NL || !need[d.lo + ol]) return;
    MsgDesc md;
    wave_snapshot(d, ol, d.lo + ol, md);
    if (lane_id() == 0) snapdesc[d.lo + ol] = md;
}

__global__ void k_jobs_merge(DS d, const MsgDesc *snapdesc, uint32_t r) {
    const uint32_t ol = wave_gid();
    if (ol >= d.NL) return;
    const uint32_t nj = d.njobs[ol];
    if (!nj) return;
    const uint32_t now = wave_clock(d, d.lo + ol, r);
    for (uint32_t q = 0; q < nj; q++) {
        const uint32_t src = d.jobs[(size_t)ol * d.maxjobs + q];
        wave_merge_msg(d, ol, d.lo + ol, snapdesc[src], now, now, 3, C_X_DENSE_JOBS);
    }
    if (lane_id() == 0 && nj) ctr_add(d, C_RFS_DONE, (unsigned long long)nj);
}

__global__ void k_jobs_reset(DS d, uint8_t *need) {
    const uint32_t i = blockIdx.x * blockDim.x + threadIdx.x;
    if (i < d.NL) d.njobs[i] = 0;
    if (i < d.N) need[i] = 0;
}

__global__ void k_fp_keys(DS d, const uint32_t *list, uint32_t n, unsigned long long *keys, uint32_t *vals,
                          unsigned long long keymask) {
    const uint32_t i = blockIdx.x * blockDim.x + threadIdx.x;
    if (i >= n) return;
    keys[i] = d.fp[list[i]] & keymask;
    vals[i] = list[i];
}

__global__ void k_fp_heads(const unsigned long long *keys, uint32_t n, uint32_t *headpos) {
    const uint32_t i = blockIdx.x * blockDim.x + threadIdx.x;
    if (i >= n) return;
    headpos[i] = (i == 0 || keys[i] != keys[i - 1]) ? i : 0u;
}

__global__ void k_fp_verify(DS d, const uint32_t *vals, const uint32_t *headpos, uint32_t n, uint8_t *hflag,
                            uint32_t *dup_of) {
    const uint32_t i = wave_gid();
    if (i >= n) return;
    const uint32_t row = vals[i], hp = headpos[i];
    bool same = false;
    if (hp != i) {
        const uint32_t head = vals[hp];
        const uint32_t *ha = d.hidx ? d.hmw + (size_t)head * d.HP : nullptr, *hb = d.hidx ? d.hmw + (size_t)row * d.HP : nullptr;
        same = !wave_rows_differ(d, d.mw + (size_t)head * d.NP, d.mw + (size_t)row * d.NP, ha, hb);
    }
    if (lane_id() == 0) {
        dup_of[row] = same ? vals[hp] : SRC_NONE;
        hflag[row] = same ? 0 : 1;
    }
}

__global__ void k_list_flagged(uint32_t nl, uint8_t *flag, uint32_t *list, uint32_t *cnt) {
    const uint32_t ol = blockIdx.x * blockDim.x + threadIdx.x;
    if (ol >= nl || !flag[ol]) return;
    flag[ol] = 0;
    list[atomicAdd(cnt, 1u)] = ol;
}

__device__ __forceinline__ void fp_slot_tag(unsigned long long fp, uint32_t mask, uint32_t &slot, uint32_t &slot2,
                                            uint32_t &tag) {
    slot = (uint32_t)fp & mask;
    tag = (uint32_t)(fp >> 32);
    slot2 = (tag ^ (uint32_t)(fp >> 13)) & mask;
}
__global__ void k_fp_table(DS d, const uint32_t *list, uint32_t n, unsigned long long *tab, uint32_t mask,
                           unsigned long long keymask, int pass) {
    const uint32_t i = blockIdx.x * blockDim.x + threadIdx.x;
    if (i >= n) return;
    const uint32_t row = list[i];
    uint32_t slot, slot2, tag;
    fp_slot_tag(d.fp[row] & keymask, mask, slot, slot2, tag);
    const unsigned long long key = ((unsigned long long)tag << 32) | row;
    if (pass == 0) atomicMin(tab + slot, key);
    else if ((uint32_t)(tab[slot] >> 32) != tag) atomicMin(tab + (mask + 1) + slot2, key);
}
__global__ void k_fp_verify_tab(DS d, const uint32_t *list, uint32_t n, const unsigned long long *tab, uint32_t mask,
                                unsigned long long keymask, uint8_t *hflag, uint32_t *dup_of) {
    const uint32_t i = wave_gid();
    if (i >= n) return;
    const uint32_t row = list[i];
    uint32_t slot, slot2, tag;
    fp_slot_tag(d.fp[row] & keymask, mask, slot, slot2, tag);
    unsigned long long key = tab[slot];
    if ((uint32_t)(key >> 32) != tag) key = tab[(mask + 1) + slot2];
    const uint32_t head = (uint32_t)key;
    bool same = false;
    if ((uint32_t)(key >> 32) == tag && head != row) {
        const uint32_t *ha = d.hidx ? d.hmw + (size_t)head * d.HP : nullptr, *hb = d.hidx ? d.hmw + (size_t)row * d.HP : nullptr;
        same = !wave_rows_differ(d, d.mw + (size_t)head * d.NP, d.mw + (size_t)row * d.NP, ha, hb);
    }
    if (lane_id() == 0) {
        dup_of[row] = same ? head : SRC_NONE;
        hflag[row] = same ? 0 : 1;
    }
}
__device__ __forceinline__ uint4 flags16(const uint8_t *flag, uint32_t base, uint32_t nl) {
    if (base + 16u <= nl) return *(const uint4 *)(flag + base);
    uint32_t w[4] = {0, 0, 0, 0};
    for (uint32_t k = 0; base + k < nl && k < 16u; k++) w[k >> 2] |= (uint32_t)flag[base + k] << (8u * (k & 3u));
    return make_uint4(w[0], w[1], w[2], w[3]);
}
__global__ void __launch_bounds__(1024) k_list_flagged_ordered(uint32_t nl, uint8_t *flag, uint32_t *list, uint32_t *cnt) {
    __shared__ uint32_t wtot[16];
    const uint32_t t = threadIdx.x, per = ((nl + 1023u) / 1024u + 15u) & ~15u;
    const uint32_t lo = t * per;
    uint32_t c = 0;
    for (uint32_t q = 0; q < per && lo + q < nl; q += 16) {
        const uint4 v = flags16(flag, lo + q, nl);
        c += __popc(v.x) + __popc(v.y) + __popc(v.z) + __popc(v.w);
    }
    uint32_t wt;
    const uint32_t ex = wscan_excl(c, wt);
    if (lane_id() == 63) wtot[t >> 6] = wt;
    __syncthreads();
    uint32_t base = 0, all = 0;
    for (uint32_t w = 0; w < 16; w++) {
        const uint32_t v = wtot[w];
        base += w < (t >> 6) ? v : 0u;
        all += v;
    }
    uint32_t p = base + ex;
    for (uint32_t q = 0; q < per && lo + q < nl && c; q += 16) {
        const uint4 v = flags16(flag, lo + q, nl);
        const uint32_t w4[4] = {v.x, v.y, v.z, v.w};
        if ((v.x | v.y | v.z | v.w) == 0) continue;
        for (uint32_t k = 0; k < 16u; k++)
            if ((w4[k >> 2] >> (8u * (k & 3u))) & 0xFFu) {
                list[p++] = lo + q + k;
                flag[lo + q + k] = 0;
            }
    }
    if (t == 0) *cnt = all;
}

__global__ void k_fp_copy(DS d, const uint32_t *vals, uint32_t n, const uint32_t *dup_of) {
    const uint32_t i = blockIdx.x * blockDim.x + threadIdx.x;
    if (i >= n) return;
    const uint32_t row = vals[i], h = dup_of[row];
    if (h == SRC_NONE) return;
    d.cs[row] = d.cs[h];
    d.dirty[row] = 0;
    ctr_add(d, C_X_CS_DUP, 1ull);
}

__global__ void k_snap_rows(DS d, const uint32_t *rows, uint32_t n, uint32_t *ids, uint32_t *idcnt, uint32_t slot0) {
    const uint32_t k = wave_gid();
    if (k == 0 && lane_id() == 0) *idcnt = n;
    if (k >= n) return;
    const uint32_t ol = rows[k], slot = slot0 + k;
    const uint4 *src = (const uint4 *)(d.mw + (size_t)ol * d.NP);
    uint4 *dst = (uint4 *)(d.dense + (size_t)slot * d.NP);
    for (uint32_t i = lane_id(); i < d.NP / 4; i += 64 * SNAP_MB) {
        uint4 v[SNAP_MB];
#pragma unroll
        for (int u = 0; u < SNAP_MB; u++) v[u] = i + u * 64 < d.NP / 4 ? src[i + u * 64] : make_uint4(0, 0, 0, 0);
#pragma unroll
        for (int u = 0; u < SNAP_MB; u++)
            if (i + u * 64 < d.NP / 4) dst[i + u * 64] = v[u];
    }
    if (lane_id() == 0) {
        d.dense_meta[slot] = make_uint4(d.lo + ol, 0, 0, 0);
        d.dense_len[slot] = d.clen[ol];
        d.dense_last[slot] = d.clast[ol];
        d.cpslot[ol] = slot;
        d.dirty[ol] = 0;
        ids[k] = d.NL + slot;
    }
}

__global__ void k_snap_dups(DS d, const uint32_t *vals, uint32_t n, const uint32_t *dup_of) {
    const uint32_t i = blockIdx.x * blockDim.x + threadIdx.x;
    if (i >= n) return;
    const uint32_t row = vals[i], h = dup_of ? dup_of[row] : SRC_NONE;
    if (h != SRC_NONE) {
        d.cpslot[row] = d.cpslot[h];
        d.dirty[row] = 0;
    }
}

__global__ void k_side_retire(DS d, uint32_t lo, uint32_t hi) {
    const uint32_t ol = blockIdx.x * blockDim.x + threadIdx.x;
    if (ol >= d.NL) return;
    const uint32_t s = d.cpslot[ol];
    if (s < lo || s >= hi) return;
    d.cs[ol] = d.dense_cs[s];
    d.cpslot[ol] = SRC_NONE;
}

#include "swimsim_checksum.hip"

__global__ void k_snapshot_row(DS d, uint32_t ol, MsgDesc *out) {
    MsgDesc md;
    wave_snapshot(d, ol, d.lo + ol, md);
    if (lane_id() == 0) *out = md;
}

__device__ __forceinline__ uint32_t outgoing(uint32_t st) { return st == ST_TOMB ? ST_FAULTY : st; }

__global__ void k_heal_diff(DS d, const MsgDesc *ma, const MsgDesc *mb, MsgDesc *outA, MsgDesc *outB) {
    const uint32_t *A = d.dense + (size_t)ma->off_lo * d.NP;
    const uint32_t *B = d.dense + (size_t)mb->off_lo * d.NP;
    int na = 0, nb = 0;
    for (uint32_t m = lane_id(); m < d.N; m += 64) {
        const uint32_t a = A[m], b = B[m];
        if ((a & 7u) == ST_UNKNOWN || (b & 7u) == ST_UNKNOWN) continue;
        const uint32_t as = outgoing(a & 7u), bs = outgoing(b & 7u);
        const uint32_t ak = ((a >> 3) << 3) | as, bk = ((b >> 3) << 3) | bs;
        if (is_pingable(bs) && ak > bk && !is_pingable(as)) nb++;
        if (is_pingable(as) && bk > ak && !is_pingable(bs)) na++;
    }
    na = wsum(na);
    nb = wsum(nb);
    const unsigned long long oa = pool_alloc(d, (uint32_t)na);
    const unsigned long long ob = pool_alloc(d, (uint32_t)nb);
    uint32_t pa = 0, pb = 0;
    for (uint32_t base = 0; base < d.NP; base += 64) {
        const uint32_t m = base + lane_id();
        bool wa = false, wb = false;
        uint32_t a = 0, b = 0;
        if (m < d.N) {
            a = A[m]; b = B[m];
            if ((a & 7u) != ST_UNKNOWN && (b & 7u) != ST_UNKNOWN) {
                const uint32_t as = outgoing(a & 7u), bs = outgoing(b & 7u);
                const uint32_t ak = ((a >> 3) << 3) | as, bk = ((b >> 3) << 3) | bs;
                wb = is_pingable(bs) && ak > bk && !is_pingable(as);
                wa = is_pingable(as) && bk > ak && !is_pingable(bs);
            }
        }
        const unsigned long long ma_ = __ballot(wa), mb_ = __ballot(wb);
        if (wa && oa != ~0ull) d.pool[oa + pa + __popcll(ma_ & lanemask_lt())] = rec_make(m, ST_SUSPECT, b >> 3, SRC_NONE, 0, RT_LOOKUP);
        if (wb && ob != ~0ull) d.pool[ob + pb + __popcll(mb_ & lanemask_lt())] = rec_make(m, ST_SUSPECT, a >> 3, SRC_NONE, 0, RT_LOOKUP);
        pa += __popcll(ma_);
        pb += __popcll(mb_);
// ... 123 lines not shown
```

Measured before the change: 97.87 million member-rounds/s.

## Replace radix-sort inbox grouping with counting-sort bucketing and single-pass scan

Receiver inboxes are now built by counting messages per receiver during pair generation, running a decoupled-lookback scan to get offsets, and scattering values into buckets, instead of a CUB radix sort plus run-length encode plus scan. Within-bucket order is restored by rank counting in k_pair_info. Several memsets are folded into kernels, and the host read of run info with its stream sync is dropped; k_recv is launched over all rows. This cuts sort passes, launches and a host round-trip, but adds per-bucket O(c^2) ranking, a spin-wait scan and more recv waves.

```diff
diff --git a/ringpop-go_amd/csrc/swimsim_engine.hip b/ringpop-go_amd/csrc/swimsim_engine.hip
--- a/ringpop-go_amd/csrc/swimsim_engine.hip
+++ b/ringpop-go_amd/csrc/swimsim_engine.hip
@@ -278,7 +278,7 @@
     uint2 *needlist = nullptr;
     uint32_t *needcnt = nullptr, needcap = 0;
     uint32_t *hsics = nullptr, *npairs = nullptr;
-    unsigned long long *keys = nullptr, *keys_sorted = nullptr;
+    unsigned long long *keys = nullptr;
     uint32_t keycap = 0;
     uint64_t x_bytes = 0, x_calls = 0;
     uint64_t x_syncs = 0;
@@ -295,10 +295,12 @@
              *dup_of = nullptr;
     uint8_t *hflag = nullptr;
     uint32_t *H = nullptr, *nh = nullptr;
-    uint32_t *keys_in = nullptr, *vals_out = nullptr;
+    uint32_t *kslot = nullptr, *vals_in = nullptr, *run_of = nullptr, *vals_out = nullptr;
     uint4 *pinfo = nullptr;
     uint32_t inbox_n = 0;
-    uint32_t *ukeys = nullptr, *counts = nullptr, *offs = nullptr, *nruns = nullptr, *info = nullptr;
+    uint32_t *counts = nullptr, *offs = nullptr, *ulist = nullptr, *info = nullptr;
+    unsigned long long *scan_agg = nullptr;
+    uint32_t scan_gen = 0;
     void *cub_tmp = nullptr;
     size_t cub_bytes = 0;
     uint32_t *list = nullptr, *cnt = nullptr;
@@ -586,25 +588,17 @@
     return 0;
 }
 
-int sort_inbox(swimsim *h, uint32_t n, uint32_t *host_info) {
+int build_inbox(swimsim *h, uint32_t nlocal, uint32_t n) {
     Scope sc(h, F_SORT);
     h->inbox_n = n;
-    int endbit = 1;
-    while ((1u << endbit) <= h->N) endbit++;
-    size_t bytes = h->cub_bytes;
-    HIPCHK(h, hipcub::DeviceRadixSort::SortKeys(h->cub_tmp, bytes, h->keys, h->keys_sorted, (int)n, 0, 32 + endbit, h->s));
-    hipLaunchKernelGGL(k_split_keys, dim3(blocks_for_threads(n)), dim3(256), 0, h->s, h->keys_sorted, n, h->keys_in,
-                       h->vals_out);
-    bytes = h->cub_bytes;
-    HIPCHK(h, hipcub::DeviceRunLengthEncode::Encode(h->cub_tmp, bytes, h->keys_in, h->ukeys, h->counts, h->nruns,
-                                                    (int)n, h->s));
-    bytes = h->cub_bytes;
-    HIPCHK(h, hipcub::DeviceScan::ExclusiveSum(h->cub_tmp, bytes, h->counts, h->offs, (int)n, h->s));
-    HIPCHK(h, hipMemsetAsync(h->info, 0, 8, h->s));
-    hipLaunchKernelGGL(k_runs_info, dim3(blocks_for_threads(n)), dim3(256), 0, h->s, h->ukeys, h->counts, h->nruns, h->N,
-                       h->info);
-    HIPCHK(h, hipMemcpyAsync(host_info, h->info, 16, hipMemcpyDeviceToHost, h->s));
-    HIPCHK(h, stream_sync(h));
+    if (n > nlocal)
+        hipLaunchKernelGGL(k_inbox_count, dim3(blocks_for_threads(n - nlocal)), dim3(256), 0, h->s, h->d, h->keys, nlocal,
+                           n, h->counts, h->kslot);
+    h->scan_gen = h->scan_gen % 0x1FFFFFu + 1u;
+    hipLaunchKernelGGL(k_inbox_scan, dim3((h->NL + 1023) / 1024), dim3(1024), 0, h->s, h->d, h->counts, h->offs,
+                       h->ulist, h->scan_agg, h->scan_gen);
+    hipLaunchKernelGGL(k_inbox_place, dim3(blocks_for_threads(n)), dim3(256), 0, h->s, h->d, h->keys, n, h->offs,
+                       h->kslot, h->vals_in, h->run_of);
     return 0;
 }
 
@@ -844,7 +838,7 @@
         size_t bytes = cub_bytes;
         HIPCHK(h, hipcub::DeviceScan::ExclusiveSum(cub, bytes, c.Lb, c.OB, (int)h->N + 1, st));
         HIPCHK(h, hipMemsetAsync(c.SBw, 0, h->csr_sbw_words * 4, st));
-        hipLaunchKernelGGL(k_ucols, dim3(1), dim3(1024), 0, st, d);
+        hipLaunchKernelGGL(k_ucols, dim3(1), dim3(1024), 0, st, d, (uint32_t *)nullptr);
         hipLaunchKernelGGL(k_csr_ucol, dim3((h->N + 255) / 256), dim3(256), 0, st, d.ucl, d.ucnt, c.B, c.OB, c.ucol);
         launch_csr(d, list, n, cnt, ca, a, st, 0);
         launch_csr(d, list, n, cnt, ca, a, st, 1);
@@ -1007,7 +1001,7 @@
         for (int pass = 0; pass < 2; pass++)
             hipLaunchKernelGGL(k_fp_table, dim3(blocks_for_threads(n)), dim3(256), 0, h->s, h->d, h->list, n, h->fp_tab,
                                fmask, keymask, pass);
-        hipLaunchKernelGGL(k_ucols, dim3(1), dim3(1024), 0, h->s, h->d);
+        hipLaunchKernelGGL(k_ucols, dim3(1), dim3(1024), 0, h->s, h->d, (uint32_t *)nullptr);
         hipLaunchKernelGGL(k_fp_verify_tab, dim3(blocks_for_waves(n)), dim3(SWIM_WAVE_BLOCK), 0, h->s, h->d, h->list, n,
                            h->fp_tab, fmask, keymask, h->hflag, h->dup_of);
         hipLaunchKernelGGL(k_list_flagged_ordered, dim3(1), dim3(1024), 0, h->s, h->NL, h->hflag, h->fplist, h->fpcnt);
@@ -1045,8 +1039,7 @@
     uint32_t maxlist = 2 * maxn;
     {
         Scope sc(h, F_CSPREP);
-        HIPCHK(h, hipMemsetAsync(h->cnt, 0, 8, h->s));
-        hipLaunchKernelGGL(k_ucols, dim3(1), dim3(1024), 0, h->s, h->d);
+        hipLaunchKernelGGL(k_ucols, dim3(1), dim3(1024), 0, h->s, h->d, h->cnt);
         if (h->rep_tab) {
             h->rep_gen = h->rep_gen % 255u + 1u;
             hipLaunchKernelGGL(k_cs_reps, dim3(blocks_for_threads(h->NL)), dim3(256), 0, h->s, h->d, h->defer_cnt, h->rep_tab,
@@ -1072,12 +1065,10 @@
         maxlist += h->keycap;
     }
     {
-        uint32_t *hc = h->hinfo + 10;
-        HIPCHK(h, hipMemcpyAsync(hc, h->cnt, 4, hipMemcpyDeviceToHost, h->s));
-        HIPCHK(h, hipMemcpyAsync(hc + 1, h->cnt + 1, 4, hipMemcpyDeviceToHost, h->s));
-        HIPCHK(h, hipMemcpyAsync(h->hinfo + 14, h->defer_cnt, 4, hipMemcpyDeviceToHost, h->s));
+        uint32_t *hc = h->hinfo + 13;
+        HIPCHK(h, hipMemcpyAsync(hc, h->cnt, 12, hipMemcpyDeviceToHost, h->s));
         HIPCHK(h, stream_sync(h));
-        if (phase != 2) h->round_deferred += h->hinfo[14];
+        if (phase != 2) h->round_deferred += hc[2];
         if (int rc = hash_rows(h, h->list, h->cnt, maxlist, *hc)) return rc;
         if (hc[1])
             if (int rc = sync_side(h)) return rc;
@@ -1093,10 +1084,9 @@
     return 0;
 }
 
-int run_waves(swimsim *h, int phase, uint32_t nruns_valid, uint32_t maxcount) {
+int run_waves(swimsim *h, int phase, uint32_t maxpairs) {
     RecvArgs a{};
-    a.ukeys = h->ukeys; a.counts = h->counts; a.offs = h->offs; a.vals = h->vals_out;
-    a.nruns_max = nruns_valid;
+    a.counts = h->counts; a.offs = h->offs; a.ulist = h->ulist;
     a.phase = phase;
     a.sdesc = phase == 0 ? h->sdesc : h->sdesc2;
     a.sI = phase == 0 ? h->sI : h->sI2;
@@ -1108,22 +1098,22 @@
     a.fsflag = h->fsflag;
     a.r = h->round;
     a.pinfo = h->pinfo;
-    hipMemsetAsync(h->defer_cnt, 0, 4, h->s);
     {
         Scope sc(h, F_SORT);
         hipLaunchKernelGGL(k_pair_info, dim3(blocks_for_threads(std::max(h->inbox_n, h->NL))), dim3(256), 0, h->s, h->d,
-                           h->vals_out, h->inbox_n, phase, a.sdesc, a.sI, a.sC, a.sS, h->pinfo);
+                           h->vals_in, h->run_of, h->counts, h->offs, h->inbox_n, phase, a.sdesc, a.sI, a.sC, a.sS,
+                           h->pinfo, h->vals_out, h->defer_cnt);
     }
     {
         Scope sc(h, F_RECV);
-        hipLaunchKernelGGL(k_recv, dim3(blocks_for_waves(nruns_valid)), dim3(SWIM_WAVE_BLOCK), 0, h->s, h->d, a);
-    }
-    const uint32_t maxdefer = std::min<uint64_t>((uint64_t)nruns_valid * maxcount, h->d.dense_cap);
+        hipLaunchKernelGGL(k_recv, dim3(blocks_for_waves(h->NL)), dim3(SWIM_WAVE_BLOCK), 0, h->s, h->d, a);
+    }
+    const uint32_t maxdefer = std::min(maxpairs, h->d.dense_cap);
     if (int rc = resolve_deferred(h, phase, a.rdesc, maxdefer)) return rc;
     if (phase == 0) {
         Scope sc(h, F_RECVFIN);
-        hipLaunchKernelGGL(k_build_jobs, dim3(blocks_for_threads(nruns_valid)), dim3(256), 0, h->s, h->d, h->ukeys,
-                           h->counts, h->offs, h->vals_out, nruns_valid, h->fsflag);
+        hipLaunchKernelGGL(k_build_jobs, dim3(blocks_for_threads(h->NL)), dim3(256), 0, h->s, h->d, h->counts, h->offs,
+                           h->vals_out, h->fsflag);
     }
     return 0;
 }
@@ -1346,13 +1336,12 @@
         Scope sc(h, F_SELECT);
         hipMemsetAsync(h->exh_cnt, 0, 4, h->s);
         hipLaunchKernelGGL(k_select, dim3(blocks_for_threads(h->NL)), dim3(256), 0, h->s, h->d, h->tgt, h->exh_list,
-                           h->exh_cnt);
+                           h->exh_cnt, h->counts, h->info);
         hipLaunchKernelGGL(k_select_exhaust, dim3(64), dim3(64), 0, h->s, h->d, h->exh_list, h->exh_cnt, h->scratch);
     }
     uint32_t *hi = h->hinfo;
     uint32_t ninbox = h->NL;
     if (int rc = bound_lazy_snapshots(h, 1)) return rc;
-    HIPCHK(h, hipMemsetAsync(h->d.dense_cur, 0, 4, h->s));
     hot_update(h);
     {
         {
@@ -1361,9 +1350,9 @@
                                h->sdesc, h->sI, h->sC, h->sS);
         }
         Scope sc(h, F_SORT);
-        HIPCHK(h, hipMemsetAsync(h->info + 2, 0, 4, h->s));
         hipLaunchKernelGGL(k_pairs_direct, dim3(blocks_for_threads(h->NL)), dim3(256), 0, h->s, h->d, h->tgt, h->keys,
-                           h->failed, h->info, h->xitems, h->xcnt, h->xcap);
+                           h->failed, h->info, h->xitems, h->xcnt, h->xcap, h->counts, h->kslot);
+        HIPCHK(h, hipMemcpyAsync(&hi[2], h->info + 2, 4, hipMemcpyDeviceToHost, h->s));
     }
     if (sharded) {
         HIPCHK(h, hipMemcpyAsync(h->npairs, &h->NL, 4, hipMemcpyHostToDevice, h->s));
@@ -1374,9 +1363,9 @@
         HIPCHK(h, stream_sync(h));
         ninbox = std::min(hi[5], h->keycap);
     }
-    if (int rc = sort_inbox(h, ninbox, hi)) return rc;
+    if (int rc = build_inbox(h, h->NL, ninbox)) return rc;
+    if (int rc = run_waves(h, 0, ninbox)) return rc;
     const uint32_t nfailed = hi[2];
-    if (int rc = run_waves(h, 0, hi[0], hi[1])) return rc;
     if (sharded) {
         hipLaunchKernelGGL(k_x_resp, dim3(blocks_for_threads(ninbox)), dim3(256), 0, h->s, h->d, h->keys, ninbox, 0,
                            h->xitems, h->xcnt, h->xcap);
@@ -1393,10 +1382,9 @@
         {
             Scope sc(h, F_PINGREQ);
             hipLaunchKernelGGL(k_helpers, dim3(blocks_for_threads(h->NL)), dim3(256), 0, h->s, h->d, h->tgt, h->failed,
-                               h->H, h->nh, r);
+                               h->H, h->nh, r, h->counts);
         }
         if (int rc = bound_lazy_snapshots(h, 2)) return rc;
-        HIPCHK(h, hipMemsetAsync(h->d.dense_cur, 0, 4, h->s));
         {
             {
                 Scope sc(h, F_ISSUE);
@@ -1405,7 +1393,7 @@
             }
             Scope sc(h, F_PINGREQ);
             hipLaunchKernelGGL(k_pairs_helpers, dim3(blocks_for_threads(h->NL * h->K)), dim3(256), 0, h->s, h->d,
-                               h->failed, h->H, h->nh, h->keys, h->xitems, h->xcnt, h->xcap);
+                               h->failed, h->H, h->nh, h->keys, h->xitems, h->xcnt, h->xcap, h->counts, h->kslot);
         }
         uint32_t ninbox2 = h->NL * h->K;
         if (sharded) {
@@ -1415,8 +1403,9 @@
             HIPCHK(h, stream_sync(h));
             ninbox2 = std::min(hi[5], h->keycap);
         }
-        if (int rc = sort_inbox(h, ninbox2, hi)) return rc;
-        if (int rc = run_waves(h, 1, hi[0], hi[1])) return rc;
+        if (int rc = build_inbox(h, h->NL * h->K, ninbox2)) return rc;
+        const uint64_t pairs2 = (uint64_t)nfailed * h->K + (ninbox2 - std::min(ninbox2, h->NL * h->K));
+        if (int rc = run_waves(h, 1, (uint32_t)std::min<uint64_t>(pairs2, ninbox2))) return rc;
         if (sharded) {
             hipLaunchKernelGGL(k_x_resp, dim3(blocks_for_threads(ninbox2)), dim3(256), 0, h->s, h->d, h->keys, ninbox2, 1,
                                h->xitems, h->xcnt, h->xcap);
@@ -1746,7 +1735,9 @@
         size_t freeb = 0, totalb = 0;
         hipMemGetInfo(&freeb, &totalb);
         const uint64_t by_mem = (uint64_t)(freeb / 3) / (4ull * h->NP);
-        d.dense_cap = (uint32_t)std::max<uint64_t>(64, std::min<uint64_t>(2ull * h->NL + 64, by_mem));
+        const uint64_t per_row = 2ull * h->NL + 64, all_pings = (uint64_t)h->N + h->NL + 64;
+        const uint64_t want_slots = std::max(per_row, std::min<uint64_t>(all_pings, 4096));
+        d.dense_cap = (uint32_t)std::max<uint64_t>(64, std::min<uint64_t>(want_slots, by_mem));
         if (tun && tun->dense_slots >= 0)
             d.dense_cap = std::max<uint32_t>(64, std::min<uint32_t>(d.dense_cap, (uint32_t)tun->dense_slots));
         const uint64_t snap_mem = (uint64_t)(freeb / 8) / (4ull * h->NP);
@@ -1780,13 +1771,15 @@
         (rc = dalloc(h, &h->fplist, h->NL, "fplist")) || (rc = dalloc(h, &h->fpcnt, 1, "fpcnt")) ||
         (rc = dalloc(h, &h->dup_of, h->NL, "dup_of")) || (rc = dalloc(h, &h->hflag, h->NL, "hflag")) || (rc = dalloc(h, &h->d.fp, h->NL, "fp")) ||
         (rc = dalloc(h, &h->H, NLK, "H")) || (rc = dalloc(h, &h->nh, h->NL, "nh")) ||
-        (rc = dalloc(h, &h->keys, KC, "keys")) || (rc = dalloc(h, &h->keys_sorted, KC, "keys_sorted")) ||
-        (rc = dalloc(h, &h->keys_in, KC, "receivers")) || (rc = dalloc(h, &h->vals_out, KC, "vals_out")) ||
+        (rc = dalloc(h, &h->keys, KC, "keys")) || (rc = dalloc(h, &h->kslot, KC, "inbox key slots")) ||
+        (rc = dalloc(h, &h->vals_in, KC, "vals_in")) || (rc = dalloc(h, &h->run_of, KC, "inbox runs")) ||
+        (rc = dalloc(h, &h->vals_out, KC, "vals_out")) ||
         (rc = dalloc(h, &h->pinfo, (size_t)KC * 2, "inbox pair snapshots")) ||
-        (rc = dalloc(h, &h->ukeys, KC, "ukeys")) || (rc = dalloc(h, &h->counts, KC, "counts")) ||
-        (rc = dalloc(h, &h->offs, KC, "offs")) || (rc = dalloc(h, &h->nruns, 1, "nruns")) ||
+        (rc = dalloc(h, &h->counts, h->NL, "counts")) || (rc = dalloc(h, &h->offs, (size_t)h->NL + 2, "offs")) ||
+        (rc = dalloc(h, &h->ulist, h->NL, "receiving rows")) ||
+        (rc = dalloc(h, &h->scan_agg, ((size_t)h->NL + 1023) / 1024, "inbox scan sums")) ||
         (rc = dalloc(h, &h->info, 8, "info")) || (rc = dalloc(h, &h->list, 3 * KC + 2 * (size_t)h->NL + 64, "list")) ||
-        (rc = dalloc(h, &h->cnt, 2, "cnt")) || (rc = dalloc(h, &h->defer, KC + 2 * (size_t)h->NL + 64, "defer")) ||
+        (rc = dalloc(h, &h->cnt, 3, "cnt")) || (rc = dalloc(h, &h->defer, KC + 2 * (size_t)h->NL + 64, "defer")) ||
         (rc = dalloc(h, &h->defer_eq, KC + 2 * (size_t)h->NL + 64, "defer eq")) ||
         (rc = dalloc(h, &h->rep_tab, (size_t)rep_slots(h->NL), "checksum representatives")) ||
         (rc = dalloc(h, &h->fp_tab, (size_t)rep_slots(h->NL) * 4, "dedup groups")) ||
@@ -1794,12 +1787,14 @@
         (rc = dalloc(h, &h->d.ulog_cnt, (size_t)h->NL, "receive-phase undo log counts")) ||
         (rc = dalloc(h, &h->d.ilen, (size_t)h->NL, "issue-time checksum lengths")) ||
         (rc = dalloc(h, &h->d.ilast, (size_t)h->NL, "issue-time last members")) ||
-        (rc = dalloc(h, &h->defer_cnt, 1, "defer_cnt")) || (rc = dalloc(h, &h->exh_list, h->NL, "exh_list")) ||
+        (rc = dalloc(h, &h->exh_list, h->NL, "exh_list")) ||
         (rc = dalloc(h, &h->exh_cnt, 1, "exh_cnt")) || (rc = dalloc(h, &h->scratch, (size_t)64 * (h->NP / 32), "scratch")) ||
         (rc = dalloc(h, &h->need, h->N, "need")) || (rc = dalloc(h, &h->digest_buf, 4, "digest")) ||
         (rc = dalloc(h, &h->fsflag, KC, "fsflag")) || (rc = dalloc(h, &h->hsics, 4, "hsics")) ||
         (rc = dalloc(h, &h->npairs, 1, "npairs")))
         return bail(rc);
+    h->defer_cnt = h->cnt + 2;
+    hipMemset(h->scan_agg, 0, ((size_t)h->NL + 1023) / 1024 * 8);
     h->rep_mask = (h->defer_test & 16) ? 0u : rep_slots(h->NL) - 1u;
     h->d.ulog_stride = ULOG_STRIDE;
     h->d.ulog_cap = (h->defer_test & 8) ? 2u : ULOG_CAP;
@@ -1809,15 +1804,9 @@
     if ((rc = dalloc(h, &h->evbuf, h->evcap, "events")) || (rc = dalloc(h, &h->ev_applied, h->evcap, "ev_applied")))
         return bail(rc);
     {
-        size_t b1 = 0, b2 = 0, b3 = 0, b4 = 0, b5 = 0;
-        hipcub::DeviceRadixSort::SortKeys(nullptr, b1, h->keys, h->keys_sorted, (int)KC, 0, 64);
-        hipcub::DeviceRunLengthEncode::Encode(nullptr, b2, h->keys_in, h->ukeys, h->counts, h->nruns, (int)KC);
-        hipcub::DeviceScan::ExclusiveSum(nullptr, b3, h->counts, h->offs, (int)KC);
-        hipcub::DeviceRadixSort::SortPairs(nullptr, b4, h->keys, h->keys_sorted, h->fpv, h->fpv_s, (int)h->NL, 0, 64);
-        hipcub::DeviceScan::InclusiveScan(nullptr, b5, h->fph, h->fph_s, hipcub::Max(), (int)h->NL);
         size_t b6 = 0;
         hipcub::DeviceRadixSort::SortKeys(nullptr, b6, h->fplist, h->list, (int)h->NL, 0, 32);
-        h->cub_bytes = std::max(std::max(std::max(b1, b6), std::max(b2, b3)), std::max(b4, b5));
+        h->cub_bytes = b6;
         if ((rc = dalloc(h, (uint8_t **)&h->cub_tmp, h->cub_bytes, "cub temp"))) return bail(rc);
     }
     {
diff --git a/ringpop-go_amd/csrc/swimsim_kernels.hip b/ringpop-go_amd/csrc/swimsim_kernels.hip
--- a/ringpop-go_amd/csrc/swimsim_kernels.hip
+++ b/ringpop-go_amd/csrc/swimsim_kernels.hip
@@ -1073,9 +1073,11 @@
     wave_finalize(d, ol, acc, 0, false);
 }
 
-__global__ void k_select(DS d, int32_t *tgt, uint32_t *exh_list, uint32_t *exh_cnt) {
+__global__ void k_select(DS d, int32_t *tgt, uint32_t *exh_list, uint32_t *exh_cnt, uint32_t *counts, uint32_t *info) {
     const uint32_t ol = blockIdx.x * blockDim.x + threadIdx.x;
+    if (ol == 0) { info[2] = 0u; *d.dense_cur = 0u; }
     if (ol >= d.NL) return;
+    counts[ol] = 0u;
     const uint32_t o = d.lo + ol;
     int32_t target = -1;
     if (d.live[o]) {
@@ -1195,6 +1197,12 @@
     }
 }
 
+__device__ __forceinline__ void inbox_count(const DS &d, unsigned long long key, uint32_t *counts, uint32_t *kslot,
+                                            uint32_t i) {
+    const uint32_t u = (uint32_t)(key >> 32) - d.lo;
+    if (u < d.NL) kslot[i] = atomicAdd(&counts[u], 1u);
+}
+
 __device__ __forceinline__ void x_push(uint4 *items, uint32_t *cnt, uint32_t cap, uint32_t *err, uint4 it) {
     const uint32_t i = atomicAdd(cnt, 1u);
     if (i < cap) items[i] = it;
@@ -1202,7 +1210,7 @@
 }
 
 __global__ void k_pairs_direct(DS d, const int32_t *tgt, unsigned long long *keys, uint8_t *failed, uint32_t *info,
-                               uint4 *xitems, uint32_t *xcnt, uint32_t xcap) {
+                               uint4 *xitems, uint32_t *xcnt, uint32_t xcap, uint32_t *counts, uint32_t *kslot) {
     const uint32_t ol = blockIdx.x * blockDim.x + threadIdx.x;
     if (ol >= d.NL) return;
     const uint32_t o = d.lo + ol;
@@ -1221,11 +1229,15 @@
     }
     keys[ol] = key;
     failed[ol] = f;
-}
-
-__global__ void k_helpers(DS d, const int32_t *tgt, const uint8_t *failed, uint32_t *H, uint32_t *nh, uint32_t r) {
+    inbox_count(d, key, counts, kslot, ol);
+}
+
+__global__ void k_helpers(DS d, const int32_t *tgt, const uint8_t *failed, uint32_t *H, uint32_t *nh, uint32_t r,
+                          uint32_t *counts) {
     const uint32_t ol = blockIdx.x * blockDim.x + threadIdx.x;
+    if (ol == 0) *d.dense_cur = 0u;
     if (ol >= d.NL) return;
+    counts[ol] = 0u;
     nh[ol] = 0;
     if (!failed[ol]) return;
     const uint32_t o = d.lo + ol, t = (uint32_t)tgt[ol], K = d.K;
@@ -1259,7 +1271,8 @@
 }
 
 __global__ void k_pairs_helpers(DS d, const uint8_t *failed, const uint32_t *H, const uint32_t *nh,
-                                unsigned long long *keys, uint4 *xitems, uint32_t *xcnt, uint32_t xcap) {
+                                unsigned long long *keys, uint4 *xitems, uint32_t *xcnt, uint32_t xcap, uint32_t *counts,
+                                uint32_t *kslot) {
     const uint32_t i = blockIdx.x * blockDim.x + threadIdx.x;
     const uint32_t K = d.K;
     if (i >= d.NL * K) return;
@@ -1275,29 +1288,74 @@
         }
     }
     keys[i] = key;
-}
-
-__global__ void k_split_keys(const unsigned long long *keys, uint32_t n, uint32_t *recv, uint32_t *vals) {
+    inbox_count(d, key, counts, kslot, i);
+}
+
+__global__ void k_inbox_count(DS d, const unsigned long long *keys, uint32_t first, uint32_t n, uint32_t *counts,
+                              uint32_t *kslot) {
+    const uint32_t i = first + blockIdx.x * blockDim.x + threadIdx.x;
+    if (i < n) inbox_count(d, keys[i], counts, kslot, i);
+}
+
+__global__ void __launch_bounds__(1024) k_inbox_scan(DS d, const uint32_t *counts, uint32_t *offs, uint32_t *ulist,
+                                                     unsigned long long *agg, uint32_t gen) {
+    __shared__ unsigned long long wsum[16];
+    __shared__ unsigned long long prior;
+    const uint32_t t = threadIdx.x, lane = t & 63u, w = t >> 6, b = blockIdx.x;
+    const uint32_t i = b * 1024u + t, c = i < d.NL ? counts[i] : 0u;
+    const unsigned long long v = (unsigned long long)c | ((unsigned long long)(c != 0u) << 32);
+    unsigned long long x = v;
+    for (uint32_t o = 1; o < 64; o <<= 1) {
+        const unsigned long long y = __shfl_up(x, o);
+        if (lane >= o) x += y;
+    }
+    if (lane == 63) wsum[w] = x;
+    __syncthreads();
+    unsigned long long before = 0, all = 0;
+    for (uint32_t k = 0; k < 16; k++) {
+        const unsigned long long s = wsum[k];
+        before += k < w ? s : 0ull;
+        all += s;
+    }
+    if (t == 0)
+        __hip_atomic_store(&agg[b], ((unsigned long long)gen << 43) | all, __ATOMIC_RELAXED, __HIP_MEMORY_SCOPE_AGENT);
+    if (w == 0) {
+        unsigned long long s = 0;
+        for (uint32_t k = lane; k < b; k += 64) {
+            unsigned long long a;
+            while ((uint32_t)((a = __hip_atomic_load(&agg[k], __ATOMIC_RELAXED, __HIP_MEMORY_SCOPE_AGENT)) >> 43) != gen)
+                __builtin_amdgcn_s_sleep(1);
+            s += a & ((1ull << 43) - 1ull);
+        }
+        for (uint32_t o = 32; o; o >>= 1) s += __shfl_xor(s, o);
+        if (lane == 0) prior = s;
+    }
+    __syncthreads();
+    const unsigned long long at = prior + before + x - v;
+    if (i < d.NL) offs[i] = (uint32_t)at;
+    if (c) ulist[(uint32_t)(at >> 32)] = i;
+    if (i + 1 == d.NL) {
+        offs[d.NL] = (uint32_t)(at + v);
+        offs[d.NL + 1] = (uint32_t)((at + v) >> 32);
+    }
+}
+
+__global__ void k_inbox_place(DS d, const unsigned long long *keys, uint32_t n, const uint32_t *offs,
+                              const uint32_t *kslot, uint32_t *vals_in, uint32_t *run_of) {
     const uint32_t i = blockIdx.x * blockDim.x + threadIdx.x;
     if (i >= n) return;
     const unsigned long long k = keys[i];
-    recv[i] = (uint32_t)(k >> 32);
-    vals[i] = (uint32_t)k;
-}
-
-__global__ void k_runs_info(const uint32_t *ukeys, const uint32_t *counts, const uint32_t *nruns, uint32_t N,
-                            uint32_t *info) {
-    const uint32_t i = blockIdx.x * blockDim.x + threadIdx.x;
-    if (i >= *nruns) return;
-    if (ukeys[i] == N) return;
-    atomicMax(&info[1], counts[i]);
-    atomicAdd(&info[0], 1u);
+    const uint32_t u = (uint32_t)(k >> 32) - d.lo;
+    if (u >= d.NL) return;
+    const uint32_t p = offs[u] + kslot[i];
+    vals_in[p] = (uint32_t)k;
+    run_of[p] = u;
 }
 
 struct RecvArgs {
-    const uint32_t *ukeys, *counts, *offs, *vals;
+    const uint32_t *counts, *offs;
+    const uint32_t *ulist;
     const uint4 *pinfo;
-    uint32_t nruns_max;
     int phase;
     const MsgDesc *sdesc;
     const uint32_t *sI, *sC;
@@ -1309,16 +1367,43 @@
     uint32_t r;
 };
 
-__global__ void k_pair_info(const DS d, const uint32_t *vals, uint32_t n, int phase, const MsgDesc *sdesc, const uint32_t *sI,
-                            const uint32_t *sC, const uint32_t *sS, uint4 *pinfo) {
+constexpr uint32_t RANK_LANE_MAX = 64;
+__global__ void k_pair_info(const DS d, const uint32_t *vals_in, const uint32_t *run_of, const uint32_t *counts,
+                            const uint32_t *offs, uint32_t n, int phase, const MsgDesc *sdesc, const uint32_t *sI,
+                            const uint32_t *sC, const uint32_t *sS, uint4 *pinfo, uint32_t *vals_out, uint32_t *defer_cnt) {
     const uint32_t i = blockIdx.x * blockDim.x + threadIdx.x;
     if (d.ulog_cnt && i < d.NL) d.ulog_cnt[i] = 0u;
-    if (i >= n) return;
-    const uint32_t v = vals[i], sender = phase == 0 ? v : v / d.K;
+    if (i == 0) *defer_cnt = 0u;
+    const bool valid = i < min(n, offs[d.NL]);
+    uint32_t v = 0, off = 0, c = 0, rank = 0;
+    if (valid) {
+        const uint32_t u = run_of[i];
+        v = vals_in[i]; off = offs[u]; c = counts[u];
+    }
+    if (c > 1 && c <= RANK_LANE_MAX)
+        for (uint32_t k = 0; k < c; k++) rank += vals_in[off + k] < v;
+    unsigned long long todo = __ballot(c > RANK_LANE_MAX);
+    while (todo) {
+        const int l = __builtin_ctzll(todo);
+        const uint32_t off_u = (uint32_t)__shfl((int)off, l), c_u = (uint32_t)__shfl((int)c, l);
+        const bool mine = c > RANK_LANE_MAX && off == off_u;
+        uint32_t rk = 0;
+        for (uint32_t base = 0; base < c_u; base += 64) {
+            const uint32_t at = base + lane_id();
+            const uint32_t x = at < c_u ? vals_in[off_u + at] : 0xFFFFFFFFu;
+#pragma unroll
+            for (int k = 0; k < 64; k++) rk += (uint32_t)__builtin_amdgcn_readlane((int)x, k) < v;
+        }
+        if (mine) rank = rk;
+        todo &= ~__ballot(mine);
+    }
+    if (!valid) return;
+    const uint32_t p = off + rank, sender = phase == 0 ? v : v / d.K;
+    vals_out[p] = v;
     if (sender >= d.N) return;
     const MsgDesc md = sdesc[sender];
-    pinfo[2 * (size_t)i] = make_uint4(md.off_lo, md.off_hi, md.len, md.kind);
-    pinfo[2 * (size_t)i + 1] = make_uint4(sI[sender], sC[sender], sS ? sS[sender] : SRC_NONE, v);
+    pinfo[2 * (size_t)p] = make_uint4(md.off_lo, md.off_hi, md.len, md.kind);
+    pinfo[2 * (size_t)p + 1] = make_uint4(sI[sender], sC[sender], sS ? sS[sender] : SRC_NONE, v);
 }
 
 __device__ __forceinline__ void recv_one_pre(const DS &d, const RecvArgs &a, uint32_t j, const uint4 pi0, const uint4 pi1,
@@ -1385,11 +1470,11 @@
 
 constexpr int RECV_MIN_WAVES = 4;
 __global__ void __launch_bounds__(256, RECV_MIN_WAVES) k_recv(DS d, RecvArgs a) {
-    const uint32_t u = wave_gid();
-    if (u >= a.nruns_max) return;
-    const uint32_t key = a.ukeys[u];
-    if (key >= d.N) return;
-    const uint32_t n = a.counts[u], off = a.offs[u];
+    const uint32_t w = wave_gid();
+    if (w >= d.NL) return;
+    const uint32_t u = a.ulist[w];
+    if (w >= a.offs[d.NL + 1]) return;
+    const uint32_t n = a.counts[u], off = a.offs[u], key = d.lo + u;
     RowPre p = row_pre(d, key - d.lo);
     const uint32_t now = wave_clock(d, key, a.r);
     const uint32_t nslots = d.hidx ? d.hot_cnt[0] : 0u;
@@ -1418,11 +1503,12 @@
     }
 }
 
-__global__ void __launch_bounds__(1024) k_ucols(DS d) {
+__global__ void __launch_bounds__(1024) k_ucols(DS d, uint32_t *zero2) {
     __shared__ uint32_t part[1024];
     __shared__ uint32_t ncold;
     const uint32_t t = threadIdx.x, per = (d.NBIT + 1023) / 1024, w0 = t * per;
     if (t == 0) ncold = 0;
+    if (t == 0 && zero2) zero2[0] = zero2[1] = 0u;
     auto bitsof = [&](uint32_t w) -> uint32_t {
         const uint32_t x = d.colx[w], lo = w * 32;
         return lo + 32 <= d.N ? x : lo >= d.N ? 0u : x & ((1u << (d.N - lo)) - 1u);
@@ -1697,11 +1783,10 @@
         list[atomicAdd(cnt, 1u)] = d.NL + z;
 }
 
-__global__ void k_build_jobs(DS d, const uint32_t *ukeys, const uint32_t *counts, const uint32_t *offs,
-                             const uint32_t *vals, uint32_t nruns, uint8_t *fsflag) {
-    const uint32_t u = blockIdx.x * blockDim.x + threadIdx.x;
-    if (u >= nruns || ukeys[u] >= d.N) return;
-    const uint32_t ol = ukeys[u] - d.lo;
+__global__ void k_build_jobs(DS d, const uint32_t *counts, const uint32_t *offs, const uint32_t *vals,
+                             uint8_t *fsflag) {
+    const uint32_t u = blockIdx.x * blockDim.x + threadIdx.x, ol = u;
+    if (u >= d.NL) return;
     for (uint32_t w = 0; w < counts[u]; w++) {
         const uint32_t p = offs[u] + w;
         if (!fsflag[p]) continue;
```

Result: faster. 116.1 million member-rounds/s, median of 6 (+18.6%).
